# vitoplantamura/OnnxStream

Measured on AMD Instinct MI355X. Metric: sd15_unet_step_latency_ms+images_per_sec_512x512_20step, higher is better.
Workload: dtype f16

## Files before the change

include/osgpu.h:

```cpp
#ifndef OSGPU_H
#define OSGPU_H

#include <stddef.h>
#include <stdint.h>

#ifdef __cplusplus
extern "C" {
#endif

typedef struct osg_ctx osg_ctx;
typedef struct osg_graph osg_graph;

typedef enum { OSG_U8 = 1, OSG_F16 = 2, OSG_F32 = 3, OSG_I64 = 4 } osg_dtype;

typedef enum {
  OSG_ACT_NONE = 0,
  OSG_ACT_SILU = 1,
  OSG_ACT_SIGMOID = 2,
  OSG_ACT_GEGLU = 3
} osg_act;

typedef enum {
  OSG_UN_SIGMOID = 0,
  OSG_UN_ERF = 1,
  OSG_UN_SQRT = 2,
  OSG_UN_SIN = 3,
  OSG_UN_COS = 4,
  OSG_UN_NEG = 5,
  OSG_UN_POW = 6,
  OSG_UN_SILU = 7,
  OSG_UN_GELU_ERF = 8
} osg_unary_kind;

typedef enum {
  OSG_BIN_ADD = 0,
  OSG_BIN_SUB = 1,
  OSG_BIN_MUL = 2,
  OSG_BIN_DIV = 3
} osg_binary_kind;

int osg_device_count(void);
int osg_init(int device, osg_ctx** out);
void osg_destroy(osg_ctx* ctx);
const char* osg_last_error(const osg_ctx* ctx);
const char* osg_device_name(const osg_ctx* ctx);
void* osg_stream(const osg_ctx* ctx);
int osg_set_autotune(osg_ctx* ctx, int on);
int osg_tune_misses(void);

int osg_malloc(osg_ctx* ctx, size_t bytes, void** dptr);
int osg_free(osg_ctx* ctx, void* dptr);
int osg_upload(osg_ctx* ctx, void* dst, const void* host_src, size_t bytes);
int osg_upload_sync(osg_ctx* ctx, void* dst, const void* host_src, size_t bytes);
int osg_host_register(osg_ctx* ctx, void* host_ptr, size_t bytes);
int osg_host_unregister(osg_ctx* ctx, void* host_ptr);
int osg_upload_pinned(osg_ctx* ctx, void* dst, const void* pinned_host_src, size_t bytes);
int osg_upload_pinned_async(osg_ctx* ctx, void* dst, const void* pinned_host_src, size_t bytes);
int osg_copy_fence(osg_ctx* ctx);
int osg_download(osg_ctx* ctx, void* host_dst, const void* src, size_t bytes);
int osg_marker_record(osg_ctx* ctx, int slot);
int osg_copy_wait_marker(osg_ctx* ctx, int slot);
int osg_copy(osg_ctx* ctx, void* dst, const void* src, size_t bytes);
int osg_memset(osg_ctx* ctx, void* dst, int value, size_t bytes);
int osg_sync(osg_ctx* ctx);

int osg_graph_begin(osg_ctx* ctx);
int osg_graph_end(osg_ctx* ctx, osg_graph** out);
int osg_graph_launch(osg_ctx* ctx, osg_graph* g);
void osg_graph_destroy(osg_graph* g);

int osg_timer_start(osg_ctx* ctx);
int osg_timer_stop(osg_ctx* ctx, float* ms);
int osg_timer_mark(osg_ctx* ctx, int index);
int osg_timer_between(osg_ctx* ctx, int a, int b, float* ms);

void osg_range_push(const char* name);
void osg_range_pop(void);

int osg_conv2d_nhwc(osg_ctx* ctx, osg_dtype dtype, const void* x, const void* w_ohwi, const void* bias, osg_dtype bias_dtype,
                    const void* residual, void* y, int N, int H, int W, int Cin, int Cout, int KH, int KW, int stride_h,
                    int stride_w, int pad_top, int pad_left, int pad_bottom, int pad_right, osg_act act);

int osg_conv2d_nhwc_rb(osg_ctx* ctx, osg_dtype dtype, const void* x, const void* w_ohwi, const void* bias, osg_dtype bias_dtype,
                       const void* image_bias, long image_bias_ld, const void* residual, void* y, int N, int H, int W, int Cin, int Cout,
                       int KH, int KW, int stride_h, int stride_w, int pad_top, int pad_left, int pad_bottom, int pad_right, osg_act act);

int osg_conv2d_nhwc_v(osg_ctx* ctx, osg_dtype dtype, const void* x, const void* w_ohwi, const void* bias, osg_dtype bias_dtype,
                      const void* image_bias, long image_bias_ld, const void* residual, void* y, long y_ld, void* y2, long y2_ld, int N, int H, int W,
                      int Cin, int Cout, int KH, int KW, int stride_h, int stride_w, int pad_top, int pad_left, int pad_bottom, int pad_right,
                      osg_act act);

int osg_gemm(osg_ctx* ctx, osg_dtype dtype, const void* A, const void* B, int b_is_nk, const void* bias, osg_dtype bias_dtype,
             const void* residual, void* C, int M, int N, int K, int batch, long stride_a, long stride_b, long stride_c,
             osg_act act);

int osg_gemm_w8(osg_ctx* ctx, const void* A, const void* Bq_nk, float w_scale, int w_zero_point, const void* bias, osg_dtype bias_dtype,
                const void* residual, void* C, int M, int N, int K, osg_act act);
int osg_conv2d_nhwc_w8(osg_ctx* ctx, const void* x, const void* wq_ohwi, float w_scale, int w_zero_point, const void* bias,
                       osg_dtype bias_dtype, const void* image_bias, long image_bias_ld, const void* residual, void* y, int N, int H, int W,
                       int Cin, int Cout, int KH, int KW, int stride_h, int stride_w, int pad_top, int pad_left, int pad_bottom,
                       int pad_right, osg_act act);
int osg_gemm_w8_v(osg_ctx* ctx, const void* A, const void* Bq_nk, float w_scale, int w_zero_point, const float* w_scale_vec,
                  const float* w_zero_point_vec, const void* bias, osg_dtype bias_dtype, const void* residual, void* C, int M, int N, int K,
                  osg_act act);
int osg_conv2d_nhwc_w8_v(osg_ctx* ctx, const void* x, const void* wq_ohwi, float w_scale, int w_zero_point, const float* w_scale_vec,
                         const float* w_zero_point_vec, const void* bias, osg_dtype bias_dtype, const void* image_bias, long image_bias_ld,
                         const void* residual, void* y, long y_ld, void* y2, long y2_ld, int N, int H, int W, int Cin, int Cout, int KH, int KW,
                         int stride_h, int stride_w, int pad_top, int pad_left, int pad_bottom, int pad_right, osg_act act);

int osg_transpose_kn_to_nk(osg_ctx* ctx, osg_dtype dtype, const void* src_kn, void* dst_nk, int K, int N);
int osg_gemm_ln(osg_ctx* ctx, const void* x, const void* w_nk_folded, const float* c1, const float* c2, float eps, const float* rowstats,
                const void* residual, void* y, int M, int N, int K, osg_act act);
int osg_gemm_rowstats(osg_ctx* ctx, const void* A, const void* B_nk, const void* bias, osg_dtype bias_dtype, const void* residual, void* C,
                      int M, int N, int K, osg_act act, float* rowstats);
int osg_last_route(const osg_ctx* ctx, int out[5]);
int osg_last_kernel(const osg_ctx* ctx, int out[8]);

int osg_attention(osg_ctx* ctx, osg_dtype dtype, const void* q, const void* k, const void* v, void* o, int heads, int Tq, int Tkv,
                  int D, float scale, int k_is_dt);
int osg_attention_strided(osg_ctx* ctx, osg_dtype dtype, const void* q, long q_tok, long q_head, long q_batch, const void* k,
                          long k_tok, long k_head, long k_batch, const void* v, long v_tok, long v_head, long v_batch, void* o,
                          long o_tok, long o_head, long o_batch, int batch, int heads, int Tq, int Tkv, int D, float scale);
typedef struct {
  const void *a1, *x0;
  const void *wo1, *bo1;
  const void *g2, *be2;
  float eps2;
  const void *wq2, *bq2;
  const void *kp, *vtp;
  float scale;
  int Tk;
  const void *wo2, *bo2;
  const void *g3, *be3;
  float eps3;
  const void *w1, *b1, *w2, *b2;
  const void *wpo, *bpo, *xin;
  void *out, *out2;
  long ldo, ldo2;
  int M, rows_per_img, C, heads;
  void* dbg[8];
  int rows_per_block;
} osg_tblock_tail_args;
int osg_tblock_tail_supported(int M, int rows_per_img, int C, int heads, int Tk);
int osg_tblock_tail(osg_ctx* ctx, const osg_tblock_tail_args* a);
int osg_tblock_pack_weight(osg_ctx* ctx, const void* w_nk, int N, int K, void* w_kn8);
size_t osg_tblock_kv_pack_elems(int imgs, int heads, int D);
int osg_tblock_kv_pack_jobs(osg_ctx* ctx, const void* base, long ld, int imgs, int Tk, int heads, int njobs, const int* jobs_dev, void* dst);
int osg_rms_norm(osg_ctx* ctx, osg_dtype dtype, const void* x, const void* w, void* y, long rows, int C, float eps);
int osg_rope(osg_ctx* ctx, osg_dtype dtype, const void* x, const void* cos_t, const void* sin_t, void* y, long bh, long T, int d);
int osg_sdpa(osg_ctx* ctx, osg_dtype dtype, const void* q, const void* k, const void* v, const void* mask, void* o, int batch, int q_heads,
             int kv_heads, int Tq, int Tkv, int D, float scale);

int osg_instance_norm(osg_ctx* ctx, osg_dtype dtype, const void* x, const float* scale, const float* bias, void* y, int rows,
                      long L, int n_scale, float eps);
int osg_group_norm_nhwc(osg_ctx* ctx, osg_dtype dtype, const void* x, const void* gamma, const void* beta, void* y, int N, long HW,
                        int C, int groups, float eps, osg_act act);
int osg_set_stat_sinks(osg_ctx* ctx, void* table0, int groups0, int cpg0, int ch_off0, void* table1, int groups1, int cpg1, int ch_off1, int rows_per_image);
int osg_group_norm_stats_nhwc(osg_ctx* ctx, const void* x, const void* gamma, const void* beta, void* y, int N, long HW, int C, int G, float eps, osg_act act,
                              const void* stat_table);
int osg_layer_norm(osg_ctx* ctx, osg_dtype dtype, const void* x, const void* gamma, const void* beta, void* y, long rows, int C,
                   float eps);
int osg_reduce_mean_last(osg_ctx* ctx, osg_dtype dtype, const void* x, void* y, long rows, long C);
int osg_softmax_last(osg_ctx* ctx, osg_dtype dtype, const void* x, void* y, long rows, long C);

int osg_unary(osg_ctx* ctx, osg_dtype dtype, osg_unary_kind kind, const void* x, void* y, long n, float param);
int osg_binary(osg_ctx* ctx, osg_dtype dtype, osg_binary_kind kind, const void* a, const long* a_shape, const void* b,
               const long* b_shape, void* y, int rank);
int osg_geglu(osg_ctx* ctx, osg_dtype dtype, const void* x, void* y, long rows, long C);

int osg_sampler_prepare(osg_ctx* ctx, const float* x, float* sample, float* timestep, int prompts, long L, float c_in, float t,
                        long t_per_sample);
int osg_sampler_cfg_euler_a(osg_ctx* ctx, float* x, const float* eps, const float* noise, int prompts, long L, float c_out,
                            float guidance, float sigma, float d_sigma, float sigma_up, float clip);
typedef enum {
    OSG_MS_DPMPP_FIRST = 0, OSG_MS_DPMPP_2M = 1, OSG_MS_EULER_D = 2, OSG_MS_IPNDM1 = 3, OSG_MS_IPNDM_V1 = 4, OSG_MS_IPNDM2 = 5, OSG_MS_IPNDM3 = 6,
    OSG_MS_IPNDM_VO1 = 7, OSG_MS_IPNDM_VO2 = 8, OSG_MS_IPNDM_VO3 = 9, OSG_MS_TAYLOR1 = 10, OSG_MS_TAYLOR2 = 11, OSG_MS_DDIM = 12, OSG_MS_FORMS = 13
} osg_multistep_form;
int osg_sampler_cfg_multistep(osg_ctx* ctx, int form, float* x, const float* eps, float* h0, const float* h1, const float* h2, const float* h3,
                              int prompts, long L, float c_out, float guidance, float sigma, float k0, float k1, float k2, float k3, float k4,
                              double da, double db);
int osg_sampler_prepare_rescale(osg_ctx* ctx, float* x, float* sample, float* timestep, int prompts, long L, float x_scale, float c_in, float t,
                                long t_per_sample);

int osg_decode_gather(osg_ctx* ctx, const float* latents, float* tiles, int images, int H, int W, int tile, float factor);
int osg_decode_blend(osg_ctx* ctx, const float* tiles, float* image, unsigned char* pixels, int images, int H, int W, int tile, int up);

int osg_transpose(osg_ctx* ctx, int elem_size, const void* x, void* y, int rank, const long* shape, const int* perm);
int osg_copy_2d(osg_ctx* ctx, int elem_size, const void* src, long src_pitch, long src_off, void* dst, long dst_pitch,
                long dst_off, long outer, long inner);
int osg_concat2(osg_ctx* ctx, int elem_size, const void* a, long inner_a, const void* b, long inner_b, void* dst, long outer);
int osg_resize_nearest(osg_ctx* ctx, int elem_size, const void* x, void* y, int N, int C, int H, int W, int Ho, int Wo, int nhwc);
int osg_gather_rows(osg_ctx* ctx, int elem_size, const void* x, const int64_t* idx, void* y, long n_idx, long row_elems, long n_rows);
int osg_maxpool_nhwc(osg_ctx* ctx, osg_dtype dtype, const void* x, void* y, int N, int H, int W, int C, int KH, int KW, int sh,
                     int sw, int pt, int pl, int pb, int pr);

int osg_convert(osg_ctx* ctx, osg_dtype src_dtype, osg_dtype dst_dtype, const void* x, void* y, long n, float scale, int zero_point);

int osg_qu8_conv2d_nhwc(osg_ctx* ctx, const void* x, float x_scale, int x_zp, const void* w_ohwi, float w_scale, int w_zp, const float* bias_f32,
                        float out_scale, int out_zp, void* y, int N, int H, int W, int Cin, int Cout, int KH, int KW, int stride_h, int stride_w,
                        int pad_top, int pad_left, int pad_bottom, int pad_right);
int osg_qu8_conv_tap_sums(osg_ctx* ctx, const void* w_ohwi, int Cout, int KH, int KW, int Cin, int* tap_sums);
int osg_qu8_conv2d_nhwc_t(osg_ctx* ctx, const void* x, float x_scale, int x_zp, const void* w_ohwi, float w_scale, int w_zp, const float* bias_f32,
                          float out_scale, int out_zp, void* y, int N, int H, int W, int Cin, int Cout, int KH, int KW, int stride_h, int stride_w,
                          int pad_top, int pad_left, int pad_bottom, int pad_right, const int* tap_sums);
int osg_qu8_gemm(osg_ctx* ctx, const void* A, long lda, float a_scale, int a_zp, const void* B_nk, float b_scale, int b_zp, const float* bias_f32,
                 float out_scale, int out_zp, void* C, int M, int N, int K, int batch, long stride_a, long stride_b, long stride_c);
int osg_qu8_lut(osg_ctx* ctx, const void* x, void* y, long n, const void* lut256);
int osg_qu8_binary(osg_ctx* ctx, osg_binary_kind kind, const void* a, const long* a_shape, float a_scale, int a_zp, const void* b, const long* b_shape,
                   float b_scale, int b_zp, void* y, float out_scale, int out_zp, int rank);
int osg_qu8_instance_norm(osg_ctx* ctx, const void* x, void* y, int rows, long L, int n_scale, const float* scale, const float* bias, float eps,
                          float in_scale, int in_zp, float out_scale, int out_zp);
int osg_qu8_affine_act(osg_ctx* ctx, const void* x, float x_scale, int x_zp, const void* g, float g_scale, int g_zp, float m_scale, int m_zp, const void* b,
                       float b_scale, int b_zp, float a_scale, int a_zp, const void* sig_lut, float s_scale, int s_zp, float o_scale, int o_zp, void* y, long n, int C,
                       long inner);
int osg_qu8_norm_affine_act_nhwc(osg_ctx* ctx, const void* x, long HW, int C, int G, int n_scale, const float* scale, const float* bias, float eps, float x_scale,
                                 int x_zp, float n_out_scale, int n_out_zp, const void* g, float g_scale, int g_zp, float m_scale, int m_zp, const void* b, float b_scale,
                                 int b_zp, float a_scale, int a_zp, const void* sig_lut, float s_scale, int s_zp, float o_scale, int o_zp, void* y);
int osg_qu8_instance_norm_nhwc(osg_ctx* ctx, const void* x, void* y, long HW, int C, int G, int n_scale, const float* scale, const float* bias, float eps,
                               float in_scale, int in_zp, float out_scale, int out_zp);
int osg_qu8_softmax_last(osg_ctx* ctx, const void* x, void* y, long rows, long C, const void* lut_u32_256);

int osg_kdbg_read(osg_ctx* ctx, void* host_dst, size_t bytes);

#ifdef __cplusplus
}
#endif
#endif
```

onnxstream_amd/build.py:

```python
from __future__ import annotations

import glob
import os
import subprocess
import sys

ROOT = os.path.dirname(os.path.abspath(__file__))
REPO = os.path.dirname(ROOT)
CSRC = os.path.join(ROOT, "csrc")
INC = os.path.join(REPO, "include")
LIB_GPU = os.path.join(ROOT, "libosgpu.so")
LIB_HOST = os.environ.get("OSA_LIB_HOST") or os.path.join(ROOT, "libonnxstream_amd.so")
ORACLE_REF = os.path.join(REPO, "oracle", "_ref", "libonnxstream_ref.so")
HIPCC = os.environ.get("HIPCC", "/opt/rocm/bin/hipcc")


def _newer(target, deps):
    if not os.path.exists(target):
        return True
    t = os.path.getmtime(target)
    return any(os.path.getmtime(d) > t for d in deps)


def _run(cmd, **kw):
    r = subprocess.run(cmd, stdout=subprocess.PIPE, stderr=subprocess.STDOUT, text=True, **kw)
    if r.returncode != 0:
        sys.stderr.write(r.stdout)
        raise RuntimeError("build failed: " + " ".join(cmd))
    return r.stdout


def build_gpu(force=False, verbose=False):
    srcs = sorted(glob.glob(os.path.join(CSRC, "osg_*.hip")))
    hdrs = sorted(glob.glob(os.path.join(CSRC, "*.h"))) + [os.path.join(INC, "osgpu.h")]
    objdir = os.path.join(CSRC, "build")
    os.makedirs(objdir, exist_ok=True)
    objs, procs = [], []
    for s in srcs:
        o = os.path.join(objdir, os.path.basename(s)[:-4] + ".o")
        objs.append(o)
        if force or _newer(o, [s] + hdrs):
            cmd = [HIPCC, "--offload-arch=gfx950", "-O3", "-std=c++17", "-fPIC", "-mllvm", "-amdgpu-mfma-vgpr-form", "-I" + INC, "-I" + CSRC, "-c", s, "-o", o]
            procs.append((cmd, subprocess.Popen(cmd, stdout=subprocess.PIPE, stderr=subprocess.STDOUT, text=True)))
    for cmd, p in procs:
        out, _ = p.communicate()
        if p.returncode != 0:
            sys.stderr.write(out)
            raise RuntimeError("build failed: " + " ".join(cmd))
        if verbose and out:
            print(out)
    if force or procs or _newer(LIB_GPU, objs):
        _run([HIPCC, "--offload-arch=gfx950", "-shared", "-fPIC", "-o", LIB_GPU] + objs)
    return LIB_GPU


def build_host(force=False):
    hdir = os.path.join(CSRC, "host")
    srcs = sorted(glob.glob(os.path.join(hdir, "*.cpp")))
    if not srcs:
        return None
    hdrs = sorted(glob.glob(os.path.join(hdir, "*.h"))) + sorted(glob.glob(os.path.join(hdir, "*.inc"))) + [os.path.join(INC, "osgpu.h")]
    if force or _newer(LIB_HOST, srcs + hdrs):
        _run(["g++", "-std=c++20", "-O2", "-fPIC", "-shared", "-I" + INC, "-I" + hdir, "-o", LIB_HOST] + srcs +
             ["-ldl", "-lpthread"])
    return LIB_HOST


def build_oracle_ref():
    if os.path.isdir("/root/reference/src"):
        _run(["make", "-C", os.path.join(REPO, "oracle"), "ref"])
    return ORACLE_REF if os.path.exists(ORACLE_REF) else None


def build_all(force=False):
    build_gpu(force)
    build_host(force)
    build_oracle_ref()


if __name__ == "__main__":
    build_all("--force" in sys.argv)
    print("built:", LIB_GPU, LIB_HOST if os.path.exists(LIB_HOST) else "(no host yet)")
```

onnxstream_amd/csrc/osg_attention.hip:

```cpp
#include "osg_common.h"
#include <cstdlib>
#include <type_traits>
#include <utility>

namespace {

struct AttnParams {
    const f16 *q, *k, *v;
    f16* o;
    long q_tok, q_head, q_batch;
    long k_tok, k_head, k_batch;
    long v_tok, v_head, v_batch;
    long o_tok, o_head, o_batch;
    int heads, Tq, Tkv, D;
    float scale_log2e;
    const f16* mask;
    float inv_scale;
    int kv_div;
};


__device__ __forceinline__ void lane_swap16(float v, float& a, float& b) {
    a = v; b = v;
    asm volatile("s_nop 1\n\tv_permlane16_swap_b32 %0, %1" : "+v"(a), "+v"(b));
// ... 78 lines not shown
                const int dc = min(wave + c * 4, dchunks - 1);
                kreg[j][c] = *reinterpret_cast<const f16x8*>(K + krow + dc * 8);
                vreg[j][c] = *reinterpret_cast<const f16x8*>(V + vrow + dc * 8);
            }
        }
    };
    const int vcol = ((lane >> 5) << 5) + (((lane >> 2) & 3) << 3) + (((lane >> 4) & 1) << 2) + (lane & 3);
    auto store_tile = [&]() {
#pragma unroll
        for (int j = 0; j < RPL; j++)
#pragma unroll
            for (int c = 0; c < NCH; c++) {
                const int dc = wave + c * 4;
                if (dc < dchunks) {
                    const f16x8 kv8 = kreg[j][c], vv8 = vreg[j][c];
                    *reinterpret_cast<f16x8*>(&Ks[(j * 64 + lane) * KLD + dc * 8]) = kv8;
#pragma unroll
                    for (int e = 0; e < 8; e++) Vt[(dc * 8 + e) * VLD + j * 64 + vcol] = vv8[e];
                }
            }
    };
    load_tile(0);
    for (int kv0 = 0; kv0 < p.Tkv; kv0 += BKV) {
        __syncthreads();
        store_tile();
        __syncthreads();
        if (kv0 + BKV < p.Tkv) load_tile(kv0 + BKV);

        f32x4 s[QT][NT];
#pragma unroll
        for (int qt = 0; qt < QT; qt++)
#pragma unroll
            for (int t = 0; t < NT; t++) s[qt][t] = f32x4{0.f, 0.f, 0.f, 0.f};
#pragma unroll
        for (int t = 0; t < NT; t++) {
#pragma unroll
            for (int ks = 0; ks < KS; ks++) {
                f16x8 kf = *reinterpret_cast<const f16x8*>(&Ks[(t * 16 + lq) * KLD + ks * 32 + g * 8]);
#pragma unroll
                for (int qt = 0; qt < QT; qt++) s[qt][t] = __builtin_amdgcn_mfma_f32_16x16x32_f16(kf, qf[qt][ks], s[qt][t], 0, 0, 0);
            }
        }

        if (p.mask) {
#pragma unroll
            for (int qt = 0; qt < QT; qt++) {
                const f16* mrow = p.mask + (long)min(q0 + qt * 16 + lq, p.Tq - 1) * p.Tkv;
#pragma unroll
                for (int t = 0; t < NT; t++)
#pragma unroll
                    for (int r = 0; r < 4; r++)
                        s[qt][t][r] = fmaf((float)mrow[min(kv0 + t * 16 + g * 4 + r, p.Tkv - 1)], p.inv_scale, s[qt][t][r]);
            }
        }
        const bool full = kv0 + BKV <= p.Tkv;
        const float c = p.scale_log2e;
        f16x8 pf[QT][NS];
#pragma unroll
        for (int qt = 0; qt < QT; qt++) {
            float mx = -INFINITY;
            if (full) {
#pragma unroll
                for (int t = 0; t < NT; t++)
#pragma unroll
                    for (int r = 0; r < 4; r++) mx = fmaxf(mx, s[qt][t][r]);
            } else {
#pragma unroll
                for (int t = 0; t < NT; t++)
#pragma unroll
                    for (int r = 0; r < 4; r++) {
                        const int kv = kv0 + t * 16 + g * 4 + r;
                        const float x = kv < p.Tkv ? s[qt][t][r] : -INFINITY;
                        s[qt][t][r] = x;
                        mx = fmaxf(mx, x);
                    }
            }
            mx = row4_max(mx);
            const float m_new = fmaxf(m_run[qt], mx);
            const float m_use = m_new == -INFINITY ? 0.f : m_new;
            const float alpha = __builtin_amdgcn_exp2f((m_run[qt] - m_use) * c);
            const float mc = -m_use * c;
            float sum = 0.f;
#pragma unroll
            for (int t = 0; t < NT; t++)
#pragma unroll
                for (int r = 0; r < 4; r++) {
                    const float e = __builtin_amdgcn_exp2f(fmaf(s[qt][t][r], c, mc));
                    s[qt][t][r] = e;
                    sum += e;
                }
            sum = row4_sum(sum);
            l_run[qt] = l_run[qt] * alpha + sum;
            if (__builtin_amdgcn_ballot_w64(m_new != m_run[qt]) != 0) {
#pragma unroll
                for (int dt = 0; dt < DT; dt++)
#pragma unroll
                    for (int r = 0; r < 4; r++) oacc[qt][dt][r] *= alpha;
            }
            m_run[qt] = m_new;
#pragma unroll
            for (int st = 0; st < NS; st++) {
                f16x8 pv;
#pragma unroll
                for (int r = 0; r < 4; r++) {
                    pv[r] = (f16)s[qt][2 * st][r];
                    pv[4 + r] = (f16)s[qt][2 * st + 1][r];
                }
                pf[qt][st] = pv;
            }
        }

#pragma unroll
        for (int dt = 0; dt < DT; dt++) {
#pragma unroll
            for (int st = 0; st < NS; st++) {
                const f16x8 vf = *reinterpret_cast<const f16x8*>(&Vt[(dt * 16 + lq) * VLD + st * 32 + g * 8]);
#pragma unroll
                for (int qt = 0; qt < QT; qt++)
                    oacc[qt][dt] = __builtin_amdgcn_mfma_f32_16x16x32_f16(vf, pf[qt][st], oacc[qt][dt], 0, 0, 0);
            }
        }
    }

#pragma unroll
    for (int qt = 0; qt < QT; qt++) {
        const int q = q0 + qt * 16 + lq;
        if (q >= p.Tq) continue;
        const float inv = 1.0f / l_run[qt];
#pragma unroll
        for (int dt = 0; dt < DT; dt++) {
            const int d = dt * 16 + g * 4;
            if (d >= D) continue;
            f16x4 o;
#pragma unroll
            for (int r = 0; r < 4; r++) o[r] = (f16)(oacc[qt][dt][r] * inv);
            *reinterpret_cast<f16x4*>(O + (long)q * p.o_tok + d) = o;
        }
    }
}

template <class F, int... I>
__device__ __forceinline__ void attn2_static_for(F&& f, std::integer_sequence<int, I...>) { (f(std::integral_constant<int, I>{}), ...); }
template <int N>
__device__ __forceinline__ void attn2_wait_vm() { asm volatile("s_waitcnt vmcnt(%0)" ::"n"(N) : "memory"); }
typedef __fp16 attn2_hx4 __attribute__((__vector_size__(4 * sizeof(__fp16))));
template <int OFF>
__device__ __forceinline__ attn2_hx4 attn2_tr_read(unsigned lds_addr) {
    attn2_hx4 v;
    asm volatile("ds_read_b64_tr_b16 %0, %1 offset:%2" : "=v"(v) : "v"(lds_addr), "n"(OFF));
    return v;
}

template <int D, int QT, int NST>
__global__ __launch_bounds__(256) void attn2_kernel(AttnParams pk, int nqb) {
    const AttnParams p = pk;
    osg_pin_all(p.q, p.k, p.v, p.o, p.q_tok, p.q_head, p.q_batch, p.k_tok, p.k_head, p.k_batch, p.v_tok, p.v_head, p.v_batch, p.o_tok, p.o_head, p.o_batch, p.heads, p.Tq, p.Tkv,
                p.scale_log2e, p.mask, p.inv_scale, p.kv_div, nqb, (int)gridDim.x);
    constexpr int DCH = D / 8;
    constexpr int RSC = DCH + ((6 - DCH % 4) % 4);
    constexpr int ROWB = RSC * 16;
    constexpr int TILE_B = 64 * ROWB;
    constexpr int STAGE_B = 2 * TILE_B;
    constexpr int K32 = D / 32, REM = D % 32;
    static_assert(REM == 0 || REM == 8 || REM == 16, "attn2: head dim = 32 a (+ 8 | 16)");
    static_assert(RSC % 4 == 2 && RSC >= DCH && (REM == 0 || RSC * 8 >= K32 * 32 + 16), "row pitch");
    constexpr bool TAIL = REM != 0;
    constexpr int DT = (D + 15) / 16;
    static_assert(DT * 16 <= RSC * 8, "the P V row blocks read inside the padded row");
    constexpr int NT = 4, NS = 2;
    constexpr int NINST = 2 * RSC;
    constexpr int MAXP = NINST / 4;
    static_assert((NST == 3 || NST == 4) && MAXP * (NST - 2) <= 63, "three or four stages (the tile being read, the next one, one or two in flight: sync_issue's tail guard `kt + 2 >= ntiles` covers no deeper ring); vmcnt is a 6-bit counter");
    constexpr unsigned OOB = 0x80000000u;
    extern __shared__ __attribute__((aligned(16))) char asmem[];
    typedef __attribute__((address_space(3))) void* lds_ptr;
    typedef attn2_hx4 hx4;

    const int tid = threadIdx.x, lane = tid & 63;
    const int wave = __builtin_amdgcn_readfirstlane(tid >> 6);
    const int lq = lane & 15, g = lane >> 4;
    int L;
    {
        const int total = gridDim.x, bid = blockIdx.x, x = bid & 7, i = bid >> 3, q = total >> 3, r = total & 7;
        L = (x < r ? x * (q + 1) : r * (q + 1) + (x - r) * q) + i;
    }
    const int bh = L / nqb, qb = L - bh * nqb;
    const int b = bh / p.heads, h = bh - b * p.heads;
    const int q0 = qb * (64 * QT) + wave * (16 * QT);

    const f16* __restrict__ Q = p.q + b * p.q_batch + h * p.q_head;
    const f16* __restrict__ K = p.k + b * p.k_batch + (h / p.kv_div) * p.k_head;
    const f16* __restrict__ V = p.v + b * p.v_batch + (h / p.kv_div) * p.v_head;
    f16* __restrict__ O = p.o + b * p.o_batch + h * p.o_head;

    const long kext = ((long)(p.Tkv - 1) * p.k_tok + D) * 2, vext = ((long)(p.Tkv - 1) * p.v_tok + D) * 2;
    __amdgpu_buffer_rsrc_t rsK = __builtin_amdgcn_make_buffer_rsrc((void*)K, 0, (int)(kext < 0x7ffffff0L ? kext : 0x7ffffff0L), 0x00020000);
    __amdgpu_buffer_rsrc_t rsV = __builtin_amdgcn_make_buffer_rsrc((void*)V, 0, (int)(vext < 0x7ffffff0L ? vext : 0x7ffffff0L), 0x00020000);

    int p_off[MAXP], p_row[MAXP];
#pragma unroll
    for (int j = 0; j < MAXP; j++) {
        const int i = wave + 4 * j;
        const bool isv = i >= RSC;
        const int c = (isv ? i - RSC : i) * 64 + lane;
        const int row = c / RSC, pp = c - row * RSC;
        p_row[j] = pp < DCH ? row : 64;
        p_off[j] = (int)(((long)row * (isv ? p.v_tok : p.k_tok) + pp * 8) * 2);
    }
    const int ntiles = (p.Tkv + 63) >> 6;
    auto issue_tile = [&](int kt) __attribute__((always_inline)) {
        char* st = asmem + (kt % NST) * STAGE_B;
        const int kv0 = kt << 6, left = min(p.Tkv - kv0, 64);
        const int sk = (int)((long)kv0 * p.k_tok * 2), sv = (int)((long)kv0 * p.v_tok * 2);
#pragma unroll
        for (int j = 0; j < MAXP; j++) {
            const int i = wave + 4 * j;
            const unsigned off = p_row[j] < left ? (unsigned)p_off[j] : OOB;
            if (i < RSC) __builtin_amdgcn_raw_ptr_buffer_load_lds(rsK, (lds_ptr)(st + i * 1024), 16, off, sk, 0, 0);
            else __builtin_amdgcn_raw_ptr_buffer_load_lds(rsV, (lds_ptr)(st + i * 1024), 16, off, sv, 0, 0);
        }
    };

    f16x8 qf[QT][K32 ? K32 : 1];
    f16x8 qtail[QT];
#pragma unroll
    for (int qt = 0; qt < QT; qt++) {
        const int q = q0 + qt * 16 + lq;
        const f16* qrow = Q + (long)min(q, p.Tq - 1) * p.q_tok;
#pragma unroll
        for (int ks = 0; ks < K32; ks++) qf[qt][ks] = *reinterpret_cast<const f16x8*>(qrow + ks * 32 + g * 8);
        if constexpr (TAIL) {
            const int d = K32 * 32 + g * 8;
            f16x8 v = *reinterpret_cast<const f16x8*>(qrow + min(d, D - 8));
            if (d >= D) v = f16x8{0, 0, 0, 0, 0, 0, 0, 0};
            qtail[qt] = v;
        }
    }
#pragma unroll
    for (int s2 = 0; s2 < NST - 1; s2++)
        if (s2 < ntiles) issue_tile(s2);

    f32x4 oacc[QT][DT], lacc[QT];
    float m_run[QT];
#pragma unroll
    for (int qt = 0; qt < QT; qt++) {
        m_run[qt] = -INFINITY;
        lacc[qt] = f32x4{0.f, 0.f, 0.f, 0.f};
#pragma unroll
        for (int dt = 0; dt < DT; dt++) oacc[qt][dt] = f32x4{0.f, 0.f, 0.f, 0.f};
    }
    const f16x8 ones = {(f16)1, (f16)1, (f16)1, (f16)1, (f16)1, (f16)1, (f16)1, (f16)1};

    int kofs[K32 + 1];
#pragma unroll
    for (int ks = 0; ks < K32 + 1; ks++) kofs[ks] = lq * ROWB + (ks * 4 + g) * 16;
    const int vofs = TILE_B + (g * 4 + (lq >> 2)) * ROWB + (lq & 3) * 8;
    const float c = p.scale_log2e;

    auto qk = [&](auto stc, f32x4 (&s)[QT][NT]) __attribute__((always_inline)) {
        constexpr int stg = decltype(stc)::value;
        const char* St = asmem + stg * STAGE_B;
#pragma unroll
        for (int qt = 0; qt < QT; qt++)
#pragma unroll
            for (int t = 0; t < NT; t++) s[qt][t] = f32x4{0.f, 0.f, 0.f, 0.f};
#pragma unroll
        for (int ks = 0; ks < K32 + (TAIL ? 1 : 0); ks++)
#pragma unroll
            for (int t = 0; t < NT; t++) {
                const f16x8 kf = *reinterpret_cast<const f16x8*>(St + t * 16 * ROWB + kofs[ks]);
#pragma unroll
                for (int qt = 0; qt < QT; qt++) s[qt][t] = __builtin_amdgcn_mfma_f32_16x16x32_f16(kf, ks < K32 ? qf[qt][ks < K32 ? ks : 0] : qtail[qt], s[qt][t], 0, 0, 0);
            }
    };
    auto softmax = [&](auto fullc, f32x4 (&s)[QT][NT], int kv0, f16x8 (&pf)[QT][NS]) __attribute__((always_inline)) {
        constexpr bool full = decltype(fullc)::value;
#pragma unroll
        for (int qt = 0; qt < QT; qt++) {
            float mx = -INFINITY;
            if constexpr (full) {
#pragma unroll
                for (int t = 0; t < NT; t++)
#pragma unroll
                    for (int r = 0; r < 4; r++) mx = fmaxf(mx, s[qt][t][r]);
            } else {
#pragma unroll
                for (int t = 0; t < NT; t++)
#pragma unroll
                    for (int r = 0; r < 4; r++) {
                        const int kv = kv0 + t * 16 + g * 4 + r;
                        const float x = kv < p.Tkv ? s[qt][t][r] : -INFINITY;
                        s[qt][t][r] = x;
                        mx = fmaxf(mx, x);
                    }
            }
            mx = row4_max(mx);
            const float m_new = fmaxf(m_run[qt], mx);
            const float mc = -m_new * c;
            if (__builtin_amdgcn_ballot_w64(m_new != m_run[qt]) != 0) {
                const float alpha = __builtin_amdgcn_exp2f((m_run[qt] - m_new) * c);
#pragma unroll
                for (int dt = 0; dt < DT; dt++)
#pragma unroll
                    for (int r = 0; r < 4; r++) oacc[qt][dt][r] *= alpha;
#pragma unroll
                for (int r = 0; r < 4; r++) lacc[qt][r] *= alpha;
            }
            m_run[qt] = m_new;
#pragma unroll
            for (int st = 0; st < NS; st++) {
                f16x8 pv;
#pragma unroll
                for (int r = 0; r < 4; r++) {
                    pv[r] = (f16)__builtin_amdgcn_exp2f(fmaf(s[qt][2 * st][r], c, mc));
                    pv[4 + r] = (f16)__builtin_amdgcn_exp2f(fmaf(s[qt][2 * st + 1][r], c, mc));
                }
                pf[qt][st] = pv;
            }
        }
    };
    auto pvstep = [&](auto stc, f16x8 (&pf)[QT][NS]) __attribute__((always_inline)) {
        constexpr int stg = decltype(stc)::value;
#pragma unroll
        for (int st = 0; st < NS; st++)
#pragma unroll
            for (int qt = 0; qt < QT; qt++) lacc[qt] = __builtin_amdgcn_mfma_f32_16x16x32_f16(ones, pf[qt][st], lacc[qt], 0, 0, 0);
        constexpr int SB = stg * STAGE_B, IMM = (SB + 48 * ROWB + DT * 32 < 65536) ? SB : 0;
        const unsigned va = (unsigned)(size_t)(lds_ptr)(asmem + vofs + (SB - IMM));
        hx4 vr[2][NS][2];
        auto vread = [&](auto dtc) __attribute__((always_inline)) {
            constexpr int dt = decltype(dtc)::value;
            vr[dt & 1][0][0] = attn2_tr_read<IMM + 0 * ROWB + dt * 32>(va);
            vr[dt & 1][0][1] = attn2_tr_read<IMM + 16 * ROWB + dt * 32>(va);
            vr[dt & 1][1][0] = attn2_tr_read<IMM + 32 * ROWB + dt * 32>(va);
            vr[dt & 1][1][1] = attn2_tr_read<IMM + 48 * ROWB + dt * 32>(va);
        };
        auto vstep = [&](auto dtc) __attribute__((always_inline)) {
            constexpr int dt = decltype(dtc)::value;
            hx4 &a0 = vr[dt & 1][0][0], &a1 = vr[dt & 1][0][1], &a2 = vr[dt & 1][1][0], &a3 = vr[dt & 1][1][1];
            if constexpr (dt + 1 < DT) {
                vread(std::integral_constant<int, dt + 1>{});
                asm volatile("s_waitcnt lgkmcnt(4)" : "+v"(a0), "+v"(a1), "+v"(a2), "+v"(a3)::"memory");
            } else asm volatile("s_waitcnt lgkmcnt(0)" : "+v"(a0), "+v"(a1), "+v"(a2), "+v"(a3)::"memory");
#pragma unroll
            for (int st = 0; st < NS; st++) {
                const hx4 lo = vr[dt & 1][st][0], hi = vr[dt & 1][st][1];
                const f16x8 vf = {(f16)lo[0], (f16)lo[1], (f16)lo[2], (f16)lo[3], (f16)hi[0], (f16)hi[1], (f16)hi[2], (f16)hi[3]};
#pragma unroll
                for (int qt = 0; qt < QT; qt++)
                    oacc[qt][dt] = __builtin_amdgcn_mfma_f32_16x16x32_f16(vf, pf[qt][st], oacc[qt][dt], 0, 0, 0);
            }
        };
        vread(std::integral_constant<int, 0>{});
        attn2_static_for(vstep, std::make_integer_sequence<int, DT>{});
    };
    auto sync_issue = [&](int kt) __attribute__((always_inline)) {
        if (NST == 3 || kt + 2 >= ntiles) attn2_wait_vm<0>();
        else attn2_wait_vm<MAXP * (NST - 3)>();
        __builtin_amdgcn_s_barrier();
        if (kt + NST - 1 < ntiles) issue_tile(kt + NST - 1);
    };
    f32x4 sA[QT][NT], sB[QT][NT];
    sync_issue(-1);
    qk(std::integral_constant<int, 0>{}, sA);
    constexpr int U = (NST % 2) ? 2 * NST : NST;
    auto step = [&](auto ic, int kt) __attribute__((always_inline)) {
        constexpr int i = decltype(ic)::value;
        f32x4 (&sc)[QT][NT] = (i & 1) ? sB : sA;
        f32x4 (&sn)[QT][NT] = (i & 1) ? sA : sB;
        f16x8 pf[QT][NS];
        sync_issue(kt);
        qk(std::integral_constant<int, (i + 1) % NST>{}, sn);
        softmax(std::true_type{}, sc, kt << 6, pf);
        pvstep(std::integral_constant<int, i % NST>{}, pf);
    };
    auto last = [&](auto ic, int kt) __attribute__((always_inline)) {
        constexpr int i = decltype(ic)::value;
        f32x4 (&sc)[QT][NT] = (i & 1) ? sB : sA;
        f16x8 pf[QT][NS];
        if ((p.Tkv & 63) == 0) softmax(std::true_type{}, sc, kt << 6, pf);
        else softmax(std::false_type{}, sc, kt << 6, pf);
        pvstep(std::integral_constant<int, i % NST>{}, pf);
    };
    int kt = 0;
    for (; kt + U < ntiles; kt += U)
        attn2_static_for([&](auto ic) __attribute__((always_inline)) { step(ic, kt + decltype(ic)::value); }, std::make_integer_sequence<int, U>{});
    bool done = false;
    attn2_static_for([&](auto ic) __attribute__((always_inline)) {
        const int k2 = kt + decltype(ic)::value;
        if (!done) {
            if (k2 + 1 < ntiles) step(ic, k2);
            else { last(ic, k2); done = true; }
        }
    }, std::make_integer_sequence<int, U>{});

#pragma unroll
    for (int qt = 0; qt < QT; qt++) {
        const int q = q0 + qt * 16 + lq;
        if (q >= p.Tq) continue;
        const float inv = 1.0f / lacc[qt][0];
#pragma unroll
        for (int dt = 0; dt < DT; dt++) {
            const int d = dt * 16 + g * 4;
            if (d >= D) continue;
            f16x4 o;
#pragma unroll
            for (int r = 0; r < 4; r++) o[r] = (f16)(oacc[qt][dt][r] * inv);
            *reinterpret_cast<f16x4*>(O + (long)q * p.o_tok + d) = o;
        }
    }
}

template <int D, int NST>
int launch_attn2(osg_ctx* ctx, const AttnParams& p, int batch) {
    static const int force_qt = getenv("OSG_ATTN_QT") ? atoi(getenv("OSG_ATTN_QT")) : 0;
    constexpr int RSC = D / 8 + ((6 - (D / 8) % 4) % 4);
    constexpr size_t smem = (size_t)NST * 2 * 64 * RSC * 16;
    static_assert(smem <= 160 * 1024, "LDS budget");
    const long blocks128 = (long)((p.Tq + 127) / 128) * batch * p.heads;
    const bool qt2 = p.Tq >= 1024 && force_qt != 1 && (blocks128 >= 2L * ctx->num_cu || force_qt == 2);
    auto k1 = attn2_kernel<D, 1, NST>;
    auto k2 = attn2_kernel<D, 2, NST>;
    static unsigned long long attr_mask = 0;
    if (osg_first_on_device(attr_mask)) {
        OSG_HIP(ctx, hipFuncSetAttribute((const void*)k1, hipFuncAttributeMaxDynamicSharedMemorySize, (int)smem));
        OSG_HIP(ctx, hipFuncSetAttribute((const void*)k2, hipFuncAttributeMaxDynamicSharedMemorySize, (int)smem));
    }
    const int nqb = qt2 ? (p.Tq + 127) / 128 : (p.Tq + 63) / 64;
    dim3 grid((unsigned)((long)nqb * batch * p.heads));
    osg_set_kernel(ctx, 0, 2, D, NST, qt2 ? 2 : 1, 64, (int)grid.x);
    if (qt2) hipLaunchKernelGGL(k2, grid, dim3(256), smem, ctx->compute, p, nqb);
    else hipLaunchKernelGGL(k1, grid, dim3(256), smem, ctx->compute, p, nqb);
    OSG_LAUNCH_CHECK(ctx);
    return 0;
}

template <int DP, int DT>
int launch_attn(osg_ctx* ctx, const AttnParams& p, int batch) {
    static const int force_qt = getenv("OSG_ATTN_QT") ? atoi(getenv("OSG_ATTN_QT")) : 0;
    const long blocks128 = (long)((p.Tq + 127) / 128) * batch * p.heads;
    static const int force_bkv = getenv("OSG_ATTN_BKV") ? atoi(getenv("OSG_ATTN_BKV")) : 0;
    constexpr bool kWide = DP <= 64;
    const bool wide = kWide && force_bkv == 128;
    if (p.Tq >= 1024 && force_qt != 1 && (blocks128 >= 2L * ctx->num_cu || force_qt == 2)) {
        dim3 grid((p.Tq + 127) / 128, batch * p.heads);
        osg_set_kernel(ctx, 0, 1, DP, DT, 2, wide ? 128 : 64, (int)(grid.x * grid.y));
        if constexpr (kWide) {
            if (wide) hipLaunchKernelGGL((attn_kernel<DP, DT, 2, 128>), grid, dim3(256), 0, ctx->compute, p);
            else hipLaunchKernelGGL((attn_kernel<DP, DT, 2, 64>), grid, dim3(256), 0, ctx->compute, p);
        } else hipLaunchKernelGGL((attn_kernel<DP, DT, 2, 64>), grid, dim3(256), 0, ctx->compute, p);
    } else {
        dim3 grid((p.Tq + 63) / 64, batch * p.heads);
        osg_set_kernel(ctx, 0, 1, DP, DT, 1, wide ? 128 : 64, (int)(grid.x * grid.y));
        if constexpr (kWide) {
            if (wide) hipLaunchKernelGGL((attn_kernel<DP, DT, 1, 128>), grid, dim3(256), 0, ctx->compute, p);
            else hipLaunchKernelGGL((attn_kernel<DP, DT, 1, 64>), grid, dim3(256), 0, ctx->compute, p);
        } else hipLaunchKernelGGL((attn_kernel<DP, DT, 1, 64>), grid, dim3(256), 0, ctx->compute, p);
    }
    OSG_LAUNCH_CHECK(ctx);
    return 0;
}

int dispatch_attn(osg_ctx* ctx, const AttnParams& p, int batch) {
    const int D = p.D;
    static const int v1 = getenv("OSG_ATTN_V1") ? atoi(getenv("OSG_ATTN_V1")) : 0;
    if (!v1 && !p.mask && (long)p.Tkv * max(p.k_tok, p.v_tok) * 2 < 0x7fffffffL) {
        if (D == 40) return launch_attn2<40, 4>(ctx, p, batch);
        if (D == 64) return launch_attn2<64, 3>(ctx, p, batch);
        if (D == 80) return launch_attn2<80, 3>(ctx, p, batch);
        if (D == 160) return launch_attn2<160, 3>(ctx, p, batch);
    }
    if (D <= 32) return launch_attn<32, 2>(ctx, p, batch);
    if (D <= 48) return launch_attn<64, 3>(ctx, p, batch);
    if (D <= 64) return launch_attn<64, 4>(ctx, p, batch);
    if (D <= 80) return launch_attn<96, 5>(ctx, p, batch);
    if (D <= 96) return launch_attn<96, 6>(ctx, p, batch);
    if (D <= 128) return launch_attn<128, 8>(ctx, p, batch);
    if (D <= 160) return launch_attn<160, 10>(ctx, p, batch);
    OSG_FAIL(ctx, "osg_attention: head dim > 160 not implemented");
}

}

extern "C" {

int osg_attention_strided(osg_ctx* ctx, osg_dtype dtype, const void* q, long q_tok, long q_head, long q_batch, const void* k, long k_tok,
                          long k_head, long k_batch, const void* v, long v_tok, long v_head, long v_batch, void* o, long o_tok,
                          long o_head, long o_batch, int batch, int heads, int Tq, int Tkv, int D, float scale) {
    if (dtype != OSG_F16) OSG_FAIL(ctx, "osg_attention: only f16 arithmetic is implemented on the device");
    if (batch <= 0 || heads <= 0 || Tq <= 0 || Tkv <= 0 || D <= 0) OSG_FAIL(ctx, "osg_attention: invalid shape(s) of q, k and/or v");
    if (!(scale > 0.f)) OSG_FAIL(ctx, "osg_attention: the fused kernel tracks the row maximum of the raw scores and needs scale > 0");
    if (D % 8) OSG_FAIL(ctx, "osg_attention: head dim must be a multiple of 8");
    if ((q_tok | q_head | q_batch | k_tok | k_head | k_batch | v_tok | v_head | v_batch) % 8 || (o_tok | o_head | o_batch) % 4)
        OSG_FAIL(ctx, "osg_attention: strides must keep 16-byte (q,k,v) / 8-byte (o) alignment");
    AttnParams p{(const f16*)q, (const f16*)k, (const f16*)v, (f16*)o, q_tok, q_head, q_batch, k_tok, k_head, k_batch,
                 v_tok, v_head, v_batch, o_tok, o_head, o_batch, heads, Tq, Tkv, D, scale * 1.4426950408889634f, nullptr, 0.f, 1};
    return dispatch_attn(ctx, p, batch);
}

int osg_sdpa(osg_ctx* ctx, osg_dtype dtype, const void* q, const void* k, const void* v, const void* mask, void* o, int batch, int q_heads,
             int kv_heads, int Tq, int Tkv, int D, float scale) {
    if (dtype != OSG_F16) OSG_FAIL(ctx, "osg_sdpa: only f16 arithmetic is implemented on the device");
    if (batch <= 0 || q_heads <= 0 || kv_heads <= 0 || Tq <= 0 || Tkv <= 0 || D <= 0) OSG_FAIL(ctx, "ScaledDotProductAttention: invalid shape of query, key or value.");
    if (q_heads % kv_heads) OSG_FAIL(ctx, "ScaledDotProductAttention: query heads must be a multiple of key/value heads.");
    if (!(scale > 0.f)) OSG_FAIL(ctx, "osg_sdpa: the fused kernel tracks the row maximum of the raw scores and needs scale > 0");
    if (D % 8) OSG_FAIL(ctx, "osg_sdpa: head dim must be a multiple of 8");
    const long qh = (long)Tq * D, kh = (long)Tkv * D;
    AttnParams p{(const f16*)q, (const f16*)k, (const f16*)v, (f16*)o, D, qh, qh * q_heads, D, kh, kh * kv_heads, D, kh, kh * kv_heads,
                 D, qh, qh * q_heads, q_heads, Tq, Tkv, D, scale * 1.4426950408889634f, (const f16*)mask, 1.0f / scale, q_heads / kv_heads};
    return dispatch_attn(ctx, p, batch);
}

int osg_attention(osg_ctx* ctx, osg_dtype dtype, const void* q, const void* k, const void* v, void* o, int heads, int Tq, int Tkv, int D,
                  float scale, int k_is_dt) {
    if (dtype != OSG_F16) OSG_FAIL(ctx, "osg_attention: only f16 arithmetic is implemented on the device");
    const void* kk = k;
    if (k_is_dt) {
        size_t bytes = (size_t)heads * D * Tkv * sizeof(f16);
        if (osg_ensure_workspace2(ctx, bytes)) return 1;
        long shape[3] = {heads, D, Tkv};
        int perm[3] = {0, 2, 1};
        if (osg_transpose(ctx, 2, k, ctx->ws2, 3, shape, perm)) return 1;
        kk = ctx->ws2;
    }
    return osg_attention_strided(ctx, dtype, q, D, (long)Tq * D, 0, kk, D, (long)Tkv * D, 0, v, D, (long)Tkv * D, 0, o, D, (long)Tq * D, 0,
                                 1, heads, Tq, Tkv, D, scale);
}

}
```

onnxstream_amd/csrc/osg_conv3x3_kernel.h:

```cpp
#pragma once
#include "osg_gemm_common.h"
#include <algorithm>
#include <array>
#include <cmath>
#include <cstdlib>
#include <type_traits>

using namespace osg_mm;

namespace {

template <int I> using ic = std::integral_constant<int, I>;
template <int B, int E, class F>
__device__ __forceinline__ void static_for(F&& f) {
    if constexpr (B < E) {
        f(ic<B>{});
        static_for<B + 1, E>(f);
    }
}

template <int N> __device__ __forceinline__ void wait_vmcnt() { asm volatile("s_waitcnt vmcnt(%0)" ::"n"(N) : "memory"); }

template <int W_, int BN, int NLW = 4, int WQ = 0>
struct Geo {
    static constexpr int TI = W_ == 8 ? 2 : 1;
    static constexpr int TH = 128 / (W_ * TI);
    static constexpr int PW = W_ == 8 ? 16 : W_ + 2;
    static constexpr int PH = TH + 2;
    static constexpr int PPI = PH * PW;
    static constexpr int PP = TI * PPI;
    static constexpr int NPW = ((PP + 7) / 8 + NLW - 1) / NLW;
    static constexpr int PATCH_BYTES = NPW * NLW * 1024;
    static constexpr int BRW = WQ ? 16 : 8;
    static constexpr int WLB = ((BN + BRW - 1) / BRW + NLW - 1) / NLW;
    static constexpr int BST_BYTES = WLB * NLW * 1024;
    static constexpr int NSTW_ = (160 * 1024 - 2 * PATCH_BYTES) / BST_BYTES;
    static constexpr int NSTW = NSTW_ > 8 ? 8 : NSTW_;
    static constexpr int D = NSTW - 1;
    static constexpr int PT = 10 - D;
    static constexpr int PPT = (NPW + PT - 1) / PT;
    static constexpr size_t SMEM = 2 * (size_t)PATCH_BYTES + (size_t)NSTW * BST_BYTES;
    static constexpr bool OK = D >= 3 && PT >= 2;
    static constexpr int patch_loads(int t) {
        if (t >= PT) return 0;
        int n = NPW - t * PPT;
        return n < 0 ? 0 : (n > PPT ? PPT : n);
    }
    static constexpr int allowed_outstanding(int t) {
        int n = 0;
        for (int d = 1; d <= D - 2; d++) n += WLB + patch_loads((t - d + 18) % 9);
        return n;
    }
};

template <int W_, int BN, int WGM, int WGN, int MODE, int NLW, int WQ = 0>
__device__ __forceinline__ void conv3x3_body(const GemmParams& p) {
    using G = Geo<W_, BN, NLW, WQ>;
    constexpr int TI = G::TI, TH = G::TH, PW = G::PW, PPI = G::PPI, PP = G::PP, NPW = G::NPW, PATCH_BYTES = G::PATCH_BYTES;
    constexpr int WLB = G::WLB, BST_BYTES = G::BST_BYTES, NSTW = G::NSTW, D = G::D, PPT = G::PPT;
    constexpr int WM = 128 / WGM, WN = BN / WGN, TM = WM / 16, TN = WN / 16;
    static_assert(WM % 16 == 0 && WN % 16 == 0 && WGM * WGN == 4, "bad wave layout");
    constexpr unsigned OOB = 0x80000000u;

    extern __shared__ __attribute__((aligned(16))) char smem3[];
    typedef __attribute__((address_space(3))) void* lds_ptr;
    char* const patch0 = smem3;
    char* const bst0 = smem3 + 2 * PATCH_BYTES;

    kdbg_stamp(p, 0);
    const int tid = threadIdx.x;
    const int lane = tid & 63;
    const int wave8 = __builtin_amdgcn_readfirstlane(tid >> 6);
    const bool loader = wave8 >= 4;
    const int wave = loader ? wave8 - 4 : wave8;

    int L;
    {
        const int total = p.grid, bid = blockIdx.x, x = bid & 7, i = bid >> 3, q = total >> 3, r = total & 7;
        L = (x < r ? x * (q + 1) : r * (q + 1) + (x - r) * q) + i;
    }
    int m_tile, n_tile, zs;
    if (p.n_major) {
        n_tile = L / (p.splits * p.mt); L -= n_tile * p.splits * p.mt;
        zs = L / (p.mt); m_tile = L - zs * p.mt;
    } else {
        m_tile = L / (p.splits * p.nt); L -= m_tile * p.splits * p.nt;
        zs = L / (p.nt); n_tile = L - zs * p.nt;
    }
    const int m0 = m_tile * 128, n0 = n_tile * BN;
    const int slab_b = zs * (p.k_per_split >> 6);
    const int slab_e = min(p.Cin >> 6, slab_b + (p.k_per_split >> 6));

    if (loader) {
        const int img0 = m0 / (p.H * W_);
        const int y0 = (m0 - img0 * p.H * W_) / W_;
        __amdgpu_buffer_rsrc_t rsA = __builtin_amdgcn_make_buffer_rsrc((void*)p.A, 0, p.a_bytes, 0x00020000);
        __amdgpu_buffer_rsrc_t rsB = __builtin_amdgcn_make_buffer_rsrc((void*)p.Bt, 0, p.b_bytes, 0x00020000);
        const int rsub = lane >> 3;
        const int gch = (lane & 7) ^ rsub;
        unsigned pa_off[NPW];
#pragma unroll
        for (int pc = 0; pc < NPW; pc++) {
            const int pp = (pc * NLW + wave) * 8 + rsub;
            const int ti = pp / PPI, rr = pp - ti * PPI;
            const int py = rr / PW, px = rr - py * PW;
            const int img = img0 + ti, y = y0 + py - 1, x = px - 1;
            const bool ok = pp < PP && (unsigned)y < (unsigned)p.H && (unsigned)x < (unsigned)W_ && img * p.H * W_ < p.M;
            pa_off[pc] = ok ? (unsigned)((((img * p.H + y) * W_ + x) * p.Cin + gch * 8) * 2) : OOB;
        }
        unsigned b_off[WLB];
#pragma unroll
        for (int j = 0; j < WLB; j++) {
            if constexpr (WQ) {
                const int nl = (j * NLW + wave) * 16 + (lane >> 2);
                const int n = n0 + nl;
                b_off[j] = (nl < BN && n < p.N) ? (unsigned)((long)n * p.K + (((lane & 3) ^ ((lane >> 4) & 3)) << 4)) : OOB;
            } else {
                const int nl = (j * NLW + wave) * 8 + rsub;
                const int n = n0 + nl;
                b_off[j] = (nl < BN && n < p.N) ? (unsigned)(((long)n * p.K + gch * 8) * 2) : OOB;
            }
        }
        auto issue_patch_piece = [&](int pc, int slab, char* buf) {
            if (MODE >= 3 && MODE != 6) return;
            const unsigned kill = (slab < slab_e && MODE != 2) ? 0u : OOB;
            __builtin_amdgcn_raw_ptr_buffer_load_lds(rsA, (lds_ptr)(buf + (pc * NLW + wave) * 1024), 16, pa_off[pc] | kill, slab * 128, 0, 0);
        };
        auto issue_weights = [&](int stage, int tap, int slab) {
            if (MODE >= 3 && MODE != 6) return;
            const unsigned kill = (slab < slab_e && MODE != 2) ? 0u : OOB;
            const int soff = (tap * p.Cin + slab * 64) * (WQ ? 1 : 2);
            char* dst = bst0 + stage * BST_BYTES;
#pragma unroll
            for (int j = 0; j < WLB; j++)
                __builtin_amdgcn_raw_ptr_buffer_load_lds(rsB, (lds_ptr)(dst + (j * NLW + wave) * 1024), 16, b_off[j] | kill, soff, 0, 0);
        };
        issue_weights(0, 0, slab_b);
#pragma unroll
        for (int pc = 0; pc < NPW; pc++) issue_patch_piece(pc, slab_b, patch0);
#pragma unroll
        for (int d = 1; d < D; d++) issue_weights(d, d % 9, slab_b + d / 9);
        wait_vmcnt<(D - 1) * WLB>();
        __builtin_amdgcn_s_barrier();
        int ust = 0;
        for (int slab = slab_b; slab < slab_e; slab++) {
            char* patch_next = patch0 + (((slab - slab_b) & 1) ^ 1) * PATCH_BYTES;
            static_for<0, 9>([&](auto tc) {
                constexpr int t = decltype(tc)::value;
                wait_vmcnt<G::allowed_outstanding(t)>();
                if (MODE != 5) __builtin_amdgcn_s_barrier();
                constexpr int td = (t + D) % 9;
                int std_ = ust + D;
                std_ = std_ >= NSTW ? std_ - NSTW : std_;
                issue_weights(std_, td, slab + (t + D) / 9);
                static_for<0, G::patch_loads(t)>([&](auto pc) { issue_patch_piece(t * PPT + decltype(pc)::value, slab + 1, patch_next); });
                ust = ust + 1 == NSTW ? 0 : ust + 1;
            });
        }
        asm volatile("s_waitcnt vmcnt(0)" ::: "memory");
        return;
    }

    const int wm0 = (wave / WGN) * WM;
    const int wn0 = (wave % WGN) * WN;
    f32x4 acc[TM][TN];
#pragma unroll
    for (int i = 0; i < TM; i++)
#pragma unroll
        for (int j = 0; j < TN; j++) acc[i][j] = f32x4{0.f, 0.f, 0.f, 0.f};

    const int frow = lane & 15, fq = lane >> 4;
    int pp0[TM];
#pragma unroll
    for (int i = 0; i < TM; i++) {
        const int ml = wm0 + i * 16 + frow;
        const int ti = ml / (TH * W_), rr = ml - ti * (TH * W_);
        const int ty = rr / W_, tx = rr - ty * W_;
        pp0[i] = ti * PPI + ty * PW + tx;
    }
    const int b_rd = WQ ? (wn0 + frow) * 64 + ((((lane >> 5) & 1) ^ ((frow >> 2) & 3)) << 4) + ((lane >> 4) & 1) * 8 : (wn0 + frow) * 128 + ((fq ^ (frow & 7)) << 4);
    constexpr bool W8SC = false;
    W8Ops<WQ ? TN : 1, W8SC> w8;
    if constexpr (WQ) w8_prefetch<TN, W8SC>(p, w8, n0, wn0, lane);

    f16x8 fa0[TM], fb0[TN], fa1[TM], fb1[TN];
    auto read_frags = [&](f16x8 (&fa)[TM], f16x8 (&fb)[TN], const char* pbuf, const char* bbuf, int tap_off, int ks) {
        if (MODE == 1 || (MODE == 4 && ks == 1)) return;
#pragma unroll
        for (int i = 0; i < TM; i++) {
            const int pp = pp0[i] + tap_off;
            fa[i] = *reinterpret_cast<const f16x8*>(pbuf + ((pp * 128 + ((fq ^ (pp & 7)) << 4)) ^ (ks << 6)));
        }
#pragma unroll
        for (int j = 0; j < TN; j++) {
            if constexpr (WQ) fb[j] = w8_frag(*reinterpret_cast<const u32x2v*>(bbuf + ((b_rd + j * 16 * 64) ^ (ks << 5))), w8.zz[j]);
            else fb[j] = *reinterpret_cast<const f16x8*>(bbuf + ((b_rd + j * 16 * 128) ^ (ks << 6)));
        }
    };
    auto mma = [&](f16x8 (&fa)[TM], f16x8 (&fb)[TN]) {
        if (MODE == 1) return;
#pragma unroll
        for (int i = 0; i < TM; i++)
#pragma unroll
            for (int j = 0; j < TN; j++) acc[i][j] = __builtin_amdgcn_mfma_f32_16x16x32_f16(fb[j], fa[i], acc[i][j], 0, 0, 0);
    };

    u32x2v rb0[WQ ? TN : 1], rb1[WQ ? TN : 1];
    auto read_a = [&](f16x8 (&fa)[TM], const char* pbuf, int tap_off, int ks) {
#pragma unroll
        for (int i = 0; i < TM; i++) {
            const int pp = pp0[i] + tap_off;
            fa[i] = *reinterpret_cast<const f16x8*>(pbuf + ((pp * 128 + ((fq ^ (pp & 7)) << 4)) ^ (ks << 6)));
        }
    };
    auto read_codes = [&](u32x2v (&rb)[WQ ? TN : 1], const char* bbuf, int ks) {
        if constexpr (WQ) {
#pragma unroll
            for (int j = 0; j < TN; j++) rb[j] = *reinterpret_cast<const u32x2v*>(bbuf + ((b_rd + j * 16 * 64) ^ (ks << 5)));
        }
    };
    auto convert = [&](f16x8 (&fb)[TN], const u32x2v (&rb)[WQ ? TN : 1]) {
        if constexpr (WQ) {
#pragma unroll
            for (int j = 0; j < TN; j++) fb[j] = w8_frag(rb[j], w8.zz[j]);
        }
    };

    constexpr bool EPRE = TM * TN <= 10 && NLW == 4;
    EpiOps<TM, TN, true, EPRE> epre;
    epi_prefetch<TM, TN, true, EPRE>(p, epre, m0, n0, wm0, wn0, lane, 0);
    kdbg_stamp(p, 1);
    __builtin_amdgcn_s_barrier();
    kdbg_stamp(p, 2);
    if constexpr (WQ) {
        w8_finalize<TN, W8SC>(w8);
        read_a(fa0, patch0, 0, 0);
        read_codes(rb0, bst0, 0);
        read_codes(rb1, bst0, 1);
        convert(fb0, rb0);
    } else
    read_frags(fa0, fb0, patch0, bst0, 0, 0);
    if (MODE == 4) {
#pragma unroll
        for (int i = 0; i < TM; i++) fa1[i] = fa0[i];
#pragma unroll
        for (int j = 0; j < TN; j++) fb1[j] = fb0[j];
    }
    int ust = 0;
    for (int slab = slab_b; slab < slab_e; slab++) {
        const char* patch = patch0 + ((slab - slab_b) & 1) * PATCH_BYTES;
        const char* patch_next = patch0 + (((slab - slab_b) & 1) ^ 1) * PATCH_BYTES;
        static_for<0, 9>([&](auto tc) {
            constexpr int t = decltype(tc)::value;
            if (MODE != 5) __builtin_amdgcn_s_barrier();
            constexpr int kh = t / 3, kw = t % 3;
            const char* Bs = bst0 + ust * BST_BYTES;
            if constexpr (WQ) {
                constexpr int KV = (8 * TN + TM * TN - 1) / (TM * TN);
                const int ustn = ust + 1 == NSTW ? 0 : ust + 1;
                const char* Bn = bst0 + ustn * BST_BYTES;
                read_a(fa1, patch, kh * PW + kw, 1);
                read_codes(rb0, Bn, 0);
                convert(fb1, rb1);
                mma(fa0, fb0);
                static_for<0, TM * TN>([&](auto ic_) {
                    __builtin_amdgcn_sched_group_barrier(0x008, 1, 0);
                    if constexpr (decltype(ic_)::value < TM + TN) __builtin_amdgcn_sched_group_barrier(0x100, 1, 0);
                    __builtin_amdgcn_sched_group_barrier(0x002, KV, 0);
                });
                __builtin_amdgcn_sched_barrier(0);
                ust = ustn;
                constexpr int tn8 = (t + 1) % 9;
                read_a(fa0, t == 8 ? patch_next : patch, (tn8 / 3) * PW + tn8 % 3, 0);
                read_codes(rb1, Bn, 1);
                convert(fb0, rb0);
                mma(fa1, fb1);
                static_for<0, TM * TN>([&](auto ic_) {
                    __builtin_amdgcn_sched_group_barrier(0x008, 1, 0);
                    if constexpr (decltype(ic_)::value < TM + TN) __builtin_amdgcn_sched_group_barrier(0x100, 1, 0);
                    __builtin_amdgcn_sched_group_barrier(0x002, KV, 0);
                });
                __builtin_amdgcn_sched_barrier(0);
            } else if constexpr (MODE == 0 || MODE == 7) {
                read_frags(fa1, fb1, patch, Bs, kh * PW + kw, 1);
                mma(fa0, fb0);
                if constexpr (MODE == 0) {
                    static_for<0, TM + TN>([&](auto) { __builtin_amdgcn_sched_group_barrier(0x008, 1, 0); __builtin_amdgcn_sched_group_barrier(0x100, 1, 0); });
                    __builtin_amdgcn_sched_group_barrier(0x008, TM * TN - (TM + TN), 0);
                } else {
                    static_for<0, TM + TN>([&](auto) { __builtin_amdgcn_sched_group_barrier(0x100, 1, 0); __builtin_amdgcn_sched_group_barrier(0x008, 1, 0); });
                    __builtin_amdgcn_sched_group_barrier(0x008, TM * TN - (TM + TN), 0);
                }
                __builtin_amdgcn_sched_barrier(0);
                ust = ust + 1 == NSTW ? 0 : ust + 1;
                constexpr int tn6 = (t + 1) % 9;
                read_frags(fa0, fb0, t == 8 ? patch_next : patch, bst0 + ust * BST_BYTES, (tn6 / 3) * PW + tn6 % 3, 0);
                mma(fa1, fb1);
                if constexpr (MODE == 0) {
                    static_for<0, TM + TN>([&](auto) { __builtin_amdgcn_sched_group_barrier(0x008, 1, 0); __builtin_amdgcn_sched_group_barrier(0x100, 1, 0); });
                    __builtin_amdgcn_sched_group_barrier(0x008, TM * TN - (TM + TN), 0);
                } else {
                    static_for<0, TM + TN>([&](auto) { __builtin_amdgcn_sched_group_barrier(0x100, 1, 0); __builtin_amdgcn_sched_group_barrier(0x008, 1, 0); });
                    __builtin_amdgcn_sched_group_barrier(0x008, TM * TN - (TM + TN), 0);
                }
                __builtin_amdgcn_sched_barrier(0);
            } else {
            read_frags(fa1, fb1, patch, Bs, kh * PW + kw, 1);
            __builtin_amdgcn_sched_barrier(0);
            mma(fa0, fb0);
            __builtin_amdgcn_sched_barrier(0);
            ust = ust + 1 == NSTW ? 0 : ust + 1;
            constexpr int tn = (t + 1) % 9;
            if (MODE != 4) read_frags(fa0, fb0, t == 8 ? patch_next : patch, bst0 + ust * BST_BYTES, (tn / 3) * PW + tn % 3, 0);
            __builtin_amdgcn_sched_barrier(0);
            mma(fa1, fb1);
            __builtin_amdgcn_sched_barrier(0);
            }
        });
    }
    kdbg_stamp(p, 3);
    if constexpr (WQ) { if constexpr (W8SC) w8_scale_acc<TM, TN>(w8, acc); else w8_scale_acc_late<TM, TN>(p, acc, n0, wn0, lane); }
    kdbg_stamp(p, 4);
    float* stat_lds = nullptr;
    if (OSG_UNLIKELY(p.sink[0].table || p.sink[1].table)) {
        __builtin_amdgcn_s_barrier();
        stat_lds = reinterpret_cast<float*>(smem3) + (wave8 & 3) * (WN * 2);
    }
    if constexpr (MODE == 0) {
        if (OSG_UNLIKELY(p.splits > 1 && p.fold_acc)) {
            if (!splitk_fold_acc<TM, TN>(p, acc, m_tile * p.nt + n_tile, zs, reinterpret_cast<int*>(smem3), tid)) return;
            EpiOps<TM, TN, true, false> none;
            none.have = false;
            gemm_epilogue_fast<TM, TN, true, false, false>(p, acc, m0, n0, wm0, wn0, lane, 0, none, nullptr);
            return;
        }
    }
    gemm_epilogue<TM, TN, true, EPRE, false>(p, acc, m0, n0, wm0, wn0, lane, 0, zs, epre, stat_lds);
    kdbg_stamp(p, 5);
    if (OSG_UNLIKELY(p.kdbg != nullptr)) { asm volatile("s_waitcnt vmcnt(0)" ::: "memory"); kdbg_stamp(p, 6); }
}

template <int W_, int BN, int WGM, int WGN, int MODE, int NLW, int WQ = 0>
__global__ __launch_bounds__(256 + 64 * NLW) void conv3x3_kernel(GemmParams pk) {
    GemmParams p = pk;
    OSG_PIN(p.A); OSG_PIN(p.Bt); OSG_PIN(p.kdbg); OSG_PIN(p.M); OSG_PIN(p.N); OSG_PIN(p.K); OSG_PIN(p.splits); OSG_PIN(p.k_per_split); OSG_PIN(p.a_bytes); OSG_PIN(p.b_bytes);
    OSG_PIN(p.mt); OSG_PIN(p.nt); OSG_PIN(p.n_major); OSG_PIN(p.grid); OSG_PIN(p.H); OSG_PIN(p.Cin);
    OSG_PIN(p.bias); OSG_PIN(p.residual); OSG_PIN(p.rowbias); OSG_PIN(p.rb_ld); OSG_PIN(p.rb_rows); OSG_PIN(p.bias_f32); OSG_PIN(p.act); OSG_PIN(p.no_epre);
    if constexpr (WQ) { OSG_PIN(p.wq_sc); OSG_PIN(p.wq_zp); OSG_PIN(p.w_zp); }
    conv3x3_body<W_, BN, WGM, WGN, MODE, NLW, WQ>(p);
}

template <int W_, int BN, int WGM, int WGN, int MODE = 0, int NLW = 4, int WQ = 0>
int launch3(osg_ctx* ctx, GemmParams& p) {
    constexpr size_t smem = Geo<W_, BN, NLW, WQ>::SMEM;
    static_assert(smem <= 160 * 1024, "LDS budget");
    static_assert(Geo<W_, BN, NLW, WQ>::OK, "pipeline depth out of range");
    auto kern = conv3x3_kernel<W_, BN, WGM, WGN, MODE, NLW, WQ>;
    static unsigned long long attr_mask = 0;
    if (osg_first_on_device(attr_mask)) {
        OSG_HIP(ctx, hipFuncSetAttribute((const void*)kern, hipFuncAttributeMaxDynamicSharedMemorySize, (int)smem));
    }
    p.mt = (p.M + 127) / 128;
    p.nt = (p.N + BN - 1) / BN;
    p.no_epre = osg_mm::no_epi_prefetch();
    p.kdbg = kdbg_buffer(ctx, (long)p.mt * p.nt * p.splits);
    const osg_mm::StatSink sinks_in[2] = {p.sink[0], p.sink[1]};
    if (p.sink[0].table || p.sink[1].table) {
        const bool ok = !ctx->tuning && p.splits == 1 && MODE == 0 && (p.N & 3) == 0 && ((p.ldc | p.ldc2) & 3) == 0 && p.sink_hw > 0 && p.sink_hw % 128 == 0 && p.M % p.sink_hw == 0;
        if (ok) { ctx->sink_fused = true; p.sink_imgs = p.M / p.sink_hw; p.sink_per_xcd = ctx->xcd_ids8 ? 1 : 0; }
        else p.sink[0].table = p.sink[1].table = nullptr;
    }
    p.grid = p.mt * p.nt * p.splits;
    hipLaunchKernelGGL(kern, dim3((unsigned)p.grid), dim3(256 + 64 * NLW), smem, ctx->compute, p);
    p.sink[0] = sinks_in[0]; p.sink[1] = sinks_in[1];
    OSG_LAUNCH_CHECK(ctx);
    return 0;
}

using V3Launch = int (*)(osg_ctx*, GemmParams&);
template <int UNIT, int I>
constexpr V3Launch v3_launcher() {
    constexpr V3Entry e = kV3Entries[I];
    if constexpr (v3_unit(e) == UNIT) return launch3<e.w, e.bn, e.wgm, e.wgn, 0, e.nlw, e.wq>;
    else return nullptr;
}
template <int UNIT, size_t... I>
constexpr std::array<V3Launch, kV3Count> v3_launchers(std::index_sequence<I...>) { return {v3_launcher<UNIT, (int)I>()...}; }
template <int UNIT>
int launch3_in_unit(int entry, osg_ctx* ctx, GemmParams& p) {
    static constexpr std::array<V3Launch, kV3Count> table = v3_launchers<UNIT>(std::make_index_sequence<kV3Count>{});
    return table[entry](ctx, p);
}

}
```

onnxstream_amd/csrc/osg_gemm.hip:

```cpp
#include "osg_gemm_common.h"
#include "osg_tune.h"
#include <algorithm>
#include <climits>
#include <cmath>
#include <cstdio>
#include <cstdlib>

using namespace osg_mm;

namespace {

template <int BM, int BN, int BK, bool CONV, bool VEC>
__global__ __launch_bounds__(256) void gemm_kernel(GemmParams p) {
    constexpr int LDS = BK + 8;
    constexpr int CPR = BK / 8;
    constexpr int ROWS_PER_PASS = 256 / CPR;
    constexpr int A_IT = BM / ROWS_PER_PASS;
    constexpr int B_IT = BN / ROWS_PER_PASS;
    constexpr int WM = BM / 2, WN = BN / 2;
    constexpr int TM = WM / 16, TN = WN / 16;
    static_assert(A_IT >= 1 && B_IT >= 1, "tile too small for 256 threads");

    extern __shared__ __attribute__((aligned(16))) f16 smem[];
    f16* As0 = smem;
// ... 662 lines not shown
}


static int conv2d_route(osg_ctx* ctx, GemmParams& p, int N, int Cin, int Cout, int KH, int KW, int sh, int sw, int pt, int pl, int pb, int pr);

extern "C" {

int osg_transpose_kn_to_nk(osg_ctx* ctx, osg_dtype dtype, const void* src, void* dst, int K, int N) {
    if (dtype != OSG_F16) OSG_FAIL(ctx, "osg_transpose_kn_to_nk: only f16 implemented");
    dim3 grid((N + 31) / 32, (K + 31) / 32);
    hipLaunchKernelGGL(transpose_kn_nk_kernel, grid, dim3(256), 0, ctx->compute, (const f16*)src, (f16*)dst, K, N);
    OSG_LAUNCH_CHECK(ctx);
    return 0;
}

int osg_gemm(osg_ctx* ctx, osg_dtype dtype, const void* A, const void* B, int b_is_nk, const void* bias, osg_dtype bias_dtype,
             const void* residual, void* C, int M, int N, int K, int batch, long stride_a, long stride_b, long stride_c,
             osg_act act) {
    if (dtype != OSG_F16) OSG_FAIL(ctx, "osg_gemm: only f16 arithmetic is implemented on the device");
    if (M <= 0 || N <= 0 || K <= 0 || batch <= 0) OSG_FAIL(ctx, "osg_gemm: invalid shape of inputs");
    if (bias && bias_dtype != OSG_F16 && bias_dtype != OSG_F32) OSG_FAIL(ctx, "osg_gemm: invalid bias dtype");
    if (act == OSG_ACT_GEGLU && (!b_is_nk || residual || N % 32 || K % 64 || batch != 1))
        OSG_FAIL(ctx, "osg_gemm: the GEGLU epilogue needs a pair-interleaved [N,K] weight, N % 32 == 0, K % 64 == 0, no residual");
    const f16* Bt = (const f16*)B;
    long sb = stride_b;
    if (!b_is_nk) {
        int nb = stride_b ? batch : 1;
        size_t bytes = (size_t)nb * K * N * sizeof(f16);
        if (osg_ensure_workspace2(ctx, bytes)) return 1;
        f16* tmp = (f16*)ctx->ws2;
        for (int b = 0; b < nb; b++) {
            dim3 grid((N + 31) / 32, (K + 31) / 32);
            hipLaunchKernelGGL(transpose_kn_nk_kernel, grid, dim3(256), 0, ctx->compute, (const f16*)B + (long)b * stride_b,
                               tmp + (long)b * K * N, K, N);
            OSG_LAUNCH_CHECK(ctx);
        }
        Bt = tmp;
        sb = stride_b ? (long)K * N : 0;
    }
    GemmParams p{};
    p.A = (const f16*)A; p.Bt = Bt; p.C = (f16*)C; p.bias = bias; p.residual = (const f16*)residual;
    p.M = M; p.N = N; p.K = K; p.lda = K;
    p.strideA = stride_a; p.strideB = sb; p.strideC = stride_c;
    p.bias_f32 = bias_dtype == OSG_F32; p.act = act;
    return run_gemm<false>(ctx, p, batch);
}

int osg_gemm_rowstats(osg_ctx* ctx, const void* A, const void* B_nk, const void* bias, osg_dtype bias_dtype, const void* residual, void* C, int M, int N,
                      int K, osg_act act, float* rowstats) {
    if (M <= 0 || N <= 0 || K <= 0) OSG_FAIL(ctx, "osg_gemm_rowstats: invalid shape of inputs");
    if (!rowstats || N % 32 || K % 64 || act == OSG_ACT_GEGLU) OSG_FAIL(ctx, "osg_gemm_rowstats: needs N % 32 == 0, K % 64 == 0, a plain activation");
    if (bias && bias_dtype != OSG_F16 && bias_dtype != OSG_F32) OSG_FAIL(ctx, "osg_gemm_rowstats: invalid bias dtype");
    GemmParams p{};
    p.A = (const f16*)A; p.Bt = (const f16*)B_nk; p.C = (f16*)C; p.bias = bias; p.residual = (const f16*)residual;
    p.M = M; p.N = N; p.K = K; p.lda = K;
    p.bias_f32 = bias_dtype == OSG_F32; p.act = act;
    p.rs_out = rowstats; p.rs_np = N / 32;
    return run_gemm<false>(ctx, p, 1);
}

int osg_gemm_ln(osg_ctx* ctx, const void* x, const void* w_nk_folded, const float* c1, const float* c2, float eps, const float* rowstats,
                const void* residual, void* y, int M, int N, int K, osg_act act) {
    if (M <= 0 || N <= 0 || K <= 0) OSG_FAIL(ctx, "osg_gemm_ln: invalid shape of inputs");
    if (!c1 || !c2) OSG_FAIL(ctx, "osg_gemm_ln: c1 and c2 are required");
    if (K % 64 || N % 4) OSG_FAIL(ctx, "osg_gemm_ln: needs K % 64 == 0, N % 4 == 0");
    if (act == OSG_ACT_GEGLU && (residual || N % 32)) OSG_FAIL(ctx, "osg_gemm_ln: the GEGLU epilogue needs N % 32 == 0 and no residual");
    GemmParams p{};
    p.A = (const f16*)x; p.Bt = (const f16*)w_nk_folded; p.C = (f16*)y; p.bias = c2; p.residual = (const f16*)residual;
    p.M = M; p.N = N; p.K = K; p.lda = K;
    p.bias_f32 = 1; p.act = act;
    p.ln_c1 = c1; p.ln_eps = eps;
    if (rowstats) {
        if (K % 32 || K > 1280) OSG_FAIL(ctx, "osg_gemm_ln: handed-over row statistics need K % 32 == 0, K <= 1280");
        p.rs_in = rowstats; p.rs_np = K / 32;
    }
    return run_gemm<false>(ctx, p, 1);
}

int osg_conv2d_nhwc(osg_ctx* ctx, osg_dtype dtype, const void* x, const void* w, const void* bias, osg_dtype bias_dtype,
                    const void* residual, void* y, int N, int H, int W, int Cin, int Cout, int KH, int KW, int sh, int sw,
                    int pt, int pl, int pb, int pr, osg_act act) {
    return osg_conv2d_nhwc_rb(ctx, dtype, x, w, bias, bias_dtype, nullptr, 0, residual, y, N, H, W, Cin, Cout, KH, KW, sh, sw, pt, pl, pb, pr, act);
}

int osg_conv2d_nhwc_rb(osg_ctx* ctx, osg_dtype dtype, const void* x, const void* w, const void* bias, osg_dtype bias_dtype,
                       const void* image_bias, long image_bias_ld, const void* residual, void* y, int N, int H, int W, int Cin, int Cout,
                       int KH, int KW, int sh, int sw, int pt, int pl, int pb, int pr, osg_act act) {
    return osg_conv2d_nhwc_v(ctx, dtype, x, w, bias, bias_dtype, image_bias, image_bias_ld, residual, y, 0, nullptr, 0, N, H, W, Cin, Cout, KH, KW, sh, sw, pt, pl,
                             pb, pr, act);
}

int osg_set_stat_sinks(osg_ctx* ctx, void* table0, int groups0, int cpg0, int ch_off0, void* table1, int groups1, int cpg1, int ch_off1, int rows_per_image) {
    if ((table0 && (groups0 <= 0 || cpg0 <= 0 || ch_off0 < 0)) || (table1 && (groups1 <= 0 || cpg1 <= 0 || ch_off1 < 0)) || rows_per_image <= 0)
        OSG_FAIL(ctx, "osg_set_stat_sinks: invalid argument");
    ctx->pending_sink[0] = osg_ctx::PendingSink{(long long*)table0, groups0, cpg0, ch_off0};
    ctx->pending_sink[1] = osg_ctx::PendingSink{(long long*)table1, groups1, cpg1, ch_off1};
    ctx->pending_hw = rows_per_image;
    return 0;
}

struct W8Quant { int on; float scale; int zp; const float* sc; const float* zv; };

static int conv2d_v(osg_ctx* ctx, const W8Quant& q, const void* x, const void* w, const void* bias, osg_dtype bias_dtype,
                    const void* image_bias, long image_bias_ld, const void* residual, void* y, long y_ld, void* y2, long y2_ld, int N, int H, int W,
                    int Cin, int Cout, int KH, int KW, int sh, int sw, int pt, int pl, int pb, int pr, osg_act act);

int osg_conv2d_nhwc_v(osg_ctx* ctx, osg_dtype dtype, const void* x, const void* w, const void* bias, osg_dtype bias_dtype,
                      const void* image_bias, long image_bias_ld, const void* residual, void* y, long y_ld, void* y2, long y2_ld, int N, int H, int W,
                      int Cin, int Cout, int KH, int KW, int sh, int sw, int pt, int pl, int pb, int pr, osg_act act) {
    if (dtype != OSG_F16) OSG_FAIL(ctx, "osg_conv2d_nhwc: only f16 arithmetic is implemented on the device");
    return conv2d_v(ctx, W8Quant{}, x, w, bias, bias_dtype, image_bias, image_bias_ld, residual, y, y_ld, y2, y2_ld, N, H, W, Cin, Cout, KH, KW, sh, sw, pt, pl, pb, pr, act);
}

static int w8_check(osg_ctx* ctx, const char* who, const W8Quant& q, int N, int K, const void* a, const void* b) {
    if (K % 64 || ((uintptr_t)a & 15) || ((uintptr_t)b & 15)) { ctx->err = (std::string(who) + ": K (Cin) must be a multiple of 64 and the operands 16-byte aligned"); return 1; }
    if ((q.sc != nullptr) != (q.zv != nullptr) || (q.sc && ((N & 3) || ((uintptr_t)q.sc & 15)))) { ctx->err = (std::string(who) + ": scale / zero-point vectors come as a pair, N % 4 == 0, 16-byte aligned"); return 1; }
    if (!q.sc && (q.zp < 0 || q.zp > 255)) { ctx->err = (std::string(who) + ": zero point outside 0 .. 255"); return 1; }
    return 0;
}

int osg_gemm_w8_v(osg_ctx* ctx, const void* A, const void* Bq_nk, float w_scale, int w_zero_point, const float* w_scale_vec, const float* w_zero_point_vec,
                  const void* bias, osg_dtype bias_dtype, const void* residual, void* C, int M, int N, int K, osg_act act) {
    if (M <= 0 || N <= 0 || K <= 0) OSG_FAIL(ctx, "osg_gemm_w8: invalid shape of inputs");
    if (bias && bias_dtype != OSG_F16 && bias_dtype != OSG_F32) OSG_FAIL(ctx, "osg_gemm_w8: invalid bias dtype");
    if (act == OSG_ACT_GEGLU && (residual || N % 32)) OSG_FAIL(ctx, "osg_gemm_w8: the GEGLU epilogue needs a pair-interleaved [N,K] weight, N % 32 == 0, no residual");
    const W8Quant q{1, w_scale, w_zero_point, w_scale_vec, w_zero_point_vec};
    if (w8_check(ctx, "osg_gemm_w8", q, N, K, A, Bq_nk)) return 1;
    GemmParams p{};
    p.A = (const f16*)A; p.Bt = (const f16*)Bq_nk; p.C = (f16*)C; p.bias = bias; p.residual = (const f16*)residual;
    p.M = M; p.N = N; p.K = K; p.lda = K;
    p.bias_f32 = bias_dtype == OSG_F32; p.act = act;
    p.w8 = 1; p.w_scale = w_scale; p.w_zp = w_zero_point; p.wq_sc = w_scale_vec; p.wq_zp = w_zero_point_vec;
    return run_gemm<false>(ctx, p, 1);
}

int osg_gemm_w8(osg_ctx* ctx, const void* A, const void* Bq_nk, float w_scale, int w_zero_point, const void* bias, osg_dtype bias_dtype,
                const void* residual, void* C, int M, int N, int K, osg_act act) {
    return osg_gemm_w8_v(ctx, A, Bq_nk, w_scale, w_zero_point, nullptr, nullptr, bias, bias_dtype, residual, C, M, N, K, act);
}

int osg_conv2d_nhwc_w8_v(osg_ctx* ctx, const void* x, const void* wq_ohwi, float w_scale, int w_zero_point, const float* w_scale_vec, const float* w_zero_point_vec,
                         const void* bias, osg_dtype bias_dtype, const void* image_bias, long image_bias_ld, const void* residual, void* y, long y_ld, void* y2,
                         long y2_ld, int N, int H, int W, int Cin, int Cout, int KH, int KW, int sh, int sw, int pt, int pl, int pb, int pr, osg_act act) {
    const W8Quant q{1, w_scale, w_zero_point, w_scale_vec, w_zero_point_vec};
    if (w8_check(ctx, "osg_conv2d_nhwc_w8", q, Cout, Cin, x, wq_ohwi)) return 1;
    return conv2d_v(ctx, q, x, wq_ohwi, bias, bias_dtype, image_bias, image_bias_ld, residual, y, y_ld, y2, y2_ld, N, H, W, Cin, Cout, KH, KW, sh, sw, pt, pl, pb, pr, act);
}

int osg_conv2d_nhwc_w8(osg_ctx* ctx, const void* x, const void* wq_ohwi, float w_scale, int w_zero_point, const void* bias,
                       osg_dtype bias_dtype, const void* image_bias, long image_bias_ld, const void* residual, void* y, int N, int H, int W,
                       int Cin, int Cout, int KH, int KW, int sh, int sw, int pt, int pl, int pb, int pr, osg_act act) {
    return osg_conv2d_nhwc_w8_v(ctx, x, wq_ohwi, w_scale, w_zero_point, nullptr, nullptr, bias, bias_dtype, image_bias, image_bias_ld, residual, y, 0, nullptr, 0, N, H, W,
                                Cin, Cout, KH, KW, sh, sw, pt, pl, pb, pr, act);
}

}

static int conv2d_v(osg_ctx* ctx, const W8Quant& q, const void* x, const void* w, const void* bias, osg_dtype bias_dtype,
                    const void* image_bias, long image_bias_ld, const void* residual, void* y, long y_ld, void* y2, long y2_ld, int N, int H, int W,
                    int Cin, int Cout, int KH, int KW, int sh, int sw, int pt, int pl, int pb, int pr, osg_act act) {
    if (y_ld < 0 || (y_ld && y_ld < Cout) || (y2 && y2_ld < Cout)) OSG_FAIL(ctx, "osg_conv2d_nhwc_v: an output pitch is smaller than Cout");
    if (Cout % 4 == 0 && ((y_ld & 3) || (y2 && (y2_ld & 3)))) OSG_FAIL(ctx, "osg_conv2d_nhwc_v: output pitches must be multiples of 4 elements");
    if ((y_ld && ((uintptr_t)y & 7)) || (y2 && ((uintptr_t)y2 & 7))) OSG_FAIL(ctx, "osg_conv2d_nhwc_v: output views must be 8-byte aligned");
    if (N <= 0 || H <= 0 || W <= 0 || Cin <= 0 || Cout <= 0 || KH <= 0 || KW <= 0 || sh <= 0 || sw <= 0)
        OSG_FAIL(ctx, "osg_conv2d_nhwc: invalid argument");
    int Ho = (H + pt + pb - KH) / sh + 1;
    int Wo = (W + pl + pr - KW) / sw + 1;
    if (Ho <= 0 || Wo <= 0) OSG_FAIL(ctx, "osg_conv2d_nhwc: empty output");
    if ((long)N * Ho * Wo > INT_MAX) OSG_FAIL(ctx, "osg_conv2d_nhwc: more than 2^31 - 1 output pixels");
    GemmParams p{};
    p.A = (const f16*)x; p.Bt = (const f16*)w; p.C = (f16*)y; p.bias = bias; p.residual = (const f16*)residual;
    p.M = N * Ho * Wo; p.N = Cout; p.K = KH * KW * Cin; p.lda = 0;
    p.bias_f32 = bias_dtype == OSG_F32; p.act = act;
    p.a_bytes_l = (long)N * H * W * Cin * 2;
    p.rowbias = (const f16*)image_bias; p.rb_rows = Ho * Wo; p.rb_ld = image_bias_ld;
    p.H = H; p.W = W; p.Cin = Cin; p.Ho = Ho; p.Wo = Wo; p.KW = KW; p.sh = sh; p.sw = sw; p.pt = pt; p.pl = pl;
    p.ldc = y_ld == Cout ? 0 : y_ld; p.C2 = (f16*)y2; p.ldc2 = y2 ? y2_ld : 0;
    if (q.on) { p.w8 = 1; p.w_scale = q.scale; p.w_zp = q.zp; p.wq_sc = q.sc; p.wq_zp = q.zv; }
    bool want_sinks = false;
    for (int k = 0; k < 2; k++) {
        const auto& ps = ctx->pending_sink[k];
        if (ps.table && (k == 0 || y2)) {
            p.sink[k] = StatSink{ps.table, ps.groups, ps.cpg, ps.ch_off};
            want_sinks = true;
        }
        ctx->pending_sink[k] = osg_ctx::PendingSink{};
    }
    p.sink_hw = ctx->pending_hw;
    ctx->sink_fused = false;
    if (want_sinks && (p.sink_hw <= 0 || p.sink_hw != Ho * Wo)) OSG_FAIL(ctx, "osg_conv2d_nhwc_v: the statistics sinks were set for another image size");
    if (epi_check(ctx, p)) return 1;
    const int rc = conv2d_route(ctx, p, N, Cin, Cout, KH, KW, sh, sw, pt, pl, pb, pr);
    if (rc || !want_sinks || ctx->sink_fused) return rc;
    return osg_mm::launch_colstats(ctx, p.C, p.ldc ? p.ldc : (long)Cout, p.M, Cout, p.sink_hw, p.sink);
}

static int conv2d_route(osg_ctx* ctx, GemmParams& p, int N, int Cin, int Cout, int KH, int KW, int sh, int sw, int pt, int pl, int pb, int pr) {
    (void)N;
    if (!p.w8 && Cin == 4 && KH == 3 && KW == 3 && Cout % 16 == 0 && (size_t)Cout * (144 + 4) <= 160 * 1024 && (p.ldc % 4) == 0 && (p.ldc2 % 4) == 0 &&
        (!p.rowbias || p.rb_ld % 4 == 0)) {
        const size_t smem = (size_t)Cout * (144 + 4);
        static size_t attr_smem = 0;
        if (smem > 64 * 1024 && smem > attr_smem) {
            OSG_HIP(ctx, hipFuncSetAttribute((const void*)conv_cin4_mfma_kernel, hipFuncAttributeMaxDynamicSharedMemorySize, (int)smem));
            attr_smem = smem;
        }
        hipLaunchKernelGGL(conv_cin4_mfma_kernel, dim3((p.M + 31) / 32), dim3(256), smem, ctx->compute, p);
        OSG_LAUNCH_CHECK(ctx);
        osg_set_route(ctx, 3, 0, 1, 0);
        return 0;
    }
    if (KH == 1 && KW == 1 && sh == 1 && sw == 1 && pt == 0 && pl == 0 && pb == 0 && pr == 0) {
        p.lda = Cin;
        return run_gemm<false>(ctx, p, 1);
    }
    if (KH == 3) {
        const bool env_forced = getenv("OSG_CONV3X3_BN") || getenv("OSG_CONV3X3_SPLITS") || getenv("OSG_CONV3X3_DBG") || getenv("OSG_GEMM_CFG") ||
                                getenv("OSG_GEMM_SPLITS") || getenv("OSG_GEMM_NST");
        if (!ctx->autotune || env_forced) {
            int rc3 = osg_conv3x3_run(ctx, p);
            if (rc3 >= 0) return rc3;
        } else if (osg_conv3x3_prepare(ctx, p) == 0) {
            const osg_tune::Key key = tune_key(ctx, 1, p, 1);
            osg_tune::Choice tc;
            if (!osg_tune::lookup(key, &tc)) {
                auto r3 = osg_conv3x3_rank(ctx, p);
                tc = osg_tune::Choice{1, 0, 0, r3.empty() ? 1 : r3[0].second.second % 1000, r3.empty() ? 128 : r3[0].second.first, -1.f};
                if (!ctx->capturing && tune_safe(p) && !osg_tune::frozen()) {
                    float best = -1.f;
                    static const bool dump3 = getenv("OSG_TUNE_DUMP") != nullptr;
                    for (auto& c : r3)
                        for (int nl : {4, 8}) {
                            static const bool no8 = getenv("OSG_TUNE_NO_NL8") != nullptr;
                            if (nl == 8 && (no8 || p.w8)) continue;
                            const int fold3 = c.second.second >= 1000;
                            const int s3 = c.second.second % 1000;
                            const float us = osg_tune::time_us(ctx, [&] { return osg_conv3x3_launch(ctx, p, c.second.first, s3, nl, fold3); });
                            if (dump3) fprintf(stderr, "[tune] conv3x3 N*H*W=%d Cin=%d Cout=%d W=%d: halo bn=%d splits=%d loaders=%d -> %.2f us\n", p.M, p.Cin, p.N, p.W, c.second.first, c.second.second, nl, us);
                            if (us >= 0.f && (best < 0.f || us < best)) { best = us; tc = osg_tune::Choice{1, tune_cfg(V2Choice{0, nl, s3, 1, fold3}), nl, s3, c.second.first, us}; }
                        }
                    V2Form form3;
                    form3.conv = true; form3.w8 = p.w8 != 0;
                    auto r2 = rank_v2(ctx, p.M, p.N, p.K, 1, true, form3);
                    if (r2.size() > 6) r2.resize(6);
                    for (auto& c : r2) {
                        const V2Choice ch = c.second;
                        const float us = osg_tune::time_us(ctx, [&] { return run_gemm<true>(ctx, p, 1, &ch); });
                        if (us >= 0.f && (best < 0.f || us < best)) { best = us; tc = osg_tune::Choice{0, tune_cfg(ch), ch.nst, ch.splits, 0, us}; }
                    }
                    if (best < 0.f) OSG_FAIL(ctx, "osg_conv2d_nhwc: autotune could not time any configuration");
                    osg_tune::store(key, tc);
                } else if (osg_tune::frozen())
                    osg_tune::remember(key, tc);
            }
            const V2Choice ch = tune_choice(tc.cfg, tc.nst, tc.splits);
            if (tc.family == 1) return osg_conv3x3_launch(ctx, p, tc.bn, tc.splits, tc.nst == 8 ? 8 : 4, ch.fold);
            return run_gemm<true>(ctx, p, 1, &ch);
        }
    }
    return run_gemm<true>(ctx, p, 1);
}
```

onnxstream_amd/csrc/osg_gemm2.h:

```cpp
#pragma once
#include "osg_gemm_common.h"
#include "osg_tune.h"
#include <array>
#include <type_traits>

#ifndef OSG_GEMM_PIN
#define OSG_GEMM_PIN 1
#endif

namespace {
using namespace osg_mm;

template <int BM, int BN, int NST, bool CONV, int MODE = 0, int SPEC = 0, int LN = 0, int NCH = 5, int KS = 1, int WGN = 2, int WQ = 0>
__global__ __launch_bounds__((SPEC || KS == 2) ? 512 : 256) void gemm2_kernel(GemmParams pk) {
    GemmParams p = pk;
#if OSG_GEMM_PIN
    OSG_PIN(p.A); OSG_PIN(p.Bt); OSG_PIN(p.kdbg); OSG_PIN(p.lda); OSG_PIN(p.strideA); OSG_PIN(p.strideB); OSG_PIN(p.M); OSG_PIN(p.N); OSG_PIN(p.K);
    OSG_PIN(p.splits); OSG_PIN(p.k_per_split); OSG_PIN(p.a_bytes); OSG_PIN(p.b_bytes); OSG_PIN(p.mt); OSG_PIN(p.nt); OSG_PIN(p.n_major); OSG_PIN(p.grid);
    if constexpr (CONV) {
        OSG_PIN(p.H); OSG_PIN(p.W); OSG_PIN(p.Cin); OSG_PIN(p.Ho); OSG_PIN(p.Wo); OSG_PIN(p.KW); OSG_PIN(p.sh); OSG_PIN(p.sw); OSG_PIN(p.pt); OSG_PIN(p.pl);
    }
    OSG_PIN(p.bias); OSG_PIN(p.residual); OSG_PIN(p.rowbias); OSG_PIN(p.rb_ld); OSG_PIN(p.strideC); OSG_PIN(p.ln_c1); OSG_PIN(p.rs_in); OSG_PIN(p.rb_rows);
    OSG_PIN(p.bias_f32); OSG_PIN(p.act); OSG_PIN(p.no_epre); OSG_PIN(p.rs_np);
    if constexpr (WQ) { OSG_PIN(p.wq_sc); OSG_PIN(p.wq_zp); OSG_PIN(p.w_zp); }
#endif
    static_assert(KS == 1 || (KS == 2 && !SPEC && MODE == 0 && LN != 1), "KS = 2: plain kernel only (row statistics come from the producer, LN = 2, or not at all)");
    static_assert(WGN == 1 || WGN == 2, "wave grid: 2 x 2 or 4 x 1");
    static_assert(!WQ || LN == 0, "W8: no folded LayerNorm");
    constexpr int ROWB = 128;
    constexpr int ROWB_B = WQ ? 64 : 128;
    constexpr int BRW = WQ ? 16 : 8;
    constexpr int BNP = (BN + 4 * BRW - 1) / (4 * BRW) * (4 * BRW);
    constexpr int A_BYTES = BM * ROWB, B_BYTES = BNP * ROWB_B, GSTAGE = A_BYTES + B_BYTES, STAGE = KS * GSTAGE;
    constexpr int A_LD = BM / 32, B_LD = BNP / (4 * BRW);
    constexpr int WM = BM / (4 / WGN), WN = BN / WGN, TM = WM / 16, TN = WN / 16;
    static_assert(BM % 32 == 0 && WM % 16 == 0 && WN % 16 == 0, "a wave's part of the tile is made of whole 16 x 16 blocks");
    constexpr int INFLIGHT = (NST - 2) * (A_LD + B_LD);
    constexpr unsigned OOB = 0x80000000u;
    static_assert(INFLIGHT <= 63, "vmcnt is a 6-bit counter");

    extern __shared__ __attribute__((aligned(16))) char smem2[];
    typedef __attribute__((address_space(3))) void* lds_ptr;

    kdbg_stamp(p, 0);
    const int tid = threadIdx.x;
    const int lane = tid & 63;
    const int wave8 = __builtin_amdgcn_readfirstlane(tid >> 6);
    const bool loader = SPEC && wave8 >= 4, math = !SPEC || wave8 < 4;
    const bool loads = !SPEC || loader;
    const int wave = wave8 & 3;
    const int grp = KS == 2 ? (wave8 >> 2) : 0;
    const int wm0 = (WGN == 2 ? (wave >> 1) : wave) * WM;
    const int wn0 = (WGN == 2 ? (wave & 1) : 0) * WN;

    const int total = p.grid;
    int L;
    {
        const int bid = blockIdx.x, x = bid & 7, i = bid >> 3, q = total >> 3, r = total & 7;
        L = (x < r ? x * (q + 1) : r * (q + 1) + (x - r) * q) + i;
    }
    const int per_batch = p.mt * p.nt * p.splits;
    int zb, m_tile, n_tile, zs;
    {
        zb = L / (per_batch);
        int rem = L - zb * per_batch;
        if (p.n_major) {
            n_tile = rem / (p.splits * p.mt); rem -= n_tile * p.splits * p.mt;
            zs = rem / (p.mt); m_tile = rem - zs * p.mt;
        } else {
            m_tile = rem / (p.splits * p.nt); rem -= m_tile * p.splits * p.nt;
            zs = rem / (p.nt); n_tile = rem - zs * p.nt;
        }
    }
    const int m0 = m_tile * BM, n0 = n_tile * BN;
    const int kbeg = zs * p.k_per_split;
    const int kend = min(p.K, kbeg + p.k_per_split);
    const int nkt = (kend - kbeg) >> 6;
    const int nsteps = (nkt + KS - 1) / KS;

    __amdgpu_buffer_rsrc_t rsA = __builtin_amdgcn_make_buffer_rsrc((void*)(p.A + (long)zb * p.strideA), 0, p.a_bytes, 0x00020000);
    __amdgpu_buffer_rsrc_t rsB = __builtin_amdgcn_make_buffer_rsrc((void*)(p.Bt + (long)zb * p.strideB), 0, p.b_bytes, 0x00020000);

    const int rsub = lane >> 3;
    const int gch = (lane & 7) ^ rsub;
    int a_base[A_LD];
    int a_hi0[A_LD], a_wi0[A_LD];
#pragma unroll
    for (int j = 0; j < A_LD; j++) {
        const int m = m0 + (j * 4 + wave) * 8 + rsub;
        if (CONV) {
            const int mm = m < p.M ? m : 0;
            const int hw = p.Ho * p.Wo;
            const int n_img = mm / hw;
            const int r2 = mm - n_img * hw;
            const int ho = r2 / p.Wo, wo = r2 - ho * p.Wo;
            a_hi0[j] = m < p.M ? ho * p.sh - p.pt : -0x40000000;
            a_wi0[j] = wo * p.sw - p.pl;
            a_base[j] = (((n_img * p.H + (ho * p.sh - p.pt)) * p.W + (wo * p.sw - p.pl)) * p.Cin + gch * 8) * 2;
        } else {
            a_base[j] = m < p.M ? (int)(((long)m * p.lda + gch * 8) * 2) : (int)OOB;
            a_hi0[j] = a_wi0[j] = 0;
        }
    }
    int b_base[B_LD];
#pragma unroll
    for (int j = 0; j < B_LD; j++) {
        if constexpr (WQ) {
            const int nl = (j * 4 + wave) * 16 + (lane >> 2), n = n0 + nl;
            b_base[j] = (n < p.N && (BNP == BN || nl < BN)) ? (int)((long)n * p.K + (((lane & 3) ^ ((lane >> 4) & 3)) << 4)) : (int)OOB;
        } else {
            const int nl = (j * 4 + wave) * 8 + rsub, n = n0 + nl;
            b_base[j] = (n < p.N && (BNP == BN || nl < BN)) ? (int)(((long)n * p.K + gch * 8) * 2) : (int)OOB;
        }
    }

    int ik = kbeg + 64 * grp, i_c0 = 0, i_kh = 0, i_kw = 0;
    if (CONV) {
        const int cell = ik / p.Cin;
        i_c0 = ik - cell * p.Cin;
        i_kh = cell / p.KW;
        i_kw = cell - i_kh * p.KW;
    }
    auto issue_tile = [&](int stage) {
        char* As = smem2 + stage * STAGE + grp * GSTAGE;
        char* Bs = As + A_BYTES;
        const bool live = ik < kend;
        const unsigned kill = live ? 0u : OOB;
        if (CONV) {
            const int tap_off = ((i_kh * p.W + i_kw) * p.Cin + i_c0) * 2;
#pragma unroll
            for (int j = 0; j < A_LD; j++) {
                const int hi = a_hi0[j] + i_kh, wi = a_wi0[j] + i_kw;
                const bool ok = live && (unsigned)hi < (unsigned)p.H && (unsigned)wi < (unsigned)p.W;
                const unsigned off = ok ? (unsigned)(a_base[j] + tap_off) : OOB;
                __builtin_amdgcn_raw_ptr_buffer_load_lds(rsA, (lds_ptr)(As + (j * 4 + wave) * 1024), 16, off, 0, 0, 0);
            }
#pragma unroll
            for (int adv = 0; adv < KS; adv++) {
                i_c0 += 64;
                if (i_c0 >= p.Cin) { i_c0 = 0; if (++i_kw == p.KW) { i_kw = 0; ++i_kh; } }
            }
        } else {
#pragma unroll
            for (int j = 0; j < A_LD; j++)
                __builtin_amdgcn_raw_ptr_buffer_load_lds(rsA, (lds_ptr)(As + (j * 4 + wave) * 1024), 16, (unsigned)a_base[j] | kill, ik * 2, 0, 0);
        }
#pragma unroll
        for (int j = 0; j < B_LD; j++)
            __builtin_amdgcn_raw_ptr_buffer_load_lds(rsB, (lds_ptr)(Bs + (j * 4 + wave) * 1024), 16, (unsigned)b_base[j] | kill, WQ ? ik : ik * 2, 0, 0);
        ik += 64 * KS;
    };

    f32x4 acc[TM][TN];
#pragma unroll
    for (int i = 0; i < TM; i++)
#pragma unroll
        for (int j = 0; j < TN; j++) acc[i][j] = f32x4{0.f, 0.f, 0.f, 0.f};

    const int frow = lane & 15;
    const int fsw = (((lane >> 4) ^ (frow & 7)) << 4);
    const int a_rd = (wm0 + frow) * ROWB + fsw;
    const int b_rd = WQ ? A_BYTES + (wn0 + frow) * ROWB_B + ((((lane >> 5) & 1) ^ ((frow >> 2) & 3)) << 4) + ((lane >> 4) & 1) * 8 : A_BYTES + (wn0 + frow) * ROWB + fsw;

    f32x4 pst[LN == 2 ? NCH : 1];
    if constexpr (LN == 2) {
        const int m = min(m0 + wm0 + (lane & 15) + 16 * ((lane >> 4) % TM), p.M - 1);
        const float* src = p.rs_in + (long)m * p.rs_np * 2;
        const int nch = p.rs_np >> 1;
#pragma unroll
        for (int c = 0; c < NCH; c++)
            pst[c] = *reinterpret_cast<const f32x4*>(src + 4 * min(c, nch - 1));
        asm volatile("" ::: "memory");
    }

    constexpr bool EPRE = TM * TN <= 8;
    W8Ops<WQ ? TN : 1, true> w8;
    if constexpr (WQ) { if (math) w8_prefetch<TN, true>(p, w8, n0, wn0, lane); }
    EpiOps<TM, TN, CONV, EPRE> epre;
    epre.have = false;
    if (math && !p.ln_c1 && grp == 0) epi_prefetch<TM, TN, CONV, EPRE>(p, epre, m0, n0, wm0, wn0, lane, zb);
    if (loads) {
#pragma unroll
        for (int s2 = 0; s2 < NST - 1; s2++) issue_tile(s2);
    }
    kdbg_stamp(p, 1);
    if constexpr (WQ) { if (math) w8_finalize<TN, true>(w8); }

    float ls[TM], lq[TM];
#pragma unroll
    for (int i = 0; i < TM; i++) ls[i] = lq[i] = 0.f;

    int cur = 0, nxt = NST - 1;
    for (int kt = 0; kt < nsteps; kt++) {
        if (loads) asm volatile("s_waitcnt vmcnt(%0)" ::"n"(INFLIGHT) : "memory");
        __builtin_amdgcn_s_barrier();
        if (kt == 0) kdbg_stamp(p, 2);
        if (loads) issue_tile(nxt);
        const char* St = smem2 + cur * STAGE + grp * GSTAGE;
        if (math)
#pragma unroll
        for (int ks = 0; ks < (MODE == 1 ? 0 : 2); ks++) {
            f16x8 a[TM], b[TN];
#pragma unroll
            for (int i = 0; i < TM; i++) a[i] = *reinterpret_cast<const f16x8*>(St + ((a_rd + i * 16 * ROWB) ^ (ks << 6)));
#pragma unroll
            for (int j = 0; j < TN; j++) {
                if constexpr (WQ) b[j] = w8_frag(*reinterpret_cast<const u32x2v*>(St + ((b_rd + j * 16 * ROWB_B) ^ (ks << 5))), w8.zz[j]);
                else b[j] = *reinterpret_cast<const f16x8*>(St + ((b_rd + j * 16 * ROWB) ^ (ks << 6)));
            }
#pragma unroll
            for (int i = 0; i < TM; i++)
#pragma unroll
                for (int j = 0; j < TN; j++) acc[i][j] = __builtin_amdgcn_mfma_f32_16x16x32_f16(b[j], a[i], acc[i][j], 0, 0, 0);
            if constexpr (LN == 1) ln_accumulate<TM>(a, ls, lq);
        }
        cur = cur + 1 == NST ? 0 : cur + 1;
        nxt = nxt + 1 == NST ? 0 : nxt + 1;
    }
    kdbg_stamp(p, 3);
    asm volatile("s_waitcnt vmcnt(0)" ::: "memory");
    if (loader) return;
    if constexpr (WQ) w8_scale_acc<TM, TN>(w8, acc);
    if constexpr (KS == 2) {
        __builtin_amdgcn_s_barrier();
        f32x4* red = reinterpret_cast<f32x4*>(smem2) + (wave * (TM * TN + 1)) * 64 + lane;
        if (grp == 1) {
#pragma unroll
            for (int i = 0; i < TM; i++)
#pragma unroll
                for (int j = 0; j < TN; j++) red[(i * TN + j) * 64] = acc[i][j];
        }
        asm volatile("s_waitcnt lgkmcnt(0)" ::: "memory");
        __builtin_amdgcn_s_barrier();
        if (grp == 1) return;
#pragma unroll
        for (int i = 0; i < TM; i++)
#pragma unroll
            for (int j = 0; j < TN; j++) acc[i][j] += red[(i * TN + j) * 64];
    }
    if constexpr (LN == 2) {
        const int nch = p.rs_np >> 1;
        float S = 0.f, Q = 0.f;
#pragma unroll
        for (int c = 0; c < NCH; c++) {
            asm volatile("" : "+v"(pst[c]));
            if (c < nch) { S += pst[c][0] + pst[c][2]; Q += pst[c][1] + pst[c][3]; }
        }
#pragma unroll
        for (int i = 0; i < TM; i++) {
            ls[i] = __shfl(S, (lane & 15) + 16 * i, 64);
            lq[i] = __shfl(Q, (lane & 15) + 16 * i, 64);
        }
    }
    if constexpr (LN != 0) ln_apply<TM, TN, LN == 1>(p, acc, ls, lq, n0, wn0, lane);
    if (OSG_UNLIKELY_IF(!SPEC, p.act == OSG_ACT_GEGLU)) {
        if constexpr (TN % 2 == 0) gemm_epilogue_geglu<TM, TN>(p, acc, m0, n0, wm0, wn0, lane, zb);
        return;
    }
    kdbg_stamp(p, 4);
    float* stat_lds = nullptr;
    if (OSG_UNLIKELY_IF(!SPEC, p.sink[0].table || p.sink[1].table)) {
        __builtin_amdgcn_s_barrier();
        stat_lds = reinterpret_cast<float*>(smem2) + wave * (WN * 2);
    }
    if constexpr (KS == 1 && !SPEC && LN == 0 && MODE == 0) {
        if (OSG_UNLIKELY_IF(!SPEC, p.splits > 1 && p.fold_acc)) {
            if (!splitk_fold_acc<TM, TN>(p, acc, (zb * p.mt + m_tile) * p.nt + n_tile, zs, reinterpret_cast<int*>(smem2), tid)) return;
            EpiOps<TM, TN, CONV, false> none;
            none.have = false;
            gemm_epilogue_fast<TM, TN, CONV, false>(p, acc, m0, n0, wm0, wn0, lane, zb, none, nullptr);
            return;
        }
    }
    gemm_epilogue<TM, TN, CONV, EPRE, !SPEC>(p, acc, m0, n0, wm0, wn0, lane, zb, zb * p.splits + zs, epre, stat_lds);
    kdbg_stamp(p, 5);
    if (OSG_UNLIKELY_IF(!SPEC, p.kdbg != nullptr)) { asm volatile("s_waitcnt vmcnt(0)" ::: "memory"); kdbg_stamp(p, 6); }
}

template <int BM, int BN, int NST, bool CONV, int MODE = 0, int SPEC = 0, int LN = 0, int NCH = 5, int KS = 1, int WGN = 2, int WQ = 0>
int launch_v2(osg_ctx* ctx, GemmParams& p, int batch) {
    constexpr size_t smem = WQ ? (size_t)NST * KS * (BM * 128 + (BN + 63) / 64 * 64 * 64) : (size_t)NST * KS * (BM + (BN + 31) / 32 * 32) * 128;
    static_assert(smem <= 160 * 1024, "LDS budget");
    static_assert(KS == 1 || (size_t)4 * ((BM / 32) * (BN / 32) + 1) * 1024 <= smem, "KS = 2: the accumulator hand-over must fit the ring");
    auto kern = gemm2_kernel<BM, BN, NST, CONV, MODE, SPEC, LN, NCH, KS, WGN, WQ>;
    static unsigned long long attr_mask = 0;
    if (osg_first_on_device(attr_mask)) {
        OSG_HIP(ctx, hipFuncSetAttribute((const void*)kern, hipFuncAttributeMaxDynamicSharedMemorySize, (int)smem));
    }
    p.mt = (p.M + BM - 1) / BM;
    p.nt = (p.N + BN - 1) / BN;
    dim3 grid((unsigned)(p.mt * p.nt * batch * p.splits));
    p.grid = (int)grid.x;
    p.no_epre = osg_mm::no_epi_prefetch();
    p.kdbg = kdbg_buffer(ctx, grid.x);
    const osg_mm::StatSink sinks_in[2] = {p.sink[0], p.sink[1]};
    if (p.sink[0].table || p.sink[1].table) {
        const bool ok = !ctx->tuning && p.splits == 1 && batch == 1 && MODE == 0 && LN == 0 && !SPEC && p.act != OSG_ACT_GEGLU && (p.N & 3) == 0 && ((p.ldc | p.ldc2) & 3) == 0 &&
                        p.sink_hw > 0 && p.sink_hw % BM == 0 && p.M % p.sink_hw == 0;
        if (ok) { ctx->sink_fused = true; p.sink_imgs = p.M / p.sink_hw; p.sink_per_xcd = ctx->xcd_ids8 ? 1 : 0; }
        else p.sink[0].table = p.sink[1].table = nullptr;
    }
    hipLaunchKernelGGL(kern, grid, dim3((SPEC || KS == 2) ? 512 : 256), smem, ctx->compute, p);
    p.sink[0] = sinks_in[0]; p.sink[1] = sinks_in[1];
    OSG_LAUNCH_CHECK(ctx);
    return 0;
}

using V2Launch = int (*)(osg_ctx*, GemmParams&, int);
template <int UNIT, int I>
constexpr V2Launch v2_launcher() {
    constexpr V2Entry e = kV2Entries[I];
    if constexpr (v2_unit(e) == UNIT) return launch_v2<e.bm, e.bn, e.nst, e.conv != 0, 0, e.spec, e.ln, e.nch, e.ks, e.wgn, e.wq>;
    else return nullptr;
}
template <int UNIT, size_t... I>
constexpr std::array<V2Launch, kV2Count> v2_launchers(std::index_sequence<I...>) { return {v2_launcher<UNIT, (int)I>()...}; }
template <int UNIT>
int launch_v2_in_unit(int entry, osg_ctx* ctx, GemmParams& p, int batch) {
    static constexpr std::array<V2Launch, kV2Count> table = v2_launchers<UNIT>(std::make_index_sequence<kV2Count>{});
    return table[entry](ctx, p, batch);
}

}
```

onnxstream_amd/csrc/osg_gemm_common.h:

```cpp
#pragma once
#include <utility>
#include <vector>
#include "osg_common.h"
#include "osg_gemm_routes.h"

#include <algorithm>
#include <type_traits>
#ifndef OSG_EPI_STORE_AUX
#define OSG_EPI_STORE_AUX 0
#endif
namespace osg_mm {

struct StatSink {
    long long* table;
    int groups, cpg, ch_off;
};
constexpr int kStatCopies = 8;
constexpr float kStatSX = 1048576.f;
__host__ __device__ inline int stat_q_shift(long elems) {
    int lg = 0;
    while ((1L << lg) < elems) lg++;
    const int e = 36 - lg;
    return e < 10 ? 10 : (e > 20 ? 20 : e);
}
__host__ __device__ inline float stat_q_scale(long elems) { return (float)(1L << stat_q_shift(elems)); }

struct GemmParams {
    const f16* A;
    const f16* Bt;
    long long* kdbg;
    long lda;
    long strideA, strideB;
    int M, N, K;
    int splits, k_per_split;
    unsigned a_bytes, b_bytes;
    int mt, nt, n_major;
    int grid;
    int H, W, Cin, Ho, Wo, KW, sh, sw, pt, pl;
    const void* bias;
    const f16* residual;
    const f16* rowbias;
    long rb_ld;
    long strideC;
    const float* ln_c1;
    const float* rs_in;
    int rb_rows;
    int bias_f32, act;
    int no_epre;
    int rs_np;
    unsigned rb_bytes;
    f16* C;
    float* partial;
    long a_bytes_l;
    int* tickets;
    int* xcd_err;
    float w_scale;
    int w_zp;
    const float* wq_sc;
    const float* wq_zp;
    int w8;
    float ln_eps;
    float* rs_out;
    long ldc;
    f16* C2;
    long ldc2;
    StatSink sink[2];
    int sink_hw;
    int sink_imgs, sink_per_xcd;
    int fold_acc;
};
#define OSG_PIN(x) asm volatile("" ::"s"(x))
#define OSG_LIKELY(x) __builtin_expect(!!(x), 1)
#define OSG_UNLIKELY(x) __builtin_expect(!!(x), 0)
#define OSG_UNLIKELY_IF(h, x) ((h) ? __builtin_expect(!!(x), 0) : !!(x))

typedef unsigned int u32x2v __attribute__((ext_vector_type(2)));
typedef _Float16 f16x2w __attribute__((ext_vector_type(2)));
__device__ __forceinline__ f16x8 w8_frag(u32x2v c, f16x2w zz) {
    union { unsigned u; f16x2w h; } d0, d1, d2, d3;
    d0.u = __builtin_amdgcn_perm(0x64646464u, c[0], 0x04010400u);
    d1.u = __builtin_amdgcn_perm(0x64646464u, c[0], 0x04030402u);
    d2.u = __builtin_amdgcn_perm(0x64646464u, c[1], 0x04010400u);
    d3.u = __builtin_amdgcn_perm(0x64646464u, c[1], 0x04030402u);
    d0.h -= zz; d1.h -= zz; d2.h -= zz; d3.h -= zz;
    return f16x8{d0.h[0], d0.h[1], d1.h[0], d1.h[1], d2.h[0], d2.h[1], d3.h[0], d3.h[1]};
}
template <int TN, bool SC = true>
struct W8Ops {
    float zraw[TN];
    f16x2w zz[TN];
    f32x4 sc[SC ? TN : 1];
};
template <int TN, bool SC>
__device__ __forceinline__ void w8_prefetch(const GemmParams& p, W8Ops<TN, SC>& w, int n0, int wn0, int lane) {
    if (p.wq_sc) {
#pragma unroll
        for (int j = 0; j < TN; j++) {
            w.zraw[j] = p.wq_zp[min(n0 + wn0 + j * 16 + (lane & 15), p.N - 1)];
            if constexpr (SC) w.sc[j] = *reinterpret_cast<const f32x4*>(p.wq_sc + min(n0 + wn0 + j * 16 + (lane >> 4) * 4, p.N - 4));
        }
    } else {
#pragma unroll
        for (int j = 0; j < TN; j++) {
            w.zraw[j] = (float)p.w_zp;
            if constexpr (SC) w.sc[j] = f32x4{p.w_scale, p.w_scale, p.w_scale, p.w_scale};
        }
    }
    asm volatile("" ::: "memory");
}
template <int TN, bool SC>
__device__ __forceinline__ void w8_finalize(W8Ops<TN, SC>& w) {
#pragma unroll
    for (int j = 0; j < TN; j++) {
        const f16 h = (f16)(1024.0f + w.zraw[j]);
        w.zz[j] = f16x2w{h, h};
    }
}
template <int TM, int TN>
__device__ __forceinline__ void w8_scale_acc(const W8Ops<TN, true>& w, f32x4 (&acc)[TM][TN]) {
#pragma unroll
    for (int i = 0; i < TM; i++)
#pragma unroll
        for (int j = 0; j < TN; j++) acc[i][j] *= w.sc[j];
}
template <int TM, int TN>
__device__ __forceinline__ void w8_scale_acc_late(const GemmParams& p, f32x4 (&acc)[TM][TN], int n0, int wn0, int lane) {
#pragma unroll
    for (int j = 0; j < TN; j++) {
        f32x4 s = {p.w_scale, p.w_scale, p.w_scale, p.w_scale};
        if (p.wq_sc) s = *reinterpret_cast<const f32x4*>(p.wq_sc + min(n0 + wn0 + j * 16 + (lane >> 4) * 4, p.N - 4));
#pragma unroll
        for (int i = 0; i < TM; i++) acc[i][j] *= s;
    }
}

__device__ __forceinline__ void kdbg_stamp(const GemmParams& p, int slot) {
    if (__builtin_expect(p.kdbg != nullptr, 0) && threadIdx.x == 0) p.kdbg[(long)blockIdx.x * 8 + slot] = wall_clock64();
}

typedef _Float16 f16x2v __attribute__((ext_vector_type(2)));
template <int TM>
__device__ __forceinline__ void ln_accumulate(const f16x8 (&a)[TM], float (&ls)[TM], float (&lq)[TM]) {
    const f16x2v ones = {(f16)1.0f, (f16)1.0f};
#pragma unroll
    for (int i = 0; i < TM; i++)
#pragma unroll
        for (int e = 0; e < 4; e++) {
            const f16x2v pr = {a[i][2 * e], a[i][2 * e + 1]};
            ls[i] = __builtin_amdgcn_fdot2(pr, ones, ls[i], false);
            lq[i] = __builtin_amdgcn_fdot2(pr, pr, lq[i], false);
        }
}
template <int TM, int TN, bool PARTIAL>
__device__ __forceinline__ void ln_apply(const GemmParams& p, f32x4 (&acc)[TM][TN], float (&ls)[TM], float (&lq)[TM], int n0, int wn0, int lane) {
#pragma unroll
    for (int i = 0; i < TM; i++) {
        float s = ls[i], q = lq[i];
        if (PARTIAL) {
            s += __shfl_xor(s, 16, 64); q += __shfl_xor(q, 16, 64);
            s += __shfl_xor(s, 32, 64); q += __shfl_xor(q, 32, 64);
        }
        const double ik = (double)(1.0f / (float)p.K);
        const double mean_d = (double)s * ik;
        const float var = fmaxf((float)((double)q * ik - mean_d * mean_d), 0.f);
        const float mean = (float)mean_d;
        const float rstd = 1.0f / sqrtf(var + p.ln_eps);
#pragma unroll
        for (int j = 0; j < TN; j++) {
            const int n = n0 + wn0 + j * 16 + (lane >> 4) * 4;
            f32x4 c = {0.f, 0.f, 0.f, 0.f};
            if (n < p.N) c = *reinterpret_cast<const f32x4*>(p.ln_c1 + n);
#pragma unroll
            for (int r = 0; r < 4; r++) acc[i][j][r] = rstd * (acc[i][j][r] - mean * c[r]);
        }
    }
}

template <int TM, int TN, bool RB = true, bool ON = true>
struct EpiOps {
    bool have;
    f32x4 bias32[ON ? TN : 1];
    f16x4 bias16[ON ? TN : 1];
    f16x4 rb[ON && RB ? TM : 1][ON && RB ? TN : 1];
    f16x4 res[ON ? TM : 1][ON ? TN : 1];
};
template <int TM, int TN, bool RB, bool ON>
__device__ __forceinline__ void epi_prefetch(const GemmParams& p, EpiOps<TM, TN, RB, ON>& e, int m0, int n0, int wm0, int wn0, int lane, int zb) {
    const int N = p.N;
    e.have = ON && !p.no_epre && p.splits == 1 && (N & 3) == 0 && p.act != OSG_ACT_GEGLU && N >= 4 && (RB || !p.rowbias);
    if constexpr (!ON) return;
    if (__builtin_expect(!e.have, 0)) return;
    const f16* __restrict__ R = p.residual ? p.residual + zb * p.strideC : nullptr;
#pragma unroll
    for (int j = 0; j < TN; j++) {
        const int n = min(n0 + wn0 + j * 16 + (lane >> 4) * 4, N - 4);
        if (p.bias) {
            if (p.bias_f32) e.bias32[j] = *reinterpret_cast<const f32x4*>((const float*)p.bias + n);
            else e.bias16[j] = *reinterpret_cast<const f16x4*>((const f16*)p.bias + n);
        }
    }
#pragma unroll
    for (int i = 0; i < TM; i++) {
        const int m = min(m0 + wm0 + i * 16 + (lane & 15), p.M - 1);
#pragma unroll
        for (int j = 0; j < TN; j++) {
            const int n = min(n0 + wn0 + j * 16 + (lane >> 4) * 4, N - 4);
            if constexpr (RB) {
                if (p.rowbias) e.rb[i][j] = *reinterpret_cast<const f16x4*>(p.rowbias + (long)(m / p.rb_rows) * p.rb_ld + n);
            }
            if (R) e.res[i][j] = *reinterpret_cast<const f16x4*>(R + (long)m * N + n);
        }
    }
    asm volatile("" ::: "memory");
}

__device__ __forceinline__ void stat_add(int per_xcd, unsigned long long* table, long copy_stride, long cell, float S, float Q, float qscale) {
    const unsigned long long vs = (unsigned long long)__float2ll_rn(S * kStatSX), vq = (unsigned long long)__float2ll_rn(Q * qscale);
    if (per_xcd) {
        unsigned xcc;
        asm volatile("s_getreg_b32 %0, hwreg(HW_REG_XCC_ID)" : "=s"(xcc));
        unsigned long long* c = table + (long)(xcc & 7u) * copy_stride + cell;
        __hip_atomic_fetch_add(c, vs, __ATOMIC_RELAXED, __HIP_MEMORY_SCOPE_WORKGROUP);
        __hip_atomic_fetch_add(c + 1, vq, __ATOMIC_RELAXED, __HIP_MEMORY_SCOPE_WORKGROUP);
// ... 556 lines not shown
```

onnxstream_amd/csrc/osg_tchain.hip:

```cpp
#include "osg_common.h"

#include <cstdlib>
#include <type_traits>

namespace osg_tb {

struct TailParams {
    const f16 *a1, *x0;
    const f16 *wo1, *bo1;
    const f16 *g2, *be2;
    float eps2;
    const f16 *wq2, *bq2;
    const f16 *kp, *vtp;
    float sc_log2e;
    int Tk;
    const f16 *wo2, *bo2;
    const f16 *g3, *be3;
    float eps3;
    const f16 *w1, *b1, *w2, *b2;
    const f16 *wpo, *bpo, *xin;
    f16 *out, *out2;
    long ldo, ldo2;
    int M, rows_per_img, heads;
    int pf_sleep0, pf_sleep;
// ... 124 lines not shown
    for (int j = 0; j < NT; j++) {
        const int n = nb + j * 16 + g4;
        const f16x4 bv = *reinterpret_cast<const f16x4*>(bias + n * 2);
#pragma unroll
        for (int i = 0; i < RT; i++) {
            const int m = i * 16 + l16;
            f16x4 rv = rg[i][j];
            if constexpr (RES_LDS) rv = *reinterpret_cast<const f16x4*>(res_lds + img_off<RT>(m, n));
            f16x4 o;
#pragma unroll
            for (int r = 0; r < 4; r++) o[r] = (f16)((acc[i][j][r] + (float)bv[r]) + (float)rv[r]);
            *reinterpret_cast<f16x4*>(out + (row0 + m) * ldo + n) = o;
            if constexpr (OUT2) *reinterpret_cast<f16x4*>(out2 + (row0 + m) * ldo2 + n) = o;
        }
    }
}

template <int RT, int C>
__device__ __forceinline__ void ln_rows(const char* X, char* P, const char* gamma, const char* beta, float eps, int tid) {
    constexpr int NCH = C / 8, LPR = 16 / RT, PER = NCH / LPR;
    static_assert(NCH % LPR == 0 && (LPR == 4 || LPR == 8), "row chunks split over the lanes of a row");
    const int row = tid / LPR, part = tid % LPR;
    float v[PER][8];
    float s = 0.f;
#pragma unroll
    for (int i = 0; i < PER; i++) {
        const int c = part + LPR * i;
        const f16x8 t = *reinterpret_cast<const f16x8*>(X + (c >> 3) * kTileBytes<RT> + row * 128 + (((c & 7) ^ (row & 7)) << 4));
#pragma unroll
        for (int e = 0; e < 8; e++) { v[i][e] = (float)t[e]; s += v[i][e]; }
    }
    s += __shfl_xor(s, 1, 64);
    s += __shfl_xor(s, 2, 64);
    if constexpr (LPR == 8) s += __shfl_xor(s, 4, 64);
    const float mean = s / (float)C;
    float q = 0.f;
#pragma unroll
    for (int i = 0; i < PER; i++)
#pragma unroll
        for (int e = 0; e < 8; e++) { const float d = v[i][e] - mean; q += d * d; }
    q += __shfl_xor(q, 1, 64);
    q += __shfl_xor(q, 2, 64);
    if constexpr (LPR == 8) q += __shfl_xor(q, 4, 64);
    const float rstd = 1.0f / sqrtf(q / (float)C + eps);
#pragma unroll
    for (int i = 0; i < PER; i++) {
        const int c = part + LPR * i;
        const f16x8 gm = *reinterpret_cast<const f16x8*>(gamma + c * 16);
        const f16x8 bt = *reinterpret_cast<const f16x8*>(beta + c * 16);
        f16x8 o;
#pragma unroll
        for (int e = 0; e < 8; e++) o[e] = (f16)((v[i][e] - mean) * rstd * (float)gm[e] + (float)bt[e]);
        *reinterpret_cast<f16x8*>(P + (c >> 3) * kTileBytes<RT> + row * 128 + (((c & 7) ^ (row & 7)) << 4)) = o;
    }
}

template <int RT, int C>
__device__ __forceinline__ void dump_img(const char* img, f16* __restrict__ dst, long row0, int tid) {
    if (!dst) return;
    constexpr int NCH = C / 8;
    for (int idx = tid; idx < 16 * RT * NCH; idx += 256) {
        const int row = idx / NCH, c = idx - row * NCH;
        *reinterpret_cast<f16x8*>(dst + (row0 + row) * C + c * 8) =
            *reinterpret_cast<const f16x8*>(img + (c >> 3) * kTileBytes<RT> + row * 128 + (((c & 7) ^ (row & 7)) << 4));
    }
}

template <int RT, int D, int TKT>
__device__ __forceinline__ void cross_attention(const char* Qi, char* Oi, const f16* __restrict__ kp, const f16* __restrict__ vtp, int head0, int nheads, float c, int Tk, int lane) {
    constexpr int DS = (D + 15) / 16, DP = DS * 16, TKP = TKT * 16;
    const int l16 = lane & 15, g = lane >> 4;
    for (int hh = 0; hh < nheads; hh++) {
        const int h = head0 + hh;
        const f16* kh = kp + (long)h * TKP * DP;
        const f16* vh = vtp + (long)h * DP * TKP;
        f16x4 kf[TKT][DS], vf[DS][TKT];
#pragma unroll
        for (int tt = 0; tt < TKT; tt++)
#pragma unroll
            for (int ds = 0; ds < DS; ds++) kf[tt][ds] = *reinterpret_cast<const f16x4*>(kh + (tt * 16 + l16) * DP + ds * 16 + g * 4);
#pragma unroll
        for (int dt = 0; dt < DS; dt++)
#pragma unroll
            for (int tt = 0; tt < TKT; tt++) vf[dt][tt] = *reinterpret_cast<const f16x4*>(vh + (dt * 16 + l16) * TKP + tt * 16 + g * 4);
#pragma unroll 1
        for (int mi = 0; mi < RT; mi++) {
            const int m = mi * 16 + l16;
            f16x4 qf[DS];
#pragma unroll
            for (int ds = 0; ds < DS; ds++) {
                const int dd = ds * 16 + g * 4;
                const bool ok = dd < D;
                const f16x4 t = *reinterpret_cast<const f16x4*>(Qi + img_off<RT>(m, h * D + (ok ? dd : 0)));
                qf[ds] = ok ? t : f16x4{0, 0, 0, 0};
            }
            f32x4 s[TKT];
#pragma unroll
            for (int tt = 0; tt < TKT; tt++) {
                s[tt] = f32x4{0.f, 0.f, 0.f, 0.f};
#pragma unroll
                for (int ds = 0; ds < DS; ds++) s[tt] = __builtin_amdgcn_mfma_f32_16x16x16f16(kf[tt][ds], qf[ds], s[tt], 0, 0, 0);
            }
            float mx = -INFINITY;
#pragma unroll
            for (int tt = 0; tt < TKT; tt++)
#pragma unroll
                for (int r = 0; r < 4; r++) {
                    const float v = (tt * 16 + g * 4 + r) < Tk ? s[tt][r] * c : -INFINITY;
                    s[tt][r] = v;
                    mx = fmaxf(mx, v);
                }
            mx = fmaxf(mx, __shfl_xor(mx, 16, 64));
            mx = fmaxf(mx, __shfl_xor(mx, 32, 64));
            float sum = 0.f;
            f16x4 pf[TKT];
#pragma unroll
            for (int tt = 0; tt < TKT; tt++)
#pragma unroll
                for (int r = 0; r < 4; r++) {
                    const float e = __builtin_amdgcn_exp2f(s[tt][r] - mx);
                    sum += e;
                    pf[tt][r] = (f16)e;
                }
            sum += __shfl_xor(sum, 16, 64);
            sum += __shfl_xor(sum, 32, 64);
            const float inv = 1.0f / sum;
#pragma unroll
            for (int dt = 0; dt < DS; dt++) {
                f32x4 o = f32x4{0.f, 0.f, 0.f, 0.f};
#pragma unroll
                for (int tt = 0; tt < TKT; tt++) o = __builtin_amdgcn_mfma_f32_16x16x16f16(vf[dt][tt], pf[tt], o, 0, 0, 0);
                const int dd = dt * 16 + g * 4;
                if (dd < D) {
                    f16x4 ov;
#pragma unroll
                    for (int r = 0; r < 4; r++) ov[r] = (f16)(o[r] * inv);
                    *reinterpret_cast<f16x4*>(Oi + img_off<RT>(m, h * D + dd)) = ov;
                }
            }
        }
    }
}

__device__ __forceinline__ void touch_lines(const void* base, int rows, int row_bytes, long pitch, int tid, char* lds_dummy) {
    const int lpr = (row_bytes + 127) >> 7, n = rows * lpr;
    __amdgpu_buffer_rsrc_t rs = __builtin_amdgcn_make_buffer_rsrc((void*)base, 0, (int)((rows - 1) * pitch + row_bytes), 0x00020000);
    for (int i = tid; i < n; i += 256) {
        const int r = i / lpr, l = i - r * lpr;
        __builtin_amdgcn_raw_ptr_buffer_load_lds(rs, (lds_ptr)lds_dummy, 4, (unsigned)(r * pitch + l * 128), 0, 0, 0);
    }
}

template <int RT, int C, int D, int TKT, int NS>
__global__ __launch_bounds__(256, RT == 2 && NS == 2 ? 2 : 1) void tblock_tail_kernel(TailParams p) {
    constexpr int RB = 16 * RT;
    constexpr int TB = kTileBytes<RT>;
    constexpr int KT = C / 64;
    constexpr int NTW = C / 64;
    constexpr int F = 4 * C;
    constexpr int HC = 128, NCHUNK = F / HC;
    constexpr int G2T = HC / 64;
    constexpr int PER = KT + G2T;
    constexpr int IMG = KT * TB;
    constexpr int AH = NS - 1;
    static_assert(C % 64 == 0 && NTW <= 5 && 2 * G2T * TB <= IMG && (RT == 2 || RT == 4) && (NS == 2 || NS == 3) && PER % NS == 1 && AH <= G2T && AH <= KT, "shape");
    constexpr int KS_C = 4 * C * 16, KT_C = 8 * C * 16, KS_1 = 4 * 2 * F * 16, KT_1 = 8 * 2 * F * 16;
    constexpr int GATE = F * 16;
    constexpr int CH1 = HC * 16;
    constexpr int CH2 = (HC / 8) * C * 16;
    const int tid = threadIdx.x;
    const int nblk = p.M / RB;

    if ((int)blockIdx.x >= nblk) {
        extern __shared__ __attribute__((aligned(16))) char lds_pf[];
        char* dummy = lds_pf + __builtin_amdgcn_readfirstlane(tid >> 6) * 256;
        auto nap = [&](int n) __attribute__((always_inline)) { for (; n > 0; n -= 127) __builtin_amdgcn_s_sleep(127); };
        touch_lines(p.wq2, 1, C * C * 2, 0, tid, dummy);
        {
            constexpr int DP = (D + 15) / 16 * 16;
            const int imgs = p.M / p.rows_per_img, bytes = imgs * p.heads * TKT * 16 * DP * 2;
            touch_lines(p.kp, 1, bytes, 0, tid, dummy);
            touch_lines(p.vtp, 1, bytes, 0, tid, dummy);
        }
        touch_lines(p.wo2, 1, C * C * 2, 0, tid, dummy);
        nap(p.pf_sleep0);
        for (int c = 0; c < NCHUNK; c++) {
            touch_lines((const char*)p.w1 + c * CH1, C / 8, HC * 16, 2 * F * 16, tid, dummy);
            touch_lines((const char*)p.w1 + GATE + c * CH1, C / 8, HC * 16, 2 * F * 16, tid, dummy);
            touch_lines((const char*)p.w2 + c * CH2, 1, CH2, 0, tid, dummy);
            if (c == NCHUNK / 2 && p.wpo) touch_lines(p.wpo, 1, C * C * 2, 0, tid, dummy);
            nap(p.pf_sleep);
        }
        return;
    }

    extern __shared__ __attribute__((aligned(16))) char lds[];
    char* const X = lds;
    char* const P = lds + IMG;
    char* const R = lds + 2 * IMG;
    char* const VEC = lds + 3 * IMG;
    enum { V_BO1, V_G2, V_BE2, V_BQ2, V_BO2, V_G3, V_BE3, V_B2, V_BPO, V_B1 };
    auto vec = [&](int k) __attribute__((always_inline)) { return VEC + k * (C * 2); };
    {
        const f16* src[10] = {p.bo1, p.g2, p.be2, p.bq2, p.bo2, p.g3, p.be3, p.b2, p.bpo, p.b1};
#pragma unroll
        for (int k = 0; k < 10; k++) {
            const int n16 = (k == V_B1 ? 2 * F : C) / 8;
            for (int i = tid; i < n16; i += 256) {
                f16x8 v = f16x8{0, 0, 0, 0, 0, 0, 0, 0};
                if (src[k]) v = *reinterpret_cast<const f16x8*>(src[k] + i * 8);
                *reinterpret_cast<f16x8*>(vec(k) + i * 16) = v;
            }
        }
    }
    const int lane = tid & 63;
    const int wave = __builtin_amdgcn_readfirstlane(tid >> 6);
    const int l16 = lane & 15, g = lane >> 4;
    const long row0 = (long)blockIdx.x * RB;
    const int img = (int)(row0 / p.rows_per_img);
    const int a_rd = l16 * 128 + ((g ^ (l16 & 7)) << 4);
    const int nb = wave * (C / 4);
    long long* const stamps = reinterpret_cast<long long*>(p.dbg[7]);
    auto stamp = [&](int k) __attribute__((always_inline)) { if (stamps && tid == 0) stamps[(long)blockIdx.x * 32 + k] = wall_clock64(); };
    stamp(0);

    f16x8 bq[NS][10];
    f16x8 bs[KT][10];
    const unsigned lo_c = (unsigned)((g * C + nb + l16) * 16);
    const unsigned lo_1 = (unsigned)((g * 2 * F + wave * 32 + l16) * 16);
    const __amdgpu_buffer_rsrc_t u_o1 = __builtin_amdgcn_make_buffer_rsrc((void*)p.wo1, 0, C * C * 2, 0x00020000);
    const __amdgpu_buffer_rsrc_t u_q2 = __builtin_amdgcn_make_buffer_rsrc((void*)p.wq2, 0, C * C * 2, 0x00020000);
    const __amdgpu_buffer_rsrc_t u_o2 = __builtin_amdgcn_make_buffer_rsrc((void*)p.wo2, 0, C * C * 2, 0x00020000);
    const __amdgpu_buffer_rsrc_t u_1 = __builtin_amdgcn_make_buffer_rsrc((void*)p.w1, 0, 2 * F * C * 2, 0x00020000);
    const __amdgpu_buffer_rsrc_t u_2 = __builtin_amdgcn_make_buffer_rsrc((void*)p.w2, 0, C * F * 2, 0x00020000);
    const __amdgpu_buffer_rsrc_t u_po = __builtin_amdgcn_make_buffer_rsrc((void*)p.wpo, 0, p.wpo ? C * C * 2 : 0, 0x00020000);
    const bool has_po = p.wpo != nullptr;
    auto ld_cc = [&](f16x8 (&b)[10], __amdgpu_buffer_rsrc_t rs, int t) __attribute__((always_inline)) { load_b<NTW>(b, rs, lo_c, t * KT_C, KS_C); };
    auto ld_ff = [&](f16x8 (&b)[10], int cc, int pos) __attribute__((always_inline)) {
        if (pos < KT) load_b_geglu(b, u_1, lo_1, cc * CH1 + pos * KT_1, KS_1, GATE);
        else load_b<NTW>(b, u_2, lo_c, (cc - 1) * CH2 + (pos - KT) * KT_C, KS_C);
    };

    static_for<KT>([&](auto tc) __attribute__((always_inline)) { ld_cc(bs[decltype(tc)::value], u_o1, decltype(tc)::value); });

    {
        __amdgpu_buffer_rsrc_t rsA = __builtin_amdgcn_make_buffer_rsrc((void*)(p.a1 + row0 * C), 0, RB * C * 2, 0x00020000);
        __amdgpu_buffer_rsrc_t rsX = __builtin_amdgcn_make_buffer_rsrc((void*)(p.x0 + row0 * C), 0, RB * C * 2, 0x00020000);
        const int rsub = lane >> 3, gch = (lane & 7) ^ rsub;
#pragma unroll
        for (int kt = 0; kt < KT; kt++)
#pragma unroll
            for (int qq = 0; qq < RT / 2; qq++) {
                const int q8 = qq * 4 + wave;
                const unsigned off = (unsigned)(((q8 * 8 + rsub) * C + kt * 64 + gch * 8) * 2);
                __builtin_amdgcn_raw_ptr_buffer_load_lds(rsA, (lds_ptr)(P + kt * TB + q8 * 1024), 16, off, 0, 0, 0);
                __builtin_amdgcn_raw_ptr_buffer_load_lds(rsX, (lds_ptr)(X + kt * TB + q8 * 1024), 16, off, 0, 0, 0);
            }
    }
    asm volatile("s_waitcnt vmcnt(0)" ::: "memory");
    lds_barrier();
    stamp(1);

    {
        f32x4 acc[RT][NTW];
        zero_acc(acc);
        square_stage<RT, KT, NTW>(P, a_rd, bs, acc, [&](f16x8 (&)[10], int t) __attribute__((always_inline)) { if (t < AH) ld_cc(bq[t % NS], u_q2, t); },
                              [&](int t) __attribute__((always_inline)) { stamp(16 + t); });
        stamp(21);
        epi_to_lds<RT, NTW, true>(acc, vec(V_BO1), nb, X, X, lane);
        stamp(22);
    }
    lds_barrier();
    stamp(2);
    dump_img<RT, C>(X, p.dbg[0], row0, tid);
    ln_rows<RT, C>(X, P, vec(V_G2), vec(V_BE2), p.eps2, tid);
    lds_barrier();
    stamp(3);
    dump_img<RT, C>(P, p.dbg[1], row0, tid);

    {
        f32x4 acc[RT][NTW];
        zero_acc(acc);
        gemm_stage<RT, KT, NTW, 0, NS>(P, a_rd, bq, acc, [&](f16x8 (&b)[10], int t) __attribute__((always_inline)) { ld_cc(b, u_q2, t); },
                                   [&](f16x8 (&b)[10], int j) __attribute__((always_inline)) { ld_cc(b, u_o2, j); });
        epi_to_lds<RT, NTW, false>(acc, vec(V_BQ2), nb, nullptr, R, lane);
    }
    lds_barrier();
    stamp(4);
    dump_img<RT, C>(R, p.dbg[2], row0, tid);

    {
        constexpr int DS = (D + 15) / 16, DP = DS * 16, TKP = TKT * 16;
        const int hpw = p.heads >> 2;
        const long per_img = (long)p.heads * TKP * DP;
        cross_attention<RT, D, TKT>(R, P, p.kp + img * per_img, p.vtp + img * per_img, wave * hpw, hpw, p.sc_log2e, p.Tk, lane);
    }
    lds_barrier();
    stamp(5);
    dump_img<RT, C>(P, p.dbg[3], row0, tid);

    {
        f32x4 acc[RT][NTW];
        zero_acc(acc);
        gemm_stage<RT, KT, NTW, KT, NS>(P, a_rd, bq, acc, [&](f16x8 (&b)[10], int t) __attribute__((always_inline)) { ld_cc(b, u_o2, t); },
                                    [&](f16x8 (&b)[10], int j) __attribute__((always_inline)) { ld_ff(b, 0, j); });
        epi_to_lds<RT, NTW, true>(acc, vec(V_BO2), nb, X, X, lane);
    }
// ... 66 lines not shown
        int c = 1;
        for (; c + NS <= NCHUNK; c += NS) {
            ff_iter(std::integral_constant<int, B0 % NS>{}, c);
            ff_iter(std::integral_constant<int, (B0 + 1) % NS>{}, c + 1);
            if constexpr (NS == 3) ff_iter(std::integral_constant<int, (B0 + 2) % NS>{}, c + 2);
        }
        constexpr int REM = (NCHUNK - 1) % NS;
        if constexpr (REM >= 1) ff_iter(std::integral_constant<int, B0 % NS>{}, c);
        if constexpr (REM >= 2) ff_iter(std::integral_constant<int, (B0 + 1) % NS>{}, c + 1);
        stamp(9);
        {
            constexpr int ST = (S0 + KT + (NCHUNK - 1) * PER) % NS;
            const char* Hp = R + ((NCHUNK - 1) & 1) * (G2T * TB);
            static_for<G2T>([&](auto uc) __attribute__((always_inline)) {
                constexpr int u = decltype(uc)::value;
                if constexpr (u + AH < G2T) ld_ff(bq[(ST + u + AH) % NS], NCHUNK, KT + u + AH);
                else if (has_po) ld_cc(bq[(ST + u + AH) % NS], u_po, u + AH - G2T);
                __builtin_amdgcn_sched_barrier(0);
                mma_ktile<RT, NTW>(Hp + u * TB, a_rd, bq[(ST + u) % NS], accY);
                __builtin_amdgcn_sched_barrier(0);
            });
        }
    }
    stamp(10);
    f16x4 rg[RT][NTW];
#pragma unroll
    for (int i = 0; i < RT; i++)
#pragma unroll
        for (int j = 0; j < NTW; j++) rg[i][j] = f16x4{0, 0, 0, 0};
    if (!has_po) {
        if (p.out2) epi_to_global<RT, NTW, true, true>(accY, vec(V_B2), nb, X, rg, p.out, p.ldo, p.out2, p.ldo2, row0, lane);
        else epi_to_global<RT, NTW, true, false>(accY, vec(V_B2), nb, X, rg, p.out, p.ldo, nullptr, 0, row0, lane);
        if (stamps) { asm volatile("s_waitcnt vmcnt(0)" ::: "memory"); stamp(13); }
        return;
    }
#pragma unroll
    for (int i = 0; i < RT; i++)
#pragma unroll
        for (int j = 0; j < NTW; j++) rg[i][j] = *reinterpret_cast<const f16x4*>(p.xin + (row0 + i * 16 + l16) * C + nb + j * 16 + g * 4);
    epi_to_lds<RT, NTW, true>(accY, vec(V_B2), nb, X, P, lane);
    lds_barrier();
    stamp(11);
    dump_img<RT, C>(P, p.dbg[6], row0, tid);
    {
        f32x4 acc[RT][NTW];
        zero_acc(acc);
        constexpr int SS = 2 * KT + KT + (NCHUNK - 1) * PER + G2T;
        gemm_stage<RT, KT, NTW, SS, NS>(P, a_rd, bq, acc, [&](f16x8 (&b)[10], int t) __attribute__((always_inline)) { ld_cc(b, u_po, t); },
                                    [&](f16x8 (&)[10], int) __attribute__((always_inline)) {});
        stamp(12);
        if (p.out2) epi_to_global<RT, NTW, false, true>(acc, vec(V_BPO), nb, nullptr, rg, p.out, p.ldo, p.out2, p.ldo2, row0, lane);
        else epi_to_global<RT, NTW, false, false>(acc, vec(V_BPO), nb, nullptr, rg, p.out, p.ldo, nullptr, 0, row0, lane);
        if (stamps) { asm volatile("s_waitcnt vmcnt(0)" ::: "memory"); stamp(13); }
    }
}

struct PackJob { int k_col, v_col, D, dst; };
__global__ __launch_bounds__(256) void kv_pack_kernel(const f16* __restrict__ base, long ld, int Tk, int heads, int imgs, const PackJob* __restrict__ jobs, f16* __restrict__ dst) {
    const int per_job = imgs * heads;
    const int j = blockIdx.x / per_job, ih = blockIdx.x - j * per_job, img = ih / heads, h = ih - img * heads;
    const PackJob job = jobs[j];
    const int D = job.D, DP = (D + 15) / 16 * 16, TKP = 80, NC = DP / 8;
    f16* kp = dst + job.dst + (long)ih * TKP * DP;
    f16* vtp = dst + job.dst + (long)per_job * TKP * DP + (long)ih * TKP * DP;
    const f16* k = base + job.k_col + h * D + (long)img * Tk * ld;
    const f16* v = base + job.v_col + h * D + (long)img * Tk * ld;
    for (int idx = threadIdx.x; idx < TKP * NC; idx += 256) {
        const int t = idx / NC, d0 = (idx - t * NC) * 8;
        const bool in = t < Tk && d0 < D;
        f16x8 kv = f16x8{0, 0, 0, 0, 0, 0, 0, 0}, vv = kv;
        if (in) {
            kv = *reinterpret_cast<const f16x8*>(k + (long)t * ld + d0);
            vv = *reinterpret_cast<const f16x8*>(v + (long)t * ld + d0);
        }
        *reinterpret_cast<f16x8*>(kp + t * DP + d0) = kv;
#pragma unroll
        for (int e = 0; e < 8; e++) vtp[(d0 + e) * TKP + t] = vv[e];
    }
}

__global__ __launch_bounds__(256) void kn8_pack_kernel(const f16x8* __restrict__ src, f16x8* __restrict__ dst, int N, int K8) {
    const long idx = (long)blockIdx.x * 256 + threadIdx.x;
    if (idx >= (long)N * K8) return;
    const int kc = (int)(idx / N), n = (int)(idx - (long)kc * N);
    dst[idx] = src[(long)n * K8 + kc];
}


}

extern "C" {

int osg_tblock_tail_supported(int M, int rows_per_img, int C, int heads, int Tk) {
    return C == 320 && heads == 8 && M > 0 && M % 32 == 0 && rows_per_img % 32 == 0 && Tk >= 1 && Tk <= 80;
}

size_t osg_tblock_kv_pack_elems(int imgs, int heads, int D) { return (size_t)imgs * heads * 80 * (size_t)((D + 15) / 16 * 16); }

int osg_tblock_pack_weight(osg_ctx* ctx, const void* w_nk, int N, int K, void* w_kn8) {
    if (N < 1 || K < 8 || K % 8) OSG_FAIL(ctx, "osg_tblock_pack_weight: K must be a multiple of 8");
    const long n = (long)N * (K / 8);
    hipLaunchKernelGGL(osg_tb::kn8_pack_kernel, dim3((unsigned)((n + 255) / 256)), dim3(256), 0, ctx->compute, (const f16x8*)w_nk, (f16x8*)w_kn8, N, K / 8);
    OSG_LAUNCH_CHECK(ctx);
    return 0;
}

int osg_tblock_kv_pack_jobs(osg_ctx* ctx, const void* base, long ld, int imgs, int Tk, int heads, int njobs, const int* jobs_dev, void* dst) {
    if (Tk < 1 || Tk > 80 || njobs < 1 || imgs < 1 || heads < 1 || ld % 8) OSG_FAIL(ctx, "osg_tblock_kv_pack_jobs: unsupported shape (1 <= Tk <= 80, row pitch a multiple of 8 elements; columns and head dims multiples of 8)");
    hipLaunchKernelGGL(osg_tb::kv_pack_kernel, dim3((unsigned)(njobs * imgs * heads)), dim3(256), 0, ctx->compute, (const f16*)base, ld, Tk, heads, imgs,
                       (const osg_tb::PackJob*)jobs_dev, (f16*)dst);
    OSG_LAUNCH_CHECK(ctx);
    return 0;
}

int osg_tblock_tail(osg_ctx* ctx, const osg_tblock_tail_args* a) {
    if (!osg_tblock_tail_supported(a->M, a->rows_per_img, a->C, a->heads, a->Tk)) OSG_FAIL(ctx, "osg_tblock_tail: unsupported shape (see osg_tblock_tail_supported)");
    if (!(a->scale > 0.f)) OSG_FAIL(ctx, "osg_tblock_tail: scale must be > 0");
    if (!a->a1 || !a->x0 || !a->wo1 || !a->g2 || !a->be2 || !a->wq2 || !a->kp || !a->vtp || !a->wo2 || !a->g3 || !a->be3 || !a->w1 || !a->w2 || !a->out)
        OSG_FAIL(ctx, "osg_tblock_tail: missing operand");
    if (a->wpo && !a->xin) OSG_FAIL(ctx, "osg_tblock_tail: proj_out needs its residual");
    osg_tb::TailParams p;
    p.a1 = (const f16*)a->a1; p.x0 = (const f16*)a->x0;
    p.wo1 = (const f16*)a->wo1; p.bo1 = (const f16*)a->bo1;
    p.g2 = (const f16*)a->g2; p.be2 = (const f16*)a->be2; p.eps2 = a->eps2;
    p.wq2 = (const f16*)a->wq2; p.bq2 = (const f16*)a->bq2;
    p.kp = (const f16*)a->kp; p.vtp = (const f16*)a->vtp;
    p.sc_log2e = a->scale * 1.4426950408889634f;
    p.Tk = a->Tk;
    p.wo2 = (const f16*)a->wo2; p.bo2 = (const f16*)a->bo2;
    p.g3 = (const f16*)a->g3; p.be3 = (const f16*)a->be3; p.eps3 = a->eps3;
    p.w1 = (const f16*)a->w1; p.b1 = (const f16*)a->b1; p.w2 = (const f16*)a->w2; p.b2 = (const f16*)a->b2;
    p.wpo = (const f16*)a->wpo; p.bpo = (const f16*)a->bpo; p.xin = (const f16*)a->xin;
    p.out = (f16*)a->out; p.out2 = (f16*)a->out2;
    p.ldo = a->ldo ? a->ldo : a->C; p.ldo2 = a->ldo2;
    p.M = a->M; p.rows_per_img = a->rows_per_img; p.heads = a->heads;
    for (int i = 0; i < 8; i++) p.dbg[i] = (f16*)a->dbg[i];
    static const int pfw = getenv("OSG_TBLOCK_PREFETCH") ? atoi(getenv("OSG_TBLOCK_PREFETCH")) : 8;
    static const int pfs0 = getenv("OSG_TBLOCK_PF_SLEEP0") ? atoi(getenv("OSG_TBLOCK_PF_SLEEP0")) : 100;
    static const int pfs = getenv("OSG_TBLOCK_PF_SLEEP") ? atoi(getenv("OSG_TBLOCK_PF_SLEEP")) : 60;
    p.pf_sleep0 = pfs0; p.pf_sleep = pfs;
    static const int rows_env = getenv("OSG_TBLOCK_ROWS") ? atoi(getenv("OSG_TBLOCK_ROWS")) : 0;
    int rows = a->rows_per_block == 32 || a->rows_per_block == 64 ? a->rows_per_block : rows_env == 32 || rows_env == 64 ? rows_env : (a->M / 64 < 2 * ctx->num_cu ? 32 : 64);
    if (a->rows_per_block != 0 && a->rows_per_block != 32 && a->rows_per_block != 64) OSG_FAIL(ctx, "osg_tblock_tail: rows_per_block must be 0, 32 or 64");
    if (a->M % 64 || a->rows_per_img % 64) {
        if (a->rows_per_block == 64) OSG_FAIL(ctx, "osg_tblock_tail: 64-row blocks need M and rows_per_img to be multiples of 64");
        rows = 32;
    }
    const int nblk = a->M / rows;
    const int npf = nblk >= 64 && nblk + pfw <= ctx->num_cu ? pfw : 0;
    auto launch = [&](auto kern, int smem, unsigned long long& attr_mask) -> int {
        if (osg_first_on_device(attr_mask)) {
            OSG_HIP(ctx, hipFuncSetAttribute((const void*)kern, hipFuncAttributeMaxDynamicSharedMemorySize, smem));
        }
        hipLaunchKernelGGL(kern, dim3((unsigned)(nblk + npf)), dim3(256), smem, ctx->compute, p);
        return 0;
    };
    constexpr int vec_bytes = (9 * 320 + 8 * 320) * 2;
    static unsigned long long attr64 = 0, attr32 = 0, attr32n3 = 0;
    static const bool ns3 = getenv("OSG_TBLOCK_NS") && atoi(getenv("OSG_TBLOCK_NS")) == 3;
    int rc;
    if (rows == 64) rc = launch(osg_tb::tblock_tail_kernel<4, 320, 40, 5, 2>, 3 * 5 * osg_tb::kTileBytes<4> + vec_bytes, attr64);
    else if (ns3) rc = launch(osg_tb::tblock_tail_kernel<2, 320, 40, 5, 3>, 3 * 5 * osg_tb::kTileBytes<2> + vec_bytes, attr32n3);
    else rc = launch(osg_tb::tblock_tail_kernel<2, 320, 40, 5, 2>, 3 * 5 * osg_tb::kTileBytes<2> + vec_bytes, attr32);
    if (rc) return rc;
    OSG_LAUNCH_CHECK(ctx);
    return 0;
}

}
```

onnxstream_amd/osgpu.py:

```python
from __future__ import annotations

import ctypes
import os
from typing import Optional, Sequence

import numpy as np

_HERE = os.path.dirname(os.path.abspath(__file__))
LIB_PATH = os.environ.get("OSGPU_LIB") or os.path.join(_HERE, "libosgpu.so")

U8, F16, F32, I64 = 1, 2, 3, 4
_NP2DT = {np.dtype(np.uint8): U8, np.dtype(np.float16): F16, np.dtype(np.float32): F32, np.dtype(np.int64): I64}
ACT_NONE, ACT_SILU, ACT_SIGMOID = 0, 1, 2
UN = dict(sigmoid=0, erf=1, sqrt=2, sin=3, cos=4, neg=5, pow=6, silu=7, gelu_erf=8)
BIN = dict(add=0, sub=1, mul=2, div=3)

EXPORTS = [
    "osg_device_count", "osg_init", "osg_destroy", "osg_last_error", "osg_device_name", "osg_stream", "osg_set_autotune", "osg_tune_misses",
    "osg_malloc", "osg_free", "osg_upload", "osg_upload_sync", "osg_host_register", "osg_host_unregister", "osg_upload_pinned", "osg_upload_pinned_async", "osg_copy_fence", "osg_download", "osg_copy", "osg_memset", "osg_sync",
    "osg_graph_begin", "osg_graph_end", "osg_graph_launch", "osg_graph_destroy", "osg_timer_start", "osg_timer_stop",
    "osg_conv2d_nhwc", "osg_conv2d_nhwc_rb", "osg_conv2d_nhwc_v", "osg_gemm", "osg_gemm_ln", "osg_gemm_rowstats", "osg_last_route", "osg_last_kernel", "osg_gemm_w8", "osg_conv2d_nhwc_w8", "osg_gemm_w8_v", "osg_conv2d_nhwc_w8_v", "osg_transpose_kn_to_nk", "osg_attention", "osg_attention_strided", "osg_sdpa", "osg_rms_norm", "osg_rope",
    "osg_instance_norm", "osg_group_norm_nhwc", "osg_layer_norm", "osg_reduce_mean_last", "osg_softmax_last",
    "osg_unary", "osg_binary", "osg_geglu", "osg_transpose", "osg_copy_2d", "osg_concat2", "osg_resize_nearest", "osg_gather_rows",
    "osg_maxpool_nhwc", "osg_convert", "osg_sampler_prepare", "osg_sampler_cfg_euler_a", "osg_sampler_cfg_multistep", "osg_sampler_prepare_rescale",
    "osg_decode_gather", "osg_decode_blend",
    "osg_range_push", "osg_range_pop", "osg_marker_record", "osg_copy_wait_marker", "osg_timer_mark", "osg_timer_between", "osg_set_stat_sinks", "osg_group_norm_stats_nhwc", "osg_qu8_conv2d_nhwc", "osg_qu8_conv2d_nhwc_t", "osg_qu8_conv_tap_sums", "osg_qu8_gemm", "osg_qu8_lut", "osg_qu8_binary", "osg_qu8_instance_norm", "osg_qu8_instance_norm_nhwc", "osg_qu8_affine_act", "osg_qu8_norm_affine_act_nhwc", "osg_qu8_softmax_last", "osg_kdbg_read",
    "osg_tblock_tail_supported", "osg_tblock_tail", "osg_tblock_kv_pack_elems", "osg_tblock_kv_pack_jobs", "osg_tblock_pack_weight", 
]


class OsgError(RuntimeError):
    pass


class TBlockTailArgs(ctypes.Structure):
    _vp, _cf, _ci, _cl = ctypes.c_void_p, ctypes.c_float, ctypes.c_int, ctypes.c_long
    _fields_ = [("a1", _vp), ("x0", _vp), ("wo1", _vp), ("bo1", _vp), ("g2", _vp), ("be2", _vp), ("eps2", _cf), ("wq2", _vp), ("bq2", _vp),
                ("kp", _vp), ("vtp", _vp), ("scale", _cf), ("Tk", _ci), ("wo2", _vp), ("bo2", _vp), ("g3", _vp), ("be3", _vp), ("eps3", _cf),
                ("w1", _vp), ("b1", _vp), ("w2", _vp), ("b2", _vp), ("wpo", _vp), ("bpo", _vp), ("xin", _vp), ("out", _vp), ("out2", _vp),
                ("ldo", _cl), ("ldo2", _cl), ("M", _ci), ("rows_per_img", _ci), ("C", _ci), ("heads", _ci), ("dbg", _vp * 8), ("rows_per_block", _ci)]


def load_library(path: str = LIB_PATH) -> ctypes.CDLL:
    if not os.path.exists(path):
        raise OsgError(f"{path} not found: build it with `python -m onnxstream_amd.build` (hipcc, gfx950)")
    lib = ctypes.CDLL(path)
    vp, ci, cl, cf = ctypes.c_void_p, ctypes.c_int, ctypes.c_long, ctypes.c_float
    lib.osg_init.argtypes = [ci, ctypes.POINTER(vp)]
    lib.osg_destroy.argtypes = [vp]
    lib.osg_destroy.restype = None
    lib.osg_last_error.argtypes = [vp]
    lib.osg_last_error.restype = ctypes.c_char_p
    lib.osg_device_name.argtypes = [vp]
    lib.osg_device_name.restype = ctypes.c_char_p
    lib.osg_stream.argtypes = [vp]
    lib.osg_stream.restype = vp
    lib.osg_malloc.argtypes = [vp, ctypes.c_size_t, ctypes.POINTER(vp)]
    lib.osg_free.argtypes = [vp, vp]
    lib.osg_host_register.argtypes = [vp, vp, ctypes.c_size_t]
    lib.osg_host_unregister.argtypes = [vp, vp]
    for f in ("osg_upload", "osg_upload_sync", "osg_upload_pinned", "osg_upload_pinned_async", "osg_download", "osg_copy"):
        getattr(lib, f).argtypes = [vp, vp, vp, ctypes.c_size_t]
    lib.osg_memset.argtypes = [vp, vp, ci, ctypes.c_size_t]
    lib.osg_sync.argtypes = [vp]
    lib.osg_copy_fence.argtypes = [vp]
    lib.osg_graph_begin.argtypes = [vp]
    lib.osg_graph_end.argtypes = [vp, ctypes.POINTER(vp)]
    lib.osg_graph_launch.argtypes = [vp, vp]
    lib.osg_graph_destroy.argtypes = [vp]
    lib.osg_graph_destroy.restype = None
    lib.osg_timer_start.argtypes = [vp]
    lib.osg_timer_stop.argtypes = [vp, ctypes.POINTER(cf)]
    lib.osg_conv2d_nhwc.argtypes = [vp, ci, vp, vp, vp, ci, vp, vp] + [ci] * 14
    lib.osg_conv2d_nhwc_rb.argtypes = [vp, ci, vp, vp, vp, ci, vp, cl, vp, vp] + [ci] * 14
    lib.osg_conv2d_nhwc_v.argtypes = [vp, ci, vp, vp, vp, ci, vp, cl, vp, vp, cl, vp, cl] + [ci] * 14
    lib.osg_gemm_w8.argtypes = [vp, vp, vp, cf, ci, vp, ci, vp, vp, ci, ci, ci, ci]
    lib.osg_conv2d_nhwc_w8.argtypes = [vp, vp, vp, cf, ci, vp, ci, vp, cl, vp, vp] + [ci] * 14
    lib.osg_gemm_w8_v.argtypes = [vp, vp, vp, cf, ci, vp, vp, vp, ci, vp, vp, ci, ci, ci, ci]
    lib.osg_conv2d_nhwc_w8_v.argtypes = [vp, vp, vp, cf, ci, vp, vp, vp, ci, vp, cl, vp, vp, cl, vp, cl] + [ci] * 14
    lib.osg_gemm.argtypes = [vp, ci, vp, vp, ci, vp, ci, vp, vp, ci, ci, ci, ci, cl, cl, cl, ci]
    lib.osg_transpose_kn_to_nk.argtypes = [vp, ci, vp, vp, ci, ci]
    lib.osg_attention.argtypes = [vp, ci, vp, vp, vp, vp, ci, ci, ci, ci, cf, ci]
    lib.osg_attention_strided.argtypes = [vp, ci, vp, cl, cl, cl, vp, cl, cl, cl, vp, cl, cl, cl, vp, cl, cl, cl, ci, ci, ci, ci,
                                          ci, cf]
    lib.osg_sdpa.argtypes = [vp, ci, vp, vp, vp, vp, vp, ci, ci, ci, ci, ci, ci, cf]
    lib.osg_rms_norm.argtypes = [vp, ci, vp, vp, vp, cl, ci, cf]
    lib.osg_rope.argtypes = [vp, ci, vp, vp, vp, vp, cl, cl, ci]
    lib.osg_instance_norm.argtypes = [vp, ci, vp, vp, vp, vp, ci, cl, ci, cf]
    lib.osg_group_norm_nhwc.argtypes = [vp, ci, vp, vp, vp, vp, ci, cl, ci, ci, cf, ci]
    lib.osg_layer_norm.argtypes = [vp, ci, vp, vp, vp, vp, cl, ci, cf]
    lib.osg_reduce_mean_last.argtypes = [vp, ci, vp, vp, cl, cl]
    lib.osg_softmax_last.argtypes = [vp, ci, vp, vp, cl, cl]
    lib.osg_unary.argtypes = [vp, ci, ci, vp, vp, cl, cf]
    lib.osg_binary.argtypes = [vp, ci, ci, vp, ctypes.POINTER(cl), vp, ctypes.POINTER(cl), vp, ci]
    lib.osg_geglu.argtypes = [vp, ci, vp, vp, cl, cl]
    lib.osg_transpose.argtypes = [vp, ci, vp, vp, ci, ctypes.POINTER(cl), ctypes.POINTER(ci)]
    lib.osg_copy_2d.argtypes = [vp, ci, vp, cl, cl, vp, cl, cl, cl, cl]
    lib.osg_resize_nearest.argtypes = [vp, ci, vp, vp] + [ci] * 7
    lib.osg_gather_rows.argtypes = [vp, ci, vp, vp, vp, cl, cl, cl]
    lib.osg_maxpool_nhwc.argtypes = [vp, ci, vp, vp] + [ci] * 12
    lib.osg_convert.argtypes = [vp, ci, ci, vp, vp, cl, cf, ci]
    lib.osg_concat2.argtypes = [vp, ci, vp, cl, vp, cl, vp, cl]
    lib.osg_gemm_ln.argtypes = [vp, vp, vp, vp, vp, cf, vp, vp, vp, ci, ci, ci, ci]
    lib.osg_gemm_rowstats.argtypes = [vp, vp, vp, vp, ci, vp, vp, ci, ci, ci, ci, vp]
    lib.osg_last_route.argtypes = [vp, ctypes.POINTER(ci)]
    lib.osg_last_kernel.argtypes = [vp, ctypes.POINTER(ci)]
    lib.osg_sampler_prepare.argtypes = [vp, vp, vp, vp, ci, cl, cf, cf, cl]
    lib.osg_sampler_cfg_euler_a.argtypes = [vp, vp, vp, vp, ci, cl, cf, cf, cf, cf, cf, cf]
    lib.osg_sampler_cfg_multistep.argtypes = [vp, ci, vp, vp, vp, vp, vp, vp, ci, cl, cf, cf, cf, cf, cf, cf, cf, cf, ctypes.c_double, ctypes.c_double]
    lib.osg_sampler_prepare_rescale.argtypes = [vp, vp, vp, vp, ci, cl, cf, cf, cf, cl]
    lib.osg_decode_gather.argtypes = [vp, vp, vp, ci, ci, ci, ci, cf]
    lib.osg_decode_blend.argtypes = [vp, vp, vp, vp, ci, ci, ci, ci, ci]
    lib.osg_set_stat_sinks.argtypes = [vp, vp, ci, ci, ci, vp, ci, ci, ci, ci]
    lib.osg_group_norm_stats_nhwc.argtypes = [vp, vp, vp, vp, vp, ci, ctypes.c_long, ci, ci, cf, ci, vp]
    lib.osg_qu8_conv2d_nhwc.argtypes = [vp, vp, cf, ci, vp, cf, ci, vp, cf, ci, vp] + [ci] * 13
    lib.osg_qu8_conv2d_nhwc_t.argtypes = [vp, vp, cf, ci, vp, cf, ci, vp, cf, ci, vp] + [ci] * 13 + [vp]
    lib.osg_qu8_conv_tap_sums.argtypes = [vp, vp, ci, ci, ci, ci, vp]
    lib.osg_qu8_gemm.argtypes = [vp, vp, cl, cf, ci, vp, cf, ci, vp, cf, ci, vp, ci, ci, ci, ci, cl, cl, cl]
    lib.osg_qu8_lut.argtypes = [vp, vp, vp, cl, vp]
    lib.osg_qu8_binary.argtypes = [vp, ci, vp, ctypes.POINTER(cl), cf, ci, vp, ctypes.POINTER(cl), cf, ci, vp, cf, ci, ci]
    lib.osg_qu8_instance_norm.argtypes = [vp, vp, vp, ci, cl, ci, vp, vp, cf, cf, ci, cf, ci]
    lib.osg_qu8_affine_act.argtypes = [vp, vp, cf, ci, vp, cf, ci, cf, ci, vp, cf, ci, cf, ci, vp, cf, ci, cf, ci, vp, cl, ci, cl]
    lib.osg_qu8_instance_norm_nhwc.argtypes = [vp, vp, vp, cl, ci, ci, ci, vp, vp, cf, cf, ci, cf, ci]
    lib.osg_qu8_norm_affine_act_nhwc.argtypes = [vp, vp, cl, ci, ci, ci, vp, vp, cf, cf, ci, cf, ci, vp, cf, ci, cf, ci, vp, cf, ci, cf, ci, vp, cf, ci, cf, ci, vp]
    lib.osg_qu8_softmax_last.argtypes = [vp, vp, vp, cl, cl, vp]
    lib.osg_tblock_tail_supported.argtypes = [ci] * 5
    lib.osg_tblock_tail.argtypes = [vp, ctypes.POINTER(TBlockTailArgs)]
    lib.osg_tblock_kv_pack_elems.argtypes = [ci, ci, ci]
    lib.osg_tblock_kv_pack_elems.restype = ctypes.c_size_t
    lib.osg_tblock_kv_pack_jobs.argtypes = [vp, vp, cl, ci, ci, ci, ci, vp, vp]
    lib.osg_tblock_pack_weight.argtypes = [vp, vp, ci, ci, vp]
    return lib


class DevBuf:

    def __init__(self, gpu: "Gpu", shape, dtype):
        self.gpu = gpu
        self.shape = tuple(int(s) for s in shape)
        self.dtype = np.dtype(dtype)
        self.nbytes = int(np.prod(self.shape, dtype=np.int64)) * self.dtype.itemsize
        p = ctypes.c_void_p()
        gpu._ck(gpu.lib.osg_malloc(gpu.ctx, max(self.nbytes, 16), ctypes.byref(p)))
        self.ptr = p.value

    @property
    def size(self):
        return int(np.prod(self.shape, dtype=np.int64))

    def numpy(self) -> np.ndarray:
        out = np.empty(self.shape, self.dtype)
        if self.nbytes:
            self.gpu._ck(self.gpu.lib.osg_download(self.gpu.ctx, out.ctypes.data, self.ptr, self.nbytes))
        return out

    def read_rows(self, lo: int, hi: int) -> np.ndarray:
        row = self.shape[-1]
        assert 0 <= lo <= hi <= self.size // row, (lo, hi, self.shape)
        out = np.empty((hi - lo, row), self.dtype)
        if out.nbytes:
            self.gpu._ck(self.gpu.lib.osg_download(self.gpu.ctx, out.ctypes.data, self.ptr + lo * row * self.dtype.itemsize, out.nbytes))
        return out

    def view(self, offset: int, shape) -> "DevBuf":
        v = DevBuf.__new__(DevBuf)
        v.gpu, v.shape, v.dtype = self.gpu, tuple(int(s) for s in shape), self.dtype
        v.nbytes = int(np.prod(v.shape, dtype=np.int64)) * self.dtype.itemsize
        assert 0 <= offset and offset * self.dtype.itemsize + v.nbytes <= self.nbytes, (offset, shape, self.shape)
        v.ptr, v.base = self.ptr + offset * self.dtype.itemsize, self
        return v

    def free(self):
        if self.ptr and getattr(self, "base", None) is None:
            self.gpu.lib.osg_free(self.gpu.ctx, self.ptr)
        self.ptr = None

    def __del__(self):
        try:
            self.free()
        except Exception:
            pass


class Gpu:
    def __init__(self, device: int = 0, lib_path: str = LIB_PATH):
        self.lib = load_library(lib_path)
        if self.lib.osg_device_count() <= 0:
            raise OsgError("no HIP device visible: the osgpu backend has no CPU fallback")
        c = ctypes.c_void_p()
        rc = self.lib.osg_init(device, ctypes.byref(c))
        if rc:
            raise OsgError(f"osg_init failed with code {rc}")
        self.ctx = c

    def close(self):
        if self.ctx:
            self.lib.osg_destroy(self.ctx)
            self.ctx = None

    def _ck(self, rc):
        if rc:
            raise OsgError(self.lib.osg_last_error(self.ctx).decode())

    @property
    def name(self):
        return self.lib.osg_device_name(self.ctx).decode()

    def empty(self, shape, dtype=np.float16) -> DevBuf:
        b = DevBuf(self, shape, dtype)
        if b.nbytes:
            self.memset(b, 0xFF)
        return b

    def last_route(self):
        r = (ctypes.c_int * 5)()
        self._ck(self.lib.osg_last_route(self.ctx, r))
        return tuple(r)

    def last_kernel(self):
        r = (ctypes.c_int * 8)()
        self._ck(self.lib.osg_last_kernel(self.ctx, r))
        return tuple(r)

    def to_dev(self, arr: np.ndarray, staged: bool = False) -> DevBuf:
        arr = np.ascontiguousarray(arr)
        b = DevBuf(self, arr.shape, arr.dtype)
        if arr.nbytes:
            fn = self.lib.osg_upload if staged else self.lib.osg_upload_sync
            self._ck(fn(self.ctx, b.ptr, arr.ctypes.data, arr.nbytes))
        return b

    def sync(self):
        self._ck(self.lib.osg_sync(self.ctx))

    def memset(self, b: DevBuf, byte: int):
        self._ck(self.lib.osg_memset(self.ctx, b.ptr, byte, b.nbytes))

    def _out(self, out: Optional[DevBuf], shape, dtype) -> DevBuf:
        if out is None:
            return self.empty(shape, dtype)
        if out.size != int(np.prod(shape, dtype=np.int64)) or out.dtype != np.dtype(dtype):
            raise OsgError(f"out= holds {out.shape} {out.dtype}, the op writes {tuple(shape)} {np.dtype(dtype)}")
        return out

    def timer_start(self):
        self._ck(self.lib.osg_timer_start(self.ctx))

    def timer_stop(self) -> float:
        ms = ctypes.c_float()
        self._ck(self.lib.osg_timer_stop(self.ctx, ctypes.byref(ms)))
        return ms.value

    @staticmethod
    def _p(b: Optional[DevBuf]):
        return b.ptr if b is not None else None

    def conv2d_nhwc(self, x: DevBuf, w: DevBuf, bias: Optional[DevBuf], stride=1, pads=(1, 1, 1, 1), residual=None, act=ACT_NONE,
                    image_bias: Optional[DevBuf] = None):
        n, h, wd, cin = x.shape
# ... 384 lines not shown
```

Before: 9.880.

## Preload hot kernel arguments into SGPRs via leading scalar kernel parameters

Enables the AMDGPU kernarg preload compiler option (16 slots) and reorders GEMM, conv3x3, attention and transformer-tail kernel signatures so the hot scalars and pointers come first as separate arguments. Some fields are packed into bitfields (splits, n_major, debug and batch flags; heads and kv_div), and the kernels rebuild the parameter struct from them. Rarely used fields such as the debug pointer and batch strides are read only behind unlikely branches, and some epilogue pins are moved after the prologue tile loads. The aim is to cut kernel-start latency from scalar loads of the kernarg segment. In exchange it adds host-side range checks that fail launches whose strides exceed 32 bits, plus a no-preload build variant selected by an environment variable.

```diff
diff --git a/include/osgpu.h b/include/osgpu.h
--- a/include/osgpu.h
+++ b/include/osgpu.h
@@ -115,6 +115,9 @@
                       int M, int N, int K, osg_act act, float* rowstats);
 int osg_last_route(const osg_ctx* ctx, int out[5]);
 int osg_last_kernel(const osg_ctx* ctx, int out[8]);
+
+int osg_gemm_kernarg_check(osg_ctx* ctx, long lda, int splits);
+int osg_attention_kernarg_check(osg_ctx* ctx, long kv_stride, int heads, int kv_div);
 
 int osg_attention(osg_ctx* ctx, osg_dtype dtype, const void* q, const void* k, const void* v, void* o, int heads, int Tq, int Tkv,
                   int D, float scale, int k_is_dt);
diff --git a/onnxstream_amd/build.py b/onnxstream_amd/build.py
--- a/onnxstream_amd/build.py
+++ b/onnxstream_amd/build.py
@@ -13,6 +13,9 @@
 LIB_HOST = os.environ.get("OSA_LIB_HOST") or os.path.join(ROOT, "libonnxstream_amd.so")
 ORACLE_REF = os.path.join(REPO, "oracle", "_ref", "libonnxstream_ref.so")
 HIPCC = os.environ.get("HIPCC", "/opt/rocm/bin/hipcc")
+NO_PRELOAD = os.environ.get("OSG_NO_KERNARG_PRELOAD", "") not in ("", "0")
+PRELOAD_FLAGS = [] if NO_PRELOAD else ["-mllvm", "-amdgpu-kernarg-preload-count=16"]
+LIB_GPU_BUILT = os.path.join(ROOT, "libosgpu_nopreload.so") if NO_PRELOAD else LIB_GPU
 
 
 def _newer(target, deps):
@@ -33,14 +36,14 @@
 def build_gpu(force=False, verbose=False):
     srcs = sorted(glob.glob(os.path.join(CSRC, "osg_*.hip")))
     hdrs = sorted(glob.glob(os.path.join(CSRC, "*.h"))) + [os.path.join(INC, "osgpu.h")]
-    objdir = os.path.join(CSRC, "build")
+    objdir = os.path.join(CSRC, "build", "nopreload") if NO_PRELOAD else os.path.join(CSRC, "build")
     os.makedirs(objdir, exist_ok=True)
     objs, procs = [], []
     for s in srcs:
         o = os.path.join(objdir, os.path.basename(s)[:-4] + ".o")
         objs.append(o)
         if force or _newer(o, [s] + hdrs):
-            cmd = [HIPCC, "--offload-arch=gfx950", "-O3", "-std=c++17", "-fPIC", "-mllvm", "-amdgpu-mfma-vgpr-form", "-I" + INC, "-I" + CSRC, "-c", s, "-o", o]
+            cmd = [HIPCC, "--offload-arch=gfx950", "-O3", "-std=c++17", "-fPIC", "-mllvm", "-amdgpu-mfma-vgpr-form"] + PRELOAD_FLAGS + ["-I" + INC, "-I" + CSRC, "-c", s, "-o", o]
             procs.append((cmd, subprocess.Popen(cmd, stdout=subprocess.PIPE, stderr=subprocess.STDOUT, text=True)))
     for cmd, p in procs:
         out, _ = p.communicate()
@@ -49,9 +52,9 @@
             raise RuntimeError("build failed: " + " ".join(cmd))
         if verbose and out:
             print(out)
-    if force or procs or _newer(LIB_GPU, objs):
-        _run([HIPCC, "--offload-arch=gfx950", "-shared", "-fPIC", "-o", LIB_GPU] + objs)
-    return LIB_GPU
+    if force or procs or _newer(LIB_GPU_BUILT, objs):
+        _run([HIPCC, "--offload-arch=gfx950", "-shared", "-fPIC", "-o", LIB_GPU_BUILT] + objs)
+    return LIB_GPU_BUILT
 
 
 def build_host(force=False):
diff --git a/onnxstream_amd/csrc/osg_attention.hip b/onnxstream_amd/csrc/osg_attention.hip
--- a/onnxstream_amd/csrc/osg_attention.hip
+++ b/onnxstream_amd/csrc/osg_attention.hip
@@ -254,10 +254,12 @@
 }
 
 template <int D, int QT, int NST>
-__global__ __launch_bounds__(256) void attn2_kernel(AttnParams pk, int nqb) {
-    const AttnParams p = pk;
-    osg_pin_all(p.q, p.k, p.v, p.o, p.q_tok, p.q_head, p.q_batch, p.k_tok, p.k_head, p.k_batch, p.v_tok, p.v_head, p.v_batch, p.o_tok, p.o_head, p.o_batch, p.heads, p.Tq, p.Tkv,
-                p.scale_log2e, p.mask, p.inv_scale, p.kv_div, nqb, (int)gridDim.x);
+__global__ __launch_bounds__(256) void attn2_kernel(const void* k, const void* v, int k_tok, int k_head, int k_batch, int v_tok, int v_head, int v_batch, int Tkv, int nqb, int grid,
+                                                    unsigned heads_kvdiv, AttnParams pk) {
+    AttnParams p = pk;
+    p.k = (const f16*)k; p.v = (const f16*)v; p.k_tok = k_tok; p.k_head = k_head; p.k_batch = k_batch; p.v_tok = v_tok; p.v_head = v_head; p.v_batch = v_batch; p.Tkv = Tkv;
+    p.heads = (int)(heads_kvdiv & 0xffffu); p.kv_div = (int)(heads_kvdiv >> 16);
+    osg_pin_all(p.q, p.o, p.q_tok, p.q_head, p.q_batch, p.o_tok, p.o_head, p.o_batch, p.Tq, p.scale_log2e, p.mask, p.inv_scale);
     constexpr int DCH = D / 8;
     constexpr int RSC = DCH + ((6 - DCH % 4) % 4);
     constexpr int ROWB = RSC * 16;
@@ -283,7 +285,7 @@
     const int lq = lane & 15, g = lane >> 4;
     int L;
     {
-        const int total = gridDim.x, bid = blockIdx.x, x = bid & 7, i = bid >> 3, q = total >> 3, r = total & 7;
+        const int total = grid, bid = blockIdx.x, x = bid & 7, i = bid >> 3, q = total >> 3, r = total & 7;
         L = (x < r ? x * (q + 1) : r * (q + 1) + (x - r) * q) + i;
     }
     const int bh = L / nqb, qb = L - bh * nqb;
@@ -513,6 +515,17 @@
     }
 }
 
+int attn2_pack(osg_ctx* ctx, const AttnParams& p, int (&st)[6], unsigned* heads_kvdiv) {
+    const long s[6] = {p.k_tok, p.k_head, p.k_batch, p.v_tok, p.v_head, p.v_batch};
+    for (int i = 0; i < 6; i++) {
+        if (s[i] < 0 || s[i] > 0x7fffffffL) OSG_FAIL(ctx, "attention launch: a key / value stride does not fit the 32-bit kernel parameter");
+        st[i] = (int)s[i];
+    }
+    if (p.heads < 1 || p.heads > 0xffff || p.kv_div < 1 || p.kv_div > 0xffff) OSG_FAIL(ctx, "attention launch: heads and heads per key / value head must fit their 16-bit kernel parameter fields");
+    *heads_kvdiv = (unsigned)p.heads | ((unsigned)p.kv_div << 16);
+    return 0;
+}
+
 template <int D, int NST>
 int launch_attn2(osg_ctx* ctx, const AttnParams& p, int batch) {
     static const int force_qt = getenv("OSG_ATTN_QT") ? atoi(getenv("OSG_ATTN_QT")) : 0;
@@ -531,8 +544,11 @@
     const int nqb = qt2 ? (p.Tq + 127) / 128 : (p.Tq + 63) / 64;
     dim3 grid((unsigned)((long)nqb * batch * p.heads));
     osg_set_kernel(ctx, 0, 2, D, NST, qt2 ? 2 : 1, 64, (int)grid.x);
-    if (qt2) hipLaunchKernelGGL(k2, grid, dim3(256), smem, ctx->compute, p, nqb);
-    else hipLaunchKernelGGL(k1, grid, dim3(256), smem, ctx->compute, p, nqb);
+    int st[6];
+    unsigned hk;
+    if (attn2_pack(ctx, p, st, &hk)) return 1;
+    if (qt2) hipLaunchKernelGGL(k2, grid, dim3(256), smem, ctx->compute, (const void*)p.k, (const void*)p.v, st[0], st[1], st[2], st[3], st[4], st[5], p.Tkv, nqb, (int)grid.x, hk, p);
+    else hipLaunchKernelGGL(k1, grid, dim3(256), smem, ctx->compute, (const void*)p.k, (const void*)p.v, st[0], st[1], st[2], st[3], st[4], st[5], p.Tkv, nqb, (int)grid.x, hk, p);
     OSG_LAUNCH_CHECK(ctx);
     return 0;
 }
@@ -629,4 +645,13 @@
                                  1, heads, Tq, Tkv, D, scale);
 }
 
-}
+int osg_attention_kernarg_check(osg_ctx* ctx, long kv_stride, int heads, int kv_div) {
+    AttnParams p = {};
+    p.k_tok = p.k_head = p.k_batch = p.v_tok = p.v_head = p.v_batch = kv_stride;
+    p.heads = heads; p.kv_div = kv_div;
+    int st[6];
+    unsigned hk;
+    return attn2_pack(ctx, p, st, &hk);
+}
+
+}
diff --git a/onnxstream_amd/csrc/osg_conv3x3_kernel.h b/onnxstream_amd/csrc/osg_conv3x3_kernel.h
--- a/onnxstream_amd/csrc/osg_conv3x3_kernel.h
+++ b/onnxstream_amd/csrc/osg_conv3x3_kernel.h
@@ -161,6 +161,8 @@
         return;
     }
 
+    OSG_PIN(p.bias); OSG_PIN(p.residual); OSG_PIN(p.rowbias); OSG_PIN(p.rb_ld); OSG_PIN(p.rb_rows); OSG_PIN(p.bias_f32); OSG_PIN(p.act); OSG_PIN(p.no_epre);
+    if constexpr (WQ) { OSG_PIN(p.wq_sc); OSG_PIN(p.wq_zp); OSG_PIN(p.w_zp); }
     const int wm0 = (wave / WGN) * WM;
     const int wn0 = (wave % WGN) * WN;
     f32x4 acc[TM][TN];
@@ -341,12 +343,14 @@
 }
 
 template <int W_, int BN, int WGM, int WGN, int MODE, int NLW, int WQ = 0>
-__global__ __launch_bounds__(256 + 64 * NLW) void conv3x3_kernel(GemmParams pk) {
+__global__ __launch_bounds__(256 + 64 * NLW) void conv3x3_kernel(const void* A, const void* Bt, int M, int N, int K, int k_per_split, unsigned a_bytes, unsigned b_bytes, int grid,
+                                                                 int H, int Cin, unsigned sp_nm, GemmParams pk) {
     GemmParams p = pk;
-    OSG_PIN(p.A); OSG_PIN(p.Bt); OSG_PIN(p.kdbg); OSG_PIN(p.M); OSG_PIN(p.N); OSG_PIN(p.K); OSG_PIN(p.splits); OSG_PIN(p.k_per_split); OSG_PIN(p.a_bytes); OSG_PIN(p.b_bytes);
-    OSG_PIN(p.mt); OSG_PIN(p.nt); OSG_PIN(p.n_major); OSG_PIN(p.grid); OSG_PIN(p.H); OSG_PIN(p.Cin);
-    OSG_PIN(p.bias); OSG_PIN(p.residual); OSG_PIN(p.rowbias); OSG_PIN(p.rb_ld); OSG_PIN(p.rb_rows); OSG_PIN(p.bias_f32); OSG_PIN(p.act); OSG_PIN(p.no_epre);
-    if constexpr (WQ) { OSG_PIN(p.wq_sc); OSG_PIN(p.wq_zp); OSG_PIN(p.w_zp); }
+    p.A = (const f16*)A; p.Bt = (const f16*)Bt; p.M = M; p.N = N; p.K = K; p.k_per_split = k_per_split; p.a_bytes = a_bytes; p.b_bytes = b_bytes; p.grid = grid; p.H = H; p.Cin = Cin;
+    p.splits = (int)(sp_nm & ((1u << kPackSplitsBits) - 1)); p.n_major = (sp_nm & kPackNMajor) != 0;
+    p.mt = (M + 127) / 128; p.nt = (N + BN - 1) / BN;
+    p.kdbg = nullptr;
+    if (OSG_UNLIKELY(sp_nm & kPackKdbg)) p.kdbg = kernarg_rare(pk.kdbg);
     conv3x3_body<W_, BN, WGM, WGN, MODE, NLW, WQ>(p);
 }
 
@@ -371,8 +375,12 @@
         else p.sink[0].table = p.sink[1].table = nullptr;
     }
     p.grid = p.mt * p.nt * p.splits;
-    hipLaunchKernelGGL(kern, dim3((unsigned)p.grid), dim3(256 + 64 * NLW), smem, ctx->compute, p);
+    int lda32;
+    unsigned sp_nm;
+    const int bad = kernarg_pack(ctx, 0, p.splits, p.n_major, p.kdbg != nullptr, false, &lda32, &sp_nm);
+    if (!bad) hipLaunchKernelGGL(kern, dim3((unsigned)p.grid), dim3(256 + 64 * NLW), smem, ctx->compute, (const void*)p.A, (const void*)p.Bt, p.M, p.N, p.K, p.k_per_split, p.a_bytes, p.b_bytes, p.grid, p.H, p.Cin, sp_nm, p);
     p.sink[0] = sinks_in[0]; p.sink[1] = sinks_in[1];
+    if (bad) return 1;
     OSG_LAUNCH_CHECK(ctx);
     return 0;
 }
diff --git a/onnxstream_amd/csrc/osg_gemm.hip b/onnxstream_amd/csrc/osg_gemm.hip
--- a/onnxstream_amd/csrc/osg_gemm.hip
+++ b/onnxstream_amd/csrc/osg_gemm.hip
@@ -838,6 +838,12 @@
                        int Cin, int Cout, int KH, int KW, int sh, int sw, int pt, int pl, int pb, int pr, osg_act act) {
     return osg_conv2d_nhwc_w8_v(ctx, x, wq_ohwi, w_scale, w_zero_point, nullptr, nullptr, bias, bias_dtype, image_bias, image_bias_ld, residual, y, 0, nullptr, 0, N, H, W,
                                 Cin, Cout, KH, KW, sh, sw, pt, pl, pb, pr, act);
+}
+
+int osg_gemm_kernarg_check(osg_ctx* ctx, long lda, int splits) {
+    int lda32;
+    unsigned sp_nm;
+    return osg_mm::kernarg_pack(ctx, lda, splits, 0, false, false, &lda32, &sp_nm);
 }
 
 }
diff --git a/onnxstream_amd/csrc/osg_gemm2.h b/onnxstream_amd/csrc/osg_gemm2.h
--- a/onnxstream_amd/csrc/osg_gemm2.h
+++ b/onnxstream_amd/csrc/osg_gemm2.h
@@ -12,17 +12,20 @@
 using namespace osg_mm;
 
 template <int BM, int BN, int NST, bool CONV, int MODE = 0, int SPEC = 0, int LN = 0, int NCH = 5, int KS = 1, int WGN = 2, int WQ = 0>
-__global__ __launch_bounds__((SPEC || KS == 2) ? 512 : 256) void gemm2_kernel(GemmParams pk) {
+__global__ __launch_bounds__((SPEC || KS == 2) ? 512 : 256) void gemm2_kernel(const void* A, const void* Bt, int M, int N, int K, int k_per_split, unsigned a_bytes, unsigned b_bytes,
+                                                                              int grid, int lda, unsigned sp_nm, GemmParams pk) {
     GemmParams p = pk;
+    p.A = (const f16*)A; p.Bt = (const f16*)Bt; p.M = M; p.N = N; p.K = K; p.k_per_split = k_per_split; p.a_bytes = a_bytes; p.b_bytes = b_bytes; p.grid = grid; p.lda = lda;
+    p.splits = (int)(sp_nm & ((1u << kPackSplitsBits) - 1)); p.n_major = (sp_nm & kPackNMajor) != 0;
+    p.mt = (M + BM - 1) / BM; p.nt = (N + BN - 1) / BN;
+    p.kdbg = nullptr;
+    if (OSG_UNLIKELY(sp_nm & kPackKdbg)) p.kdbg = kernarg_rare(pk.kdbg);
 #if OSG_GEMM_PIN
-    OSG_PIN(p.A); OSG_PIN(p.Bt); OSG_PIN(p.kdbg); OSG_PIN(p.lda); OSG_PIN(p.strideA); OSG_PIN(p.strideB); OSG_PIN(p.M); OSG_PIN(p.N); OSG_PIN(p.K);
-    OSG_PIN(p.splits); OSG_PIN(p.k_per_split); OSG_PIN(p.a_bytes); OSG_PIN(p.b_bytes); OSG_PIN(p.mt); OSG_PIN(p.nt); OSG_PIN(p.n_major); OSG_PIN(p.grid);
     if constexpr (CONV) {
         OSG_PIN(p.H); OSG_PIN(p.W); OSG_PIN(p.Cin); OSG_PIN(p.Ho); OSG_PIN(p.Wo); OSG_PIN(p.KW); OSG_PIN(p.sh); OSG_PIN(p.sw); OSG_PIN(p.pt); OSG_PIN(p.pl);
     }
-    OSG_PIN(p.bias); OSG_PIN(p.residual); OSG_PIN(p.rowbias); OSG_PIN(p.rb_ld); OSG_PIN(p.strideC); OSG_PIN(p.ln_c1); OSG_PIN(p.rs_in); OSG_PIN(p.rb_rows);
-    OSG_PIN(p.bias_f32); OSG_PIN(p.act); OSG_PIN(p.no_epre); OSG_PIN(p.rs_np);
     if constexpr (WQ) { OSG_PIN(p.wq_sc); OSG_PIN(p.wq_zp); OSG_PIN(p.w_zp); }
+    if constexpr (LN == 2) { OSG_PIN(p.rs_in); OSG_PIN(p.rs_np); }
 #endif
     static_assert(KS == 1 || (KS == 2 && !SPEC && MODE == 0 && LN != 1), "KS = 2: plain kernel only (row statistics come from the producer, LN = 2, or not at all)");
     static_assert(WGN == 1 || WGN == 2, "wave grid: 2 x 2 or 4 x 1");
@@ -78,8 +81,14 @@
     const int nkt = (kend - kbeg) >> 6;
     const int nsteps = (nkt + KS - 1) / KS;
 
-    __amdgpu_buffer_rsrc_t rsA = __builtin_amdgcn_make_buffer_rsrc((void*)(p.A + (long)zb * p.strideA), 0, p.a_bytes, 0x00020000);
-    __amdgpu_buffer_rsrc_t rsB = __builtin_amdgcn_make_buffer_rsrc((void*)(p.Bt + (long)zb * p.strideB), 0, p.b_bytes, 0x00020000);
+    const f16* Ab = p.A;
+    const f16* Bb = p.Bt;
+    if (OSG_UNLIKELY(sp_nm & kPackBatch)) {
+        Ab += (long)zb * kernarg_rare(pk.strideA);
+        Bb += (long)zb * kernarg_rare(pk.strideB);
+    }
+    __amdgpu_buffer_rsrc_t rsA = __builtin_amdgcn_make_buffer_rsrc((void*)Ab, 0, p.a_bytes, 0x00020000);
+    __amdgpu_buffer_rsrc_t rsB = __builtin_amdgcn_make_buffer_rsrc((void*)Bb, 0, p.b_bytes, 0x00020000);
 
     const int rsub = lane >> 3;
     const int gch = (lane & 7) ^ rsub;
@@ -176,13 +185,17 @@
     constexpr bool EPRE = TM * TN <= 8;
     W8Ops<WQ ? TN : 1, true> w8;
     if constexpr (WQ) { if (math) w8_prefetch<TN, true>(p, w8, n0, wn0, lane); }
+    if (loads) {
+#pragma unroll
+        for (int s2 = 0; s2 < NST - 1; s2++) issue_tile(s2);
+    }
+#if OSG_GEMM_PIN
+    OSG_PIN(p.bias); OSG_PIN(p.residual); OSG_PIN(p.rowbias); OSG_PIN(p.rb_ld); OSG_PIN(p.strideC); OSG_PIN(p.ln_c1); OSG_PIN(p.rb_rows);
+    OSG_PIN(p.bias_f32); OSG_PIN(p.act); OSG_PIN(p.no_epre);
+#endif
     EpiOps<TM, TN, CONV, EPRE> epre;
     epre.have = false;
     if (math && !p.ln_c1 && grp == 0) epi_prefetch<TM, TN, CONV, EPRE>(p, epre, m0, n0, wm0, wn0, lane, zb);
-    if (loads) {
-#pragma unroll
-        for (int s2 = 0; s2 < NST - 1; s2++) issue_tile(s2);
-    }
     kdbg_stamp(p, 1);
     if constexpr (WQ) { if (math) w8_finalize<TN, true>(w8); }
 
@@ -300,8 +313,12 @@
         if (ok) { ctx->sink_fused = true; p.sink_imgs = p.M / p.sink_hw; p.sink_per_xcd = ctx->xcd_ids8 ? 1 : 0; }
         else p.sink[0].table = p.sink[1].table = nullptr;
     }
-    hipLaunchKernelGGL(kern, grid, dim3((SPEC || KS == 2) ? 512 : 256), smem, ctx->compute, p);
+    int lda32;
+    unsigned sp_nm;
+    const int bad = kernarg_pack(ctx, p.lda, p.splits, p.n_major, p.kdbg != nullptr, batch > 1, &lda32, &sp_nm);
+    if (!bad) hipLaunchKernelGGL(kern, grid, dim3((SPEC || KS == 2) ? 512 : 256), smem, ctx->compute, (const void*)p.A, (const void*)p.Bt, p.M, p.N, p.K, p.k_per_split, p.a_bytes, p.b_bytes, p.grid, lda32, sp_nm, p);
     p.sink[0] = sinks_in[0]; p.sink[1] = sinks_in[1];
+    if (bad) return 1;
     OSG_LAUNCH_CHECK(ctx);
     return 0;
 }
diff --git a/onnxstream_amd/csrc/osg_gemm_common.h b/onnxstream_amd/csrc/osg_gemm_common.h
--- a/onnxstream_amd/csrc/osg_gemm_common.h
+++ b/onnxstream_amd/csrc/osg_gemm_common.h
@@ -69,6 +69,26 @@
     int sink_imgs, sink_per_xcd;
     int fold_acc;
 };
+constexpr int kPackSplitsBits = 16;
+constexpr unsigned kPackNMajor = 1u << 16, kPackKdbg = 1u << 17, kPackBatch = 1u << 18;
+template <class T>
+__device__ __forceinline__ T kernarg_rare(T v) {
+    asm volatile("" : "+s"(v));
+    return v;
+}
+inline int kernarg_pack(osg_ctx* ctx, long lda, int splits, int n_major, bool kdbg, bool batched, int* lda32, unsigned* sp_nm) {
+    if (lda < 0 || lda > 0x7fffffffL) {
+        ctx->err = "contraction launch: the row pitch of A does not fit the 32-bit kernel parameter";
+        return 1;
+    }
+    if (splits < 1 || splits >= (1 << kPackSplitsBits)) {
+        ctx->err = "contraction launch: the number of k-slices does not fit its 16-bit kernel parameter field";
+        return 1;
+    }
+    *lda32 = (int)lda;
+    *sp_nm = (unsigned)splits | (n_major ? kPackNMajor : 0u) | (kdbg ? kPackKdbg : 0u) | (batched ? kPackBatch : 0u);
+    return 0;
+}
 #define OSG_PIN(x) asm volatile("" ::"s"(x))
 #define OSG_LIKELY(x) __builtin_expect(!!(x), 1)
 #define OSG_UNLIKELY(x) __builtin_expect(!!(x), 0)
diff --git a/onnxstream_amd/csrc/osg_tchain.hip b/onnxstream_amd/csrc/osg_tchain.hip
--- a/onnxstream_amd/csrc/osg_tchain.hip
+++ b/onnxstream_amd/csrc/osg_tchain.hip
@@ -300,7 +300,9 @@
 }
 
 template <int RT, int C, int D, int TKT, int NS>
-__global__ __launch_bounds__(256, RT == 2 && NS == 2 ? 2 : 1) void tblock_tail_kernel(TailParams p) {
+__global__ __launch_bounds__(256, RT == 2 && NS == 2 ? 2 : 1) void tblock_tail_kernel(const void* a1, const void* x0, const void* wo1, const void* bo1, const void* g2, const void* be2, int M, int rows_per_img, TailParams pk) {
+    TailParams p = pk;
+    p.a1 = (const f16*)a1; p.x0 = (const f16*)x0; p.wo1 = (const f16*)wo1; p.bo1 = (const f16*)bo1; p.g2 = (const f16*)g2; p.be2 = (const f16*)be2; p.M = M; p.rows_per_img = rows_per_img;
     constexpr int RB = 16 * RT;
     constexpr int TB = kTileBytes<RT>;
     constexpr int KT = C / 64;
@@ -673,7 +675,7 @@
         if (osg_first_on_device(attr_mask)) {
             OSG_HIP(ctx, hipFuncSetAttribute((const void*)kern, hipFuncAttributeMaxDynamicSharedMemorySize, smem));
         }
-        hipLaunchKernelGGL(kern, dim3((unsigned)(nblk + npf)), dim3(256), smem, ctx->compute, p);
+        hipLaunchKernelGGL(kern, dim3((unsigned)(nblk + npf)), dim3(256), smem, ctx->compute, (const void*)p.a1, (const void*)p.x0, (const void*)p.wo1, (const void*)p.bo1, (const void*)p.g2, (const void*)p.be2, p.M, p.rows_per_img, p);
         return 0;
     };
     constexpr int vec_bytes = (9 * 320 + 8 * 320) * 2;
diff --git a/onnxstream_amd/osgpu.py b/onnxstream_amd/osgpu.py
--- a/onnxstream_amd/osgpu.py
+++ b/onnxstream_amd/osgpu.py
@@ -19,7 +19,7 @@
     "osg_device_count", "osg_init", "osg_destroy", "osg_last_error", "osg_device_name", "osg_stream", "osg_set_autotune", "osg_tune_misses",
     "osg_malloc", "osg_free", "osg_upload", "osg_upload_sync", "osg_host_register", "osg_host_unregister", "osg_upload_pinned", "osg_upload_pinned_async", "osg_copy_fence", "osg_download", "osg_copy", "osg_memset", "osg_sync",
     "osg_graph_begin", "osg_graph_end", "osg_graph_launch", "osg_graph_destroy", "osg_timer_start", "osg_timer_stop",
-    "osg_conv2d_nhwc", "osg_conv2d_nhwc_rb", "osg_conv2d_nhwc_v", "osg_gemm", "osg_gemm_ln", "osg_gemm_rowstats", "osg_last_route", "osg_last_kernel", "osg_gemm_w8", "osg_conv2d_nhwc_w8", "osg_gemm_w8_v", "osg_conv2d_nhwc_w8_v", "osg_transpose_kn_to_nk", "osg_attention", "osg_attention_strided", "osg_sdpa", "osg_rms_norm", "osg_rope",
+    "osg_conv2d_nhwc", "osg_conv2d_nhwc_rb", "osg_conv2d_nhwc_v", "osg_gemm", "osg_gemm_ln", "osg_gemm_rowstats", "osg_last_route", "osg_last_kernel", "osg_gemm_kernarg_check", "osg_attention_kernarg_check", "osg_gemm_w8", "osg_conv2d_nhwc_w8", "osg_gemm_w8_v", "osg_conv2d_nhwc_w8_v", "osg_transpose_kn_to_nk", "osg_attention", "osg_attention_strided", "osg_sdpa", "osg_rms_norm", "osg_rope",
     "osg_instance_norm", "osg_group_norm_nhwc", "osg_layer_norm", "osg_reduce_mean_last", "osg_softmax_last",
     "osg_unary", "osg_binary", "osg_geglu", "osg_transpose", "osg_copy_2d", "osg_concat2", "osg_resize_nearest", "osg_gather_rows",
     "osg_maxpool_nhwc", "osg_convert", "osg_sampler_prepare", "osg_sampler_cfg_euler_a", "osg_sampler_cfg_multistep", "osg_sampler_prepare_rescale",
@@ -105,6 +105,9 @@
     lib.osg_gemm_rowstats.argtypes = [vp, vp, vp, vp, ci, vp, vp, ci, ci, ci, ci, vp]
     lib.osg_last_route.argtypes = [vp, ctypes.POINTER(ci)]
     lib.osg_last_kernel.argtypes = [vp, ctypes.POINTER(ci)]
+    if hasattr(lib, "osg_gemm_kernarg_check"):
+        lib.osg_gemm_kernarg_check.argtypes = [vp, cl, ci]
+        lib.osg_attention_kernarg_check.argtypes = [vp, cl, ci, ci]
     lib.osg_sampler_prepare.argtypes = [vp, vp, vp, vp, ci, cl, cf, cf, cl]
     lib.osg_sampler_cfg_euler_a.argtypes = [vp, vp, vp, vp, ci, cl, cf, cf, cf, cf, cf, cf]
     lib.osg_sampler_cfg_multistep.argtypes = [vp, ci, vp, vp, vp, vp, vp, vp, ci, cl, cf, cf, cf, cf, cf, cf, cf, cf, ctypes.c_double, ctypes.c_double]
```

New measurement: 10.09, median of 6. 1.02x the previous value.
